# hamaadshah/gan_deeplearning4j

Hardware: NVIDIA H100
Metric: images/sec (full G+D step) (higher is better)
Workload: dtype bf16

## Files before the change

gan_deeplearning4j_b200/__init__.py:

```python
from ._lib import B200GanError, LIB_PATH, PROTOTYPES, load
from .engine import BF16, FP32, EPI_ACTBWD, EPI_BNBWD, EPI_PLAIN, EPI_STATS, Context, Gan, Net, comm_unique_id, test_bn, test_conv, test_conv_ex, test_dropout, test_ew, test_pool
from . import data, models, parallel, serializer
```

gan_deeplearning4j_b200/_lib.py:

```python
from __future__ import annotations

import ctypes as C
import os

_HERE = os.path.dirname(os.path.abspath(__file__))
LIB_PATH = os.path.join(_HERE, "lib", "libb200gan.so")
NAME_LEN = 64


class B200GanError(RuntimeError):
    def __init__(self, code, msg):
        super().__init__(f"libb200gan error {code}: {msg}")
        self.code = code


class LayerDesc(C.Structure):
    _fields_ = [("type", C.c_int32), ("name", C.c_char * NAME_LEN), ("n_in", C.c_int32), ("n_out", C.c_int32),
                ("k_h", C.c_int32), ("k_w", C.c_int32), ("s_h", C.c_int32), ("s_w", C.c_int32), ("p_h", C.c_int32), ("p_w", C.c_int32),
                ("has_bias", C.c_int32), ("act", C.c_int32), ("act_alpha", C.c_float), ("updater", C.c_int32),
                ("lr", C.c_float), ("beta1", C.c_float), ("beta2", C.c_float), ("eps", C.c_float), ("l2", C.c_float),
                ("bn_decay", C.c_float), ("bn_eps", C.c_float), ("pre_h", C.c_int32), ("pre_w", C.c_int32), ("pre_c", C.c_int32),
                ("loss", C.c_int32), ("frozen", C.c_int32)]


class NetConfig(C.Structure):
    _fields_ = [("in_h", C.c_int32), ("in_w", C.c_int32), ("in_c", C.c_int32), ("max_batch", C.c_int32), ("precision", C.c_int32),
                ("grad_clip", C.c_float), ("xent_clip_eps", C.c_float), ("bn_groups", C.c_int32), ("seed", C.c_uint64)]


class GanConfig(C.Structure):
    _fields_ = [("fake_bn_train", C.c_int32), ("use_cuda_graph", C.c_int32)]


class LrSchedule(C.Structure):
    _fields_ = [("kind", C.c_int32), ("type", C.c_int32), ("initial", C.c_double), ("gamma", C.c_double), ("power", C.c_double),
                ("step", C.c_double), ("decay_rate", C.c_double), ("n_map", C.c_int32), ("map_keys", C.POINTER(C.c_int32)),
                ("map_values", C.POINTER(C.c_double))]


class Constraint(C.Structure):
    _fields_ = [("kind", C.c_int32), ("dims_mask", C.c_int32), ("max_norm", C.c_double), ("min_norm", C.c_double), ("rate", C.c_double)]


class ConvGeom(C.Structure):
    _fields_ = [(k, C.c_int32) for k in ("n", "h", "w", "c", "oh", "ow", "o", "kh", "kw", "sh", "sw", "ph", "pw")]


class TestConvOpts(C.Structure):
    _fields_ = [("epi", C.c_int32), ("act", C.c_int32), ("alpha", C.c_float), ("bias", C.POINTER(C.c_float)), ("scale", C.POINTER(C.c_float)),
                ("groups", C.c_int32), ("aux", C.POINTER(C.c_float)), ("aux2", C.POINTER(C.c_float)), ("stats", C.POINTER(C.c_double)), ("kernel", C.c_char * 64),
                ("bn", C.c_int32), ("max_ctas", C.c_int32), ("poison", C.c_int32), ("w_mn", C.c_int32), ("per_tap", C.c_int32), ("slab", C.c_int32),
                ("defer", C.c_int32), ("db", C.POINTER(C.c_float)), ("param_offset", C.c_int32), ("splits", C.c_int32)]


class EwReduceJob(C.Structure):
    _fields_ = [("n", C.c_int64), ("stride", C.c_int64), ("src_off", C.c_int64), ("dst_off", C.c_int64), ("splits", C.c_int32), ("wide", C.c_int32)]


class TestEwOpts(C.Structure):
    _fields_ = [("op", C.c_int32), ("n", C.c_int64), ("rows", C.c_int32), ("cols", C.c_int32), ("groups", C.c_int32), ("splits", C.c_int32),
                ("stride", C.c_int64)] + [(k, C.c_int32) for k in ("N", "H", "W", "C", "KH", "KW", "SH", "SW", "act")] + [
                ("alpha", C.c_float), ("clip_eps", C.c_float), ("offset", C.c_int32), ("in_place", C.c_int32), ("accumulate", C.c_int32),
                ("poison", C.c_int32), ("n_jobs", C.c_int32), ("jobs", C.POINTER(EwReduceJob)), ("n_seg", C.c_int32),
                ("seg_off", C.POINTER(C.c_int64)), ("seg_len", C.POINTER(C.c_int64)), ("seg_coef", C.POINTER(C.c_float)), ("sumsq", C.c_double),
                ("kernel", C.c_char * 64), ("loss", C.c_int32)]


class TestPoolOpts(C.Structure):
    _fields_ = [("op", C.c_int32), ("pool", C.c_int32), ("pnorm", C.c_float)] + [
                (k, C.c_int32) for k in ("N", "H", "W", "C", "KH", "KW", "SH", "SW", "PH", "PW", "offset", "poison")] + [
                ("kernel", C.c_char * 64), ("splits", C.c_int32)]


_vp, _i32, _i64, _fp = C.c_void_p, C.c_int32, C.c_int64, C.POINTER(C.c_float)
_pvp = C.POINTER(C.c_void_p)

PROTOTYPES = {
    "b2g_version": (_i32, []),
    "b2g_ctx_create": (_i32, [_i32, _pvp]),
    "b2g_ctx_destroy": (_i32, [_vp]),
    "b2g_last_error": (C.c_char_p, []),
    "b2g_sync": (_i32, [_vp]),
    "b2g_launch_count": (_i32, [_vp, C.POINTER(C.c_uint64)]),
    "b2g_timer_start": (_i32, [_vp]),
    "b2g_timer_stop_ms": (_i32, [_vp, _fp]),
    "b2g_flush_l2": (_i32, [_vp]),
    "b2g_device_info": (_i32, [_vp, C.POINTER(_i32), C.POINTER(_i32), C.POINTER(_i32), C.POINTER(C.c_uint64)]),
    "b2g_net_create": (_i32, [_vp, C.POINTER(NetConfig), C.POINTER(LayerDesc), _i32, _pvp]),
    "b2g_net_destroy": (_i32, [_vp]),
    "b2g_net_num_params": (_i32, [_vp, C.POINTER(_i64)]),
    "b2g_net_output_size": (_i32, [_vp, C.POINTER(_i64)]),
    "b2g_net_layer_output_size": (_i32, [_vp, _i32, C.POINTER(_i64)]),
    "b2g_net_set_param": (_i32, [_vp, C.c_char_p, C.c_char_p, _fp, _i64]),
    "b2g_net_get_param": (_i32, [_vp, C.c_char_p, C.c_char_p, _fp, _i64]),
    "b2g_net_get_params": (_i32, [_vp, _fp, _i64]),
    "b2g_net_set_params": (_i32, [_vp, _fp, _i64]),
    "b2g_net_get_gradients": (_i32, [_vp, _fp, _i64]),
    "b2g_net_updater_state_size": (_i32, [_vp, C.POINTER(_i64)]),
    "b2g_net_get_updater_state": (_i32, [_vp, _fp, _i64]),
    "b2g_net_set_updater_state": (_i32, [_vp, _fp, _i64]),
    "b2g_net_output": (_i32, [_vp, _fp, _i32, _i32, _fp]),
    "b2g_net_get_activation": (_i32, [_vp, _i32, _i32, _fp]),
    "b2g_net_compute_gradient_and_score": (_i32, [_vp, _fp, _fp, _i32, _fp]),
    "b2g_net_get_input_gradient": (_i32, [_vp, _i32, _fp]),
    "b2g_net_fit": (_i32, [_vp, _fp, _fp, _i32, _fp]),
    "b2g_net_get_iteration": (_i32, [_vp, C.POINTER(_i64)]),
    "b2g_net_set_iteration": (_i32, [_vp, _i64]),
    "b2g_net_get_dropout_pass": (_i32, [_vp, C.POINTER(_i64)]),
    "b2g_net_set_dropout_pass": (_i32, [_vp, _i64]),
    "b2g_net_set_gradient_normalization": (_i32, [_vp, _i32, C.c_float]),
    "b2g_net_set_lr_schedule": (_i32, [_vp, C.c_char_p, C.POINTER(LrSchedule)]),
    "b2g_net_set_constraints": (_i32, [_vp, C.c_char_p, C.c_char_p, C.POINTER(Constraint), _i32]),
    "b2g_net_apply_constraints": (_i32, [_vp]),
    "b2g_net_get_learning_rate": (_i32, [_vp, C.c_char_p, _fp]),
    "b2g_net_get_epoch": (_i32, [_vp, C.POINTER(_i64)]),
    "b2g_net_set_epoch": (_i32, [_vp, _i64]),
    "b2g_net_simt_gemm_calls": (_i32, [_vp, C.POINTER(C.c_uint64)]),
    "b2g_gan_create": (_i32, [_vp, _vp, C.POINTER(GanConfig), _pvp]),
    "b2g_gan_destroy": (_i32, [_vp]),
    "b2g_gan_step": (_i32, [_vp, _fp, _fp, _fp, _fp, _fp, _fp, _i32, _fp]),
    "b2g_gan_upload": (_i32, [_vp, _fp, _fp, _fp, _fp, _fp, _fp, _i32]),
    "b2g_gan_step_resident": (_i32, [_vp, _i32]),
    "b2g_gan_read_losses": (_i32, [_vp, _fp]),
    "b2g_gan_last_step_ms": (_i32, [_vp, _fp]),
    "b2g_comm_unique_id": (_i32, [_vp]),
    "b2g_ctx_comm_init": (_i32, [_vp, _i32, _i32, _vp]),
    "b2g_ctx_comm_destroy": (_i32, [_vp]),
    "b2g_net_set_grad_allreduce": (_i32, [_vp, _i32]),
    "b2g_net_average_parameters": (_i32, [_vp]),
    "b2g_net_set_sync_bn": (_i32, [_vp, _i32]),
    "b2g_net_set_grad_payload_bf16": (_i32, [_vp, _i32]),
    "b2g_net_enable_p2p_allreduce": (_i32, [_vp, C.POINTER(C.c_int32)]),
    "b2g_ctx_allreduce_test": (_i32, [_vp, _fp, _i64]),
    "b2g_test_conv": (_i32, [_vp, _i32, _i32, _i32, C.POINTER(ConvGeom), _fp, _fp, _fp, _i32, _fp]),
    "b2g_test_hbm_kernels": (_i32, [_vp, _i32, _i32, _i32, _fp]),
    "b2g_test_conv_ex": (_i32, [_vp, _i32, _i32, _i32, C.POINTER(ConvGeom), _fp, _fp, _fp, _i32, _fp, C.POINTER(TestConvOpts)]),
    "b2g_test_bn": (_i32, [_vp, _i32, _i32, _i32, _i32, _i32, _fp, _fp, _fp, _fp, _fp, _fp, _i32, C.c_float, C.c_float, C.c_float,
                           _i32, _fp, _fp, _fp, _fp, _fp, _fp, _fp, _fp]),
    "b2g_test_net_shadow": (_i32, [_vp, _i32, _i32, _fp, _i64]),
    "b2g_test_dropout": (_i32, [_vp, _i32, C.c_uint64, _i32, _i32, _i64, _i32, _i32, _i32, _i32, C.c_float, _fp, _fp, _fp, _fp]),
    "b2g_test_ew": (_i32, [_vp, _i32, C.POINTER(TestEwOpts), _fp, _fp, _fp, _fp, _fp]),
    "b2g_test_pool": (_i32, [_vp, _i32, C.POINTER(TestPoolOpts), _fp, _fp, _fp, _fp, _fp]),
}

_lib = None


def load():
    global _lib
    if _lib is not None:
        return _lib
    if not os.path.exists(LIB_PATH):
        raise B200GanError(-7, f"{LIB_PATH} is missing: build it with `make` (nvcc, sm_90a). There is no CPU fallback.")
    lib = C.CDLL(LIB_PATH, mode=C.RTLD_GLOBAL)
    for name, (res, args) in PROTOTYPES.items():
        fn = getattr(lib, name)
        fn.restype, fn.argtypes = res, args
    _lib = lib
    return lib


def check(code):
    if code != 0:
        raise B200GanError(code, load().b2g_last_error().decode(errors="replace"))
```

gan_deeplearning4j_b200/csrc/engine.cu:

```cuda
#include <cuda_runtime.h>
#include <dlfcn.h>
#include <math.h>
#include <stdarg.h>
#include <stdio.h>
#include <stdlib.h>
#include <string.h>

#include <algorithm>
#include <string>
#include <vector>

#include "../../include/b200gan.h"
#include "kernels.h"

using namespace b2g;

static thread_local char g_err[1024] = "";
static int32_t fail(int32_t code, const char* fmt, ...) {
  va_list ap; va_start(ap, fmt); vsnprintf(g_err, sizeof(g_err), fmt, ap); va_end(ap); return code;
}
#define CU(call) do { cudaError_t e_ = (call); if (e_ != cudaSuccess) return fail(B2G_ERR_CUDA, "%s:%d %s -> %s", __FILE__, __LINE__, #call, cudaGetErrorString(e_)); } while (0)
#define B2(call) do { int32_t r_ = (call); if (r_ != 0) return r_; } while (0)
#define CHECK_KERNELS() CU(cudaGetLastError())

// ... 336 lines not shown
      const size_t part = k_global_pool_partial_elems(n->prec, R, l.ih * l.iw, l.ic);
      if (part) {
        B2(dalloc(n, &l.pool_part, sizeof(float) * part));
        if (l.pool == B2G_POOL_MAX) B2(dalloc(n, &l.pool_part_idx, sizeof(int32_t) * part));
      }
      B2(dalloc(n, &l.pool_ticket, sizeof(unsigned))); CU(cudaMemsetAsync(l.pool_ticket, 0, sizeof(unsigned), n->ctx->stream));
    }
    if (l.d.type == B2G_LAYER_BATCHNORM) { B2(dalloc(n, &l.bn_fold, sizeof(float) * 2 * l.oc)); B2(dalloc(n, &l.bn_mean, sizeof(float) * G * l.oc)); B2(dalloc(n, &l.bn_invstd, sizeof(float) * G * l.oc)); scratch = std::max(scratch, k_bn_scratch_floats(l.oc, G));
      if (k_bn_vec_ok(n->prec, l.oc)) { B2(dalloc(n, &l.bn_coef, sizeof(float) * 4 * G * l.oc)); bn_acc_words += 2 * k_bn_acc_elems(l.oc, G); } }
    if (l.has_gemm()) {
      ConvGeom g = l.geom; g.N = R;
      scratch = std::max(scratch, std::max(k_simt_wgrad_scratch_floats(g), k_tc_wgrad_scratch_floats(g)));
      scratch = std::max(scratch, std::max(k_edge_wgrad_scratch_floats(g), k_dense_small_o_wgrad_scratch_floats(g)));
      scratch = std::max(scratch, k_tc_edge_wgrad_scratch_floats(g));
      scratch = std::max(scratch, k_colsum_scratch_floats(std::max(l.oc, l.ic)));
      max_w = std::max(max_w, (size_t)l.n_W);
      if (n->prec == PREC_BF16 && n->ctx->tc_ok && !l.d.frozen) {
        l.wg_part_floats = std::max(std::max(k_tc_wgrad_scratch_floats(g), k_tc_edge_wgrad_scratch_floats(g)), k_head_wgrad_scratch_floats(g));
        if (l.wg_part_floats) B2(dalloc(n, &l.wg_part, sizeof(float) * l.wg_part_floats));
      }
    }
  }
  if (bn_acc_words) {
    n->bn_acc_bytes = sizeof(unsigned long long) * bn_acc_words; B2(dalloc(n, &n->bn_acc, n->bn_acc_bytes));
    unsigned long long* q = n->bn_acc;
    for (auto& l : n->L) if (l.bn_coef) { const size_t w = k_bn_acc_elems(l.oc, G); l.acc_fwd = q; l.acc_bwd = q + w; q += 2 * w; }
  }
  n->eps_elems = (size_t)R * max_act;
  B2(dalloc(n, (char**)&n->epsA, ts * n->eps_elems)); B2(dalloc(n, (char**)&n->epsB, ts * n->eps_elems)); B2(dalloc(n, (char**)&n->epsC, ts * n->eps_elems));
  n->scratch_floats = scratch; B2(dalloc(n, &n->scratch, sizeof(float) * scratch)); B2(dalloc(n, &n->scratch2, sizeof(float) * scratch));
  {
    double tot_p = (double)std::max<int64_t>(1, n->n_params), tot_w = 0; std::vector<double> work(n->L.size(), 0.0);
    for (size_t i = 0; i < n->L.size(); ++i) { const auto& l = n->L[i]; if (l.has_gemm()) work[i] = (double)l.geom.OH * l.geom.OW * l.geom.O * l.geom.KH * l.geom.KW * l.geom.C; tot_w += work[i]; }
    double best = 0.0, ahead = 0.0;
    for (size_t i = 1; i < n->L.size(); ++i) {
      ahead += work[i - 1];
      const auto& l = n->L[i]; int64_t off = -1;
      if (l.has_gemm()) off = l.off_b >= 0 ? std::min(l.off_b, l.off_W) : l.off_W; else if (l.d.type == B2G_LAYER_BATCHNORM) off = l.off_gamma;
      if (off < 0 || tot_w <= 0) continue;
      const double score = std::min((tot_p - (double)off) / tot_p, ahead / tot_w);
      if (score > best) { best = score; n->ar_split_layer = (int)i; n->ar_split_off = off; }
    }
    if (best < 0.1) n->ar_split_layer = -1;
  }
  n->ev_fork.resize(n->L.size()); n->ev_done.resize(n->L.size());
  for (size_t i = 0; i < n->L.size(); ++i) { CU(cudaEventCreateWithFlags(&n->ev_fork[i], cudaEventDisableTiming)); CU(cudaEventCreateWithFlags(&n->ev_done[i], cudaEventDisableTiming)); }
  CU(cudaEventCreateWithFlags(&n->ev_join, cudaEventDisableTiming));
  n->stage_floats = std::max((size_t)R * max_act, std::max((size_t)n->n_params, max_w)); B2(dalloc(n, &n->stage_f32, sizeof(float) * n->stage_floats));
  return 0;
}

static int updater_kind(int u) { return u; }

static int32_t net_init_params_and_updater(b2g_net* n) {
  cudaStream_t s = n->ctx->stream;
  std::vector<float> hp(n->n_params, 0.f), h0(n->n_params, 0.f);
  uint64_t seed = n->cfg.seed ? n->cfg.seed : 666;
  std::vector<int64_t> l2o, l2l; std::vector<float> l2c;
  std::vector<int> seg_layer;
  for (auto& l : n->L) {
    const b2g_layer_desc& d = l.d;
    auto add_seg = [&](int64_t off, int64_t len, bool weight, bool noop) {
      if (d.frozen) return;
      UpdSeg sg{}; sg.off = off; sg.len = len; sg.kind = noop ? 3 : updater_kind(d.updater);
      sg.lr = d.lr; sg.b1 = d.beta1; sg.b2 = d.beta2; sg.eps = d.eps; sg.l2 = weight ? d.l2 : 0.f; sg.clip = n->cfg.grad_clip; sg.div_mb = noop ? 0 : 1;
      sg.off_bf = (weight && l.off_W_bf >= 0) ? l.off_W_bf : -1; sg.off_ps = (weight && l.off_Wps_bf >= 0) ? l.off_Wps_bf : -1; sg.ps_O = l.geom.O; sg.ps_C = l.geom.C; n->segs.push_back(sg); seg_layer.push_back((int)(&l - n->L.data()));
      if (!noop && (sg.kind == 1 || sg.kind == 5)) for (int64_t i = 0; i < len; ++i) h0[off + i] = d.eps;
      if (weight && d.l2 != 0.f) { l2o.push_back(off); l2l.push_back(len); l2c.push_back(0.5f * d.l2); }
    };
    if (l.has_gemm()) {
      double fi = (double)d.n_in * l.wTaps, fo = (double)d.n_out * l.wTaps / ((d.type == B2G_LAYER_CONV2D || d.type == B2G_LAYER_DECONV2D) ? (double)(d.s_h * d.s_w) : 1.0);
      float sd = (float)sqrt(2.0 / (fi + fo));
      for (int64_t i = 0; i < l.n_W; ++i) hp[l.off_W + i] = sd * nrand(seed);
      if (l.off_b >= 0 && l.off_b < l.off_W) add_seg(l.off_b, d.n_out, false, false);
      add_seg(l.off_W, l.n_W, true, false);
      if (l.off_b >= 0 && l.off_b > l.off_W) add_seg(l.off_b, d.n_out, false, false);
    } else if (d.type == B2G_LAYER_BATCHNORM) {
      for (int c = 0; c < l.oc; ++c) { hp[l.off_gamma + c] = 1.f; hp[l.off_var + c] = 1.f; }
      add_seg(l.off_gamma, l.oc, false, false); add_seg(l.off_beta, l.oc, false, false);
      add_seg(l.off_mean, l.oc, false, true); add_seg(l.off_var, l.oc, false, true);
    }
  }
  CU(cudaMemcpyAsync(n->params, hp.data(), sizeof(float) * n->n_params, cudaMemcpyHostToDevice, s));
  CU(cudaMemcpyAsync(n->st0, h0.data(), sizeof(float) * n->n_params, cudaMemcpyHostToDevice, s));
  CU(cudaMemsetAsync(n->st1, 0, sizeof(float) * n->n_params, s)); CU(cudaMemsetAsync(n->grads, 0, sizeof(float) * n->n_params, s));
  bool amsgrad = false;
  for (const UpdSeg& sg : n->segs) { n->upd_ext = n->upd_ext || sg.kind >= 4; amsgrad = amsgrad || sg.kind == 8; }
  if (amsgrad) { B2(dalloc(n, &n->st2, sizeof(float) * n->n_params)); CU(cudaMemsetAsync(n->st2, 0, sizeof(float) * n->n_params, s)); }
  CU(cudaMemsetAsync(n->step_dev, 0, sizeof(int), s));
  std::vector<int32_t> cs; std::vector<int64_t> co;
  for (size_t i = 0; i < n->segs.size(); ++i) for (int64_t o = n->segs[i].off; o < n->segs[i].off + n->segs[i].len; o += UPD_CHUNK) { cs.push_back((int32_t)i); co.push_back(o); }
  n->nchunks = (int)cs.size();
  B2(dalloc(n, &n->segs_dev, sizeof(UpdSeg) * std::max<size_t>(1, n->segs.size()))); B2(dalloc(n, &n->chunk_seg_dev, sizeof(int32_t) * std::max(1, n->nchunks))); B2(dalloc(n, &n->chunk_off_dev, sizeof(int64_t) * std::max(1, n->nchunks)));
  CU(cudaMemcpyAsync(n->segs_dev, n->segs.data(), sizeof(UpdSeg) * n->segs.size(), cudaMemcpyHostToDevice, s));
  CU(cudaMemcpyAsync(n->chunk_seg_dev, cs.data(), sizeof(int32_t) * cs.size(), cudaMemcpyHostToDevice, s));
  CU(cudaMemcpyAsync(n->chunk_off_dev, co.data(), sizeof(int64_t) * co.size(), cudaMemcpyHostToDevice, s));
  {
    const int ns = (int)n->segs.size();
    std::vector<int32_t> seg_c0(ns + 1, n->nchunks);
    for (int c = n->nchunks - 1; c >= 0; --c) seg_c0[cs[c]] = c;
    std::vector<GnGroup> per_layer, per_param;
    for (int i = 0; i < ns; ++i) {
      per_param.push_back(GnGroup{seg_c0[i], seg_c0[i + 1], i, i + 1});
      if (i > 0 && seg_layer[i] == seg_layer[i - 1]) { per_layer.back().chunk_end = seg_c0[i + 1]; per_layer.back().seg_end = i + 1; }
      else per_layer.push_back(GnGroup{seg_c0[i], seg_c0[i + 1], i, i + 1});
    }
    n->gn_n_layer_groups = (int)per_layer.size(); n->gn_n_param_groups = (int)per_param.size();
    B2(dalloc(n, &n->gn_layer_groups, sizeof(GnGroup) * std::max<size_t>(1, per_layer.size()))); B2(dalloc(n, &n->gn_param_groups, sizeof(GnGroup) * std::max<size_t>(1, per_param.size())));
    B2(dalloc(n, &n->gn_partial, sizeof(double) * std::max(1, n->nchunks))); B2(dalloc(n, &n->gn_mult, sizeof(float) * std::max(1, ns)));
    B2(dalloc(n, &n->gn_ticket, sizeof(unsigned))); CU(cudaMemsetAsync(n->gn_ticket, 0, sizeof(unsigned), s));
    CU(cudaMemcpyAsync(n->gn_layer_groups, per_layer.data(), sizeof(GnGroup) * per_layer.size(), cudaMemcpyHostToDevice, s));
    CU(cudaMemcpyAsync(n->gn_param_groups, per_param.data(), sizeof(GnGroup) * per_param.size(), cudaMemcpyHostToDevice, s));
  }
  {
    n->seg_layer = seg_layer; n->layer_sched.assign(n->L.size(), b2g_net::LayerSched{});
    B2(dalloc(n, &n->sched_dev, sizeof(UpdSched) * std::max<size_t>(1, n->segs.size()))); CU(cudaMemsetAsync(n->sched_dev, 0, sizeof(UpdSched) * std::max<size_t>(1, n->segs.size()), s));
    B2(dalloc(n, &n->epoch_dev, sizeof(int64_t))); CU(cudaMemsetAsync(n->epoch_dev, 0, sizeof(int64_t), s));
    B2(dalloc(n, &n->lr_out, sizeof(float)));
  }
  n->n_l2 = (int)l2o.size();
  if (n->n_l2) {
    B2(dalloc(n, &n->l2_off_dev, sizeof(int64_t) * n->n_l2)); B2(dalloc(n, &n->l2_len_dev, sizeof(int64_t) * n->n_l2)); B2(dalloc(n, &n->l2_coef_dev, sizeof(float) * n->n_l2));
    CU(cudaMemcpyAsync(n->l2_off_dev, l2o.data(), sizeof(int64_t) * n->n_l2, cudaMemcpyHostToDevice, s));
    CU(cudaMemcpyAsync(n->l2_len_dev, l2l.data(), sizeof(int64_t) * n->n_l2, cudaMemcpyHostToDevice, s));
    CU(cudaMemcpyAsync(n->l2_coef_dev, l2c.data(), sizeof(float) * n->n_l2, cudaMemcpyHostToDevice, s));
  }
  CU(cudaStreamSynchronize(s));
  return 0;
}

static void net_refresh_shadow(b2g_net* n, int only_layer = -1) {
  if (n->prec != PREC_BF16) return;
  cudaStream_t st = n->ctx->stream;
  for (size_t i = 0; i < n->L.size(); ++i) { auto& l = n->L[i];
    if (!l.has_gemm() || (only_layer >= 0 && (int)i != only_layer)) continue;
    if (l.off_Wps_bf >= 0) k_pack_deconv_ps(n->params + l.off_W, n->shadow + l.off_Wps_bf, l.geom.O, l.geom.C, st);
    k_cast_f32_to_bf16(n->params + l.off_W, n->shadow + l.off_W_bf, (size_t)l.n_W, st);
  }
}

struct FwdOpts { int rows; int groups; bool train; bool update_running; void* out_override; };

static const void* w_ptr(const b2g_net* n, const LayerRT& l, int* wprec) {
  if (n->prec == PREC_BF16) { *wprec = PREC_BF16; return n->shadow + l.off_W_bf; }
  *wprec = PREC_F32; return n->params + l.off_W;
}

static inline bool tc_on(const b2g_net* n) { return n->prec == PREC_BF16 && n->ctx->tc_ok; }
static inline cudaStream_t fstream(const b2g_net* n) { return n->fwd_stream ? n->fwd_stream : n->ctx->stream; }
static inline void note_simt(b2g_net* n) { if (n->prec == PREC_BF16) ++n->simt_gemm_calls; }

static inline int sync_bn_world(const b2g_net* n) { return (n->sync_bn && n->ctx->comm && n->ctx->world > 1) ? n->ctx->world : 1; }
static int32_t gemm_fprop(b2g_net* n, const LayerRT& l, const ConvGeom& g, const void* x, const float* bias, void* out, int act, float alpha,
                          const float* scale = nullptr, const TcEpi* fuse = nullptr, bool* fused = nullptr) {
  cudaStream_t s = fstream(n); int wp; const void* w = w_ptr(n, l, &wp);
  if (fused) *fused = false;
  if (scale) {
    if (tc_on(n) && tc_fprop_supported(g)) { TcEpi e{}; e.mode = EPI_PLAIN; e.scale = scale; return k_tc_fprop(g, (const __nv_bfloat16*)x, (const __nv_bfloat16*)w, bias, (__nv_bfloat16*)out, act, alpha, s, &e) == 0 ? 0 : fail(B2G_ERR_CUDA, "tensor-core fprop launch failed"); }
    note_simt(n); k_simt_fprop(n->prec, wp, g, x, w, bias, out, act, alpha, s, scale); return 0;
  }
  if (tc_on(n) && tc_edge_conv_supported(g) && k_tc_edge_conv(g, (const __nv_bfloat16*)x, (const __nv_bfloat16*)w, bias, (__nv_bfloat16*)out, act, alpha, s) == 0) return 0;
  if (edge_conv_small_cin_supported(g)) { note_simt(n); k_edge_conv_small_cin(n->prec, wp, g, x, w, bias, out, act, alpha, s); return 0; }
  if (dense_small_o_supported(g)) { note_simt(n); k_dense_small_o_fwd(n->prec, wp, g, x, w, bias, out, act, alpha, s); return 0; }
  if (tc_on(n) && tc_fprop_supported(g)) {
    if (fuse && k_tc_fprop(g, (const __nv_bfloat16*)x, (const __nv_bfloat16*)w, bias, (__nv_bfloat16*)out, act, alpha, s, fuse) == 0) { if (fused) *fused = true; return 0; }
    if (k_tc_fprop(g, (const __nv_bfloat16*)x, (const __nv_bfloat16*)w, bias, (__nv_bfloat16*)out, act, alpha, s) == 0) return 0;
    return fail(B2G_ERR_CUDA, "tensor-core fprop launch failed");
  }
  if (n->prec == PREC_BF16 && head_conv_supported(g)) { k_head_fwd(g, (const __nv_bfloat16*)x, (const __nv_bfloat16*)w, bias, (__nv_bfloat16*)out, act, alpha, s); return 0; }
  note_simt(n); k_simt_fprop(n->prec, wp, g, x, w, bias, out, act, alpha, s); return 0;
}
static int32_t gemm_dgrad(b2g_net* n, const LayerRT& l, const ConvGeom& g, const void* dy, const float* bias, void* dx, int act, float alpha,
                          const float* scale = nullptr, const TcEpi* fuse = nullptr, bool* fused = nullptr) {
  cudaStream_t s = fstream(n); int wp; const void* w = w_ptr(n, l, &wp);
  if (fused) *fused = false;
  if (scale) {
    if (tc_on(n) && tc_dgrad_supported(g) && !edge_deconv_small_c_supported(g)) { TcEpi e{}; e.mode = EPI_PLAIN; e.scale = scale; return k_tc_dgrad(g, (const __nv_bfloat16*)dy, (const __nv_bfloat16*)w, bias, (__nv_bfloat16*)dx, act, alpha, s, &e) == 0 ? 0 : fail(B2G_ERR_CUDA, "tensor-core dgrad launch failed"); }
    note_simt(n); k_simt_dgrad(n->prec, wp, g, dy, w, bias, dx, act, alpha, s, scale); return 0;
  }
  if (tc_on(n) && l.off_Wps_bf >= 0 && tc_deconv_ps_supported(g)) {
    const TcEpi* f = (fuse && fuse->mode == EPI_ACTBWD) ? fuse : nullptr;
    if (k_tc_deconv_ps(g, (const __nv_bfloat16*)dy, n->shadow + l.off_Wps_bf, bias, (__nv_bfloat16*)dx, act, alpha, s, f) == 0) { if (fused) *fused = f != nullptr; return 0; }
    return fail(B2G_ERR_CUDA, "tensor-core pixel-shuffle deconv launch failed");
  }
  if (edge_deconv_small_c_supported(g)) { note_simt(n); k_edge_deconv_small_c(n->prec, wp, g, dy, w, bias, dx, act, alpha, s); return 0; }
  if (dense_small_o_supported(g) && !bias && act == ACT_IDENTITY) { note_simt(n); k_dense_small_o_dgrad(n->prec, wp, g, dy, w, dx, s); return 0; }
  if (dense_small_k_supported(g) && !(tc_on(n) && g.O % 64 == 0)) { note_simt(n); k_dense_small_k_dgrad(n->prec, wp, g, dy, w, bias, dx, act, alpha, s); return 0; }
  if (tc_on(n) && g.KH == 1 && g.KW == 1 && g.H == 1 && g.W == 1) {
    ConvGeom t = g; t.C = g.O; t.O = g.C;
    if (tc_fprop_supported(t)) {
      if (fuse && k_tc_fprop(t, (const __nv_bfloat16*)dy, (const __nv_bfloat16*)w, bias, (__nv_bfloat16*)dx, act, alpha, s, fuse, 1) == 0) { if (fused) *fused = true; return 0; }
      if (k_tc_fprop(t, (const __nv_bfloat16*)dy, (const __nv_bfloat16*)w, bias, (__nv_bfloat16*)dx, act, alpha, s, nullptr, 1) == 0) return 0;
      return fail(B2G_ERR_CUDA, "tensor-core dense dgrad launch failed");
    }
  }
  if (tc_on(n) && tc_dgrad_supported(g)) {
    if (fuse && k_tc_dgrad(g, (const __nv_bfloat16*)dy, (const __nv_bfloat16*)w, bias, (__nv_bfloat16*)dx, act, alpha, s, fuse) == 0) { if (fused) *fused = true; return 0; }
    if (k_tc_dgrad(g, (const __nv_bfloat16*)dy, (const __nv_bfloat16*)w, bias, (__nv_bfloat16*)dx, act, alpha, s) == 0) return 0;
    return fail(B2G_ERR_CUDA, "tensor-core dgrad launch failed");
  }
  if (n->prec == PREC_BF16 && head_conv_supported(g)) { k_head_dgrad(g, (const __nv_bfloat16*)dy, (const __nv_bfloat16*)w, bias, (__nv_bfloat16*)dx, act, alpha, s); return 0; }
  note_simt(n); k_simt_dgrad(n->prec, wp, g, dy, w, bias, dx, act, alpha, s); return 0;
}
static int32_t gemm_wgrad(b2g_net* n, LayerRT& l, const ConvGeom& g, const void* x, const void* dy, float* dw, cudaStream_t s, float* scratch, float* db = nullptr, bool* bias_done = nullptr) {
  if (tc_on(n) && tc_edge_wgrad_supported(g) && l.wg_part) { const int r = k_tc_edge_wgrad(g, (const __nv_bfloat16*)x, (const __nv_bfloat16*)dy, dw, db, l.wg_part, l.wg_part_floats, 0, s, &n->pending); if (r >= 0) { if (bias_done) *bias_done = r == 1; return 0; } }
  if (edge_wgrad_small_cin_supported(g)) { note_simt(n); k_edge_wgrad_small_cin(n->prec, g, x, dy, dw, scratch, 0, s); return 0; }
  if (dense_small_o_supported(g)) { note_simt(n); k_dense_small_o_wgrad(n->prec, g, x, dy, dw, scratch, 0, s); return 0; }
  if (dense_small_k_supported(g) && !(tc_on(n) && tc_wgrad_supported(g))) { note_simt(n); k_dense_small_k_wgrad(n->prec, g, x, dy, dw, s); return 0; }
  if (tc_on(n) && tc_wgrad_supported(g) && l.wg_part) {
    if (k_tc_wgrad(g, (const __nv_bfloat16*)x, (const __nv_bfloat16*)dy, dw, l.wg_part, l.wg_part_floats, 0, s, &n->pending) == 0) return 0;
    return fail(B2G_ERR_CUDA, "tensor-core wgrad launch failed");
  }
  if (n->prec == PREC_BF16 && head_conv_supported(g) && l.wg_part) {
    if (k_head_wgrad(g, (const __nv_bfloat16*)x, (const __nv_bfloat16*)dy, dw, l.wg_part, l.wg_part_floats, 0, s, &n->pending) == 0) return 0;
    return fail(B2G_ERR_CUDA, "few-output conv weight gradient: partials larger than the layer's region");
  }
  note_simt(n); k_simt_wgrad(n->prec, g, x, dy, dw, scratch, n->scratch_floats, 0, s); return 0;
}

static DropoutArgs make_dropout_args(uint64_t seed, int layer, int rank, float p) {
  DropoutArgs a{}; a.seed = seed ? seed : 666; a.tag = (uint32_t)layer | ((uint32_t)rank << 16);
  a.keep_all = p >= 1.f ? 1 : 0; a.threshold = a.keep_all ? 0u : (uint32_t)floor((double)p * 4294967296.0); a.scale = 1.0f / p;
  return a;
}
static DropoutArgs dropout_args(const b2g_net* n, int layer) { return make_dropout_args(n->cfg.seed, layer, n->ctx->rank, n->L[layer].d.act_alpha); }

static int32_t net_forward(b2g_net* n, const void* in, const FwdOpts& o, const void** result) {
  cudaStream_t s = fstream(n);
  if (o.rows > n->max_rows || o.rows < 1) return fail(B2G_ERR_SHAPE, "batch %d outside [1, max_batch=%d]", o.rows, n->max_rows);
  if (o.groups < 1 || o.rows % o.groups) return fail(B2G_ERR_SHAPE, "batch %d not divisible into %d groups", o.rows, o.groups);
  const int R = o.rows; const void* cur = in;
  n->last_rows = R;
  if (o.train && n->bn_acc) CU(cudaMemsetAsync(n->bn_acc, 0, n->bn_acc_bytes, s));
  int last_drop = -1;
  if (o.train) for (size_t i = 0; i < n->L.size(); ++i) if (n->L[i].drop_active()) last_drop = (int)i;
  for (size_t i = 0; i < n->L.size(); ++i) {
    LayerRT& l = n->L[i]; const b2g_layer_desc& d = l.d;
    void* out = l.out;
    if (i + 1 == n->L.size() && o.out_override && !l.out_alias) out = o.out_override;
    const float* bias = l.off_b >= 0 ? n->params + l.off_b : nullptr;
    const bool gemm_then_bn = (d.type == B2G_LAYER_CONV2D || d.type == B2G_LAYER_DECONV2D || d.type == B2G_LAYER_DENSE) && i + 1 < n->L.size() && n->L[i + 1].d.type == B2G_LAYER_BATCHNORM;
    const bool remapped = d.type == B2G_LAYER_DECONV2D && l.geom.KH == 1 && l.geom.C != l.oc;
    if (gemm_then_bn && d.act == B2G_ACT_IDENTITY && !l.ext_act && (!o.train || n->L[i + 1].d.frozen) && !(i + 2 == n->L.size() && o.out_override) && !remapped &&
        !l.n_skip) {
      LayerRT& bn = n->L[i + 1];
      ConvGeom g = l.geom; g.N = R;
      k_bn_fold(n->params + bn.off_mean, n->params + bn.off_var, n->params + bn.off_gamma, n->params + bn.off_beta, bias, bn.oc, bn.d.bn_eps, bn.bn_fold, bn.bn_fold + bn.oc, s);
      if (d.type == B2G_LAYER_DECONV2D) B2(gemm_dgrad(n, l, g, cur, bn.bn_fold + bn.oc, bn.out, bn.fused_act, bn.fused_alpha, bn.bn_fold));
      else B2(gemm_fprop(n, l, g, cur, bn.bn_fold + bn.oc, bn.out, bn.fused_act, bn.fused_alpha, bn.bn_fold));
      cur = bn.out; ++i; continue;
    }
    TcEpi st{}; const TcEpi* fuse = nullptr; bool fused = false;
    if (gemm_then_bn && o.train && !n->L[i + 1].d.frozen && n->L[i + 1].bn_coef && !remapped && tc_on(n) && !l.ext_act) {
      st.mode = EPI_STATS; st.acc = n->L[i + 1].acc_fwd; st.imgs_per_group = R / o.groups; fuse = &st;
    }
    void* gout = l.ext_z ? l.ext_z : out;
    switch (d.type) {
      case B2G_LAYER_CONV2D: case B2G_LAYER_DENSE: case B2G_LAYER_OUTPUT: { ConvGeom g = l.geom; g.N = R; B2(gemm_fprop(n, l, g, cur, bias, gout, d.act, d.act_alpha, nullptr, fuse, &fused)); } break;
      case B2G_LAYER_DECONV2D: { ConvGeom g = l.geom; g.N = R; B2(gemm_dgrad(n, l, g, cur, bias, gout, d.act, d.act_alpha, nullptr, fuse, &fused)); } break;
      case B2G_LAYER_BATCHNORM: {
        int rows_pg = (R / o.groups) * l.oh * l.ow;
        const bool bn_train = o.train && !d.frozen;
        l.fwd_fused = false;
        if (bn_train && l.bn_coef) {
          if (!l.stats_by_producer) k_bn_stats_acc(cur, rows_pg, l.oc, o.groups, l.acc_fwd, s);
          const int reps = sync_bn_world(n);
          if (reps > 1) NC(g_nccl.ar(l.acc_fwd, l.acc_fwd, k_bn_acc_elems(l.oc, o.groups),  5,  0, n->ctx->comm, s));
          k_bn_apply_acc(cur, out, rows_pg, l.oc, o.groups, l.acc_fwd, n->params + l.off_gamma, n->params + l.off_beta, l.fused_act, l.fused_alpha, d.bn_eps, l.bn_coef,
                         n->params + l.off_mean, n->params + l.off_var, o.update_running ? n->grads + l.off_mean : nullptr, o.update_running ? n->grads + l.off_var : nullptr, d.bn_decay, s, reps);
          l.fwd_fused = true; l.stats_by_producer = false; l.fwd_groups = o.groups;
          break;
        }
        if (bn_train) k_bn_stats(n->prec, cur, rows_pg, l.oc, o.groups, n->scratch, l.bn_mean, l.bn_invstd, d.bn_eps, n->params + l.off_mean, n->params + l.off_var,
                                o.update_running ? n->grads + l.off_mean : nullptr, o.update_running ? n->grads + l.off_var : nullptr, d.bn_decay, s);
        else k_bn_prep_infer(n->params + l.off_mean, n->params + l.off_var, l.oc, o.groups, d.bn_eps, l.bn_mean, l.bn_invstd, s);
        k_bn_apply(n->prec, cur, out, rows_pg, l.oc, o.groups, l.bn_mean, l.bn_invstd, n->params + l.off_gamma, n->params + l.off_beta, l.fused_act, l.fused_alpha, s);
      } break;
      case B2G_LAYER_ACTIVATION:
        if (l.act_fused_into_prev) out = (void*)cur;
        else if (l.ext_act) k_act_ext_fwd(n->prec, l.ext_act, l.ext_alpha, cur, out, (size_t)R * l.out_elems, s);
        else k_act_fwd(n->prec, cur, out, (size_t)R * l.out_elems, d.act, d.act_alpha, s);
        break;
      case B2G_LAYER_MAXPOOL: k_maxpool_fwd(n->prec, cur, out, l.argmax, R, l.ih, l.iw, l.ic, l.oh, l.ow, d.k_h, d.k_w, d.s_h, d.s_w, s); break;
      case B2G_LAYER_SUBSAMPLING: k_pool2d_fwd(n->prec, l.pool, l.pnorm, cur, out, R, l.ih, l.iw, l.ic, l.oh, l.ow, d.k_h, d.k_w, d.s_h, d.s_w, d.p_h, d.p_w, s); break;
      case B2G_LAYER_GLOBAL_POOLING: k_global_pool_fwd(n->prec, l.pool, l.pnorm, cur, out, l.pool_idx, R, l.ih * l.iw, l.ic, l.pool_part, l.pool_part_idx, l.pool_ticket, s); break;
      case B2G_LAYER_UPSAMPLE2D: k_upsample_fwd(n->prec, cur, out, R, l.ih, l.iw, l.ic, d.k_h, s); break;
      case B2G_LAYER_LOSS: case B2G_LAYER_CNN_LOSS: out = (void*)cur; break;
      case B2G_LAYER_FF_TO_CNN: if (l.out_alias) out = (void*)cur; else k_permute(n->prec, cur, out, R, l.oc, l.oh * l.ow, 1, s); break;
      case B2G_LAYER_CNN_TO_FF: if (l.out_alias) out = (void*)cur; else k_permute(n->prec, cur, out, R, l.ic, l.ih * l.iw, 0, s); break;
      case B2G_LAYER_DROPOUT:
        l.drop_live = o.train && l.drop_active();
        if (l.drop_live) {
          k_dropout_fwd(n->prec, cur, l.drop_buf, l.drop_mask, (size_t)R * l.out_elems, dropout_args(n, (int)i), n->drop_pass, n->drop_ticket, (int)i == last_drop, s);
          out = l.drop_buf;
        } else out = (void*)cur;
        l.out = out;
        break;
      case B2G_LAYER_ELEMENTWISE: {
        const void* sk = n->L[l.vsrc].out;
        k_vertex_ew_fwd(n->prec, d.act, l.vorder ? sk : cur, l.vorder ? cur : sk, out, (size_t)R * l.out_elems, s);
      } break;
      case B2G_LAYER_MERGE: {
        const LayerRT& src = n->L[l.vsrc]; const size_t px = (size_t)R * l.oh * l.ow;
        if (l.vorder) k_merge_fwd(n->prec, src.out, cur, out, px, src.oc, l.ic, s);
        else k_merge_fwd(n->prec, cur, src.out, out, px, l.ic, src.oc, s);
      } break;
    }
    if (l.ext_z) k_act_ext_fwd(n->prec, l.ext_act, l.ext_alpha, l.ext_z, out, (size_t)R * l.out_elems, s);
    if (fuse) n->L[i + 1].stats_by_producer = fused;
    if (l.out_alias) l.out = out;
    cur = out;
  }
  CHECK_KERNELS();
  if (result) *result = cur;
  return 0;
}

static bool ar_overlap_on(const b2g_net* n) {
  static int on = -1; if (on < 0) { const char* e = getenv("B2G_AR_OVERLAP"); on = (e && e[0] == '1') ? 1 : 0; }
  return on && n->ctx->comm && n->ctx->world > 1 && n->grad_allreduce && n->ar_split_layer > 0 && !n->sync_bn;
}
static void flush_pending_reduce(b2g_net* n, cudaStream_t s2) { if (n->pending.count) { k_reduce_multi(n->pending, s2); n->pending.count = 0; } }

static int32_t net_backward(b2g_net* n, const void* net_in, void* eps, int rows, int groups, bool want_wgrad, bool need_input_grad, bool allreduce_follows = false,
                            const TcEpi* input_act = nullptr, bool* input_act_done = nullptr, bool top_act_done = false) {
  cudaStream_t s = n->ctx->stream, s2 = n->ctx->side; const int R = rows;
  void* cur = eps;
  if (input_act_done) *input_act_done = false;
  n->pending.count = 0;
  void* bufs[3] = {n->epsA, n->epsB, n->epsC}; cudaEvent_t reader[3] = {nullptr, nullptr, nullptr}; bool forked = false;
  auto other = [&](void* p) -> void* {
    int pick = -1;
    for (int k = 0; k < 3; ++k) if (bufs[k] != p && !reader[k]) { pick = k; break; }
    if (pick < 0) for (int k = 0; k < 3; ++k) if (bufs[k] != p) { pick = k; break; }
    if (reader[pick]) { cudaStreamWaitEvent(s, reader[pick], 0); reader[pick] = nullptr; }
    return bufs[pick];
  };
  auto fork_wgrad = [&](int li, const void* delta) {
    cudaEventRecord(n->ev_fork[li], s); cudaStreamWaitEvent(s2, n->ev_fork[li], 0); forked = true; (void)delta;
  };
  auto mark_reader = [&](int li, const void* delta) {
    cudaEventRecord(n->ev_done[li], s2);
    for (int k = 0; k < 3; ++k) if (bufs[k] == delta) reader[k] = n->ev_done[li];
  };
  std::vector<char> act_done(n->L.size(), 0);
  if (top_act_done) act_done.back() = 1;
  auto pick_fuse = [&](int i, TcEpi* e, int* target) -> bool {
    *target = -1;
    if (!tc_on(n)) return false;
    int k = i - 1; while (k >= 0 && n->L[k].act_fused_into_prev) --k;
    if (k < 0) { if (input_act) { *e = *input_act; *target = -2; return true; } return false; }
    for (int m = k; m < i; ++m) if (n->L[m].n_skip) return false;
    LayerRT& b = n->L[k];
    if (b.d.type == B2G_LAYER_BATCHNORM && b.fwd_fused && !b.d.frozen && b.fwd_groups == groups) {
      e->mode = EPI_BNBWD; e->acc = b.acc_bwd; e->imgs_per_group = R / groups; e->aux = (const __nv_bfloat16*)b.out; e->aux2 = (const __nv_bfloat16*)(k == 0 ? net_in : n->L[k - 1].out);
      e->act = b.fused_act; e->alpha = b.fused_alpha; *target = k; return true;
    }
    if (k == i - 1 && b.has_gemm() && b.d.act != B2G_ACT_IDENTITY && b.d.type != B2G_LAYER_OUTPUT) {
      e->mode = EPI_ACTBWD; e->aux = (const __nv_bfloat16*)b.out; e->act = b.d.act; e->alpha = b.d.act_alpha; *target = k; return true;
    }
    return false;
  };
  auto note_fused = [&](int target, const TcEpi& e, bool fused) {
    if (!fused || target == -1) return;
    if (target == -2) { if (input_act_done) *input_act_done = true; return; }
    if (e.mode == EPI_BNBWD) n->L[target].bwd_premul = true; else act_done[target] = 1;
  };
  for (int i = (int)n->L.size() - 1; i >= 0; --i) {
    LayerRT& l = n->L[i]; const b2g_layer_desc& d = l.d;
    const void* lin = i == 0 ? net_in : n->L[i - 1].out;
    bool need_in = need_input_grad;
    if (!need_in) for (int j = 0; j < i; ++j) if (!n->L[j].d.frozen && (n->L[j].has_gemm() || n->L[j].d.type == B2G_LAYER_BATCHNORM)) need_in = true;
    const bool want_wgrad_l = want_wgrad && !d.frozen;
    if (l.skip_acc) k_skip_add(n->prec, cur, l.skip_acc, (size_t)R * l.out_elems, s);
    switch (d.type) {
      case B2G_LAYER_LOSS: case B2G_LAYER_CNN_LOSS: break;
      case B2G_LAYER_ELEMENTWISE:
        if (need_in) k_vertex_ew_bwd(n->prec, d.act, l.vorder, cur, lin, n->L[l.vsrc].out, n->L[l.vsrc].skip_acc, l.vfirst ? 0 : 1, (size_t)R * l.out_elems, s);
        break;
      case B2G_LAYER_MERGE:
        if (need_in) {
          const LayerRT& src = n->L[l.vsrc]; void* nx = other(cur);
          k_merge_bwd(n->prec, cur, nx, src.skip_acc, (size_t)R * l.oh * l.ow, l.vorder ? src.oc : l.ic, l.vorder ? l.ic : src.oc, l.vorder == 0, l.vfirst ? 0 : 1, s);
          cur = nx;
        }
        break;
      case B2G_LAYER_CONV2D: case B2G_LAYER_DENSE: case B2G_LAYER_OUTPUT: {
        ConvGeom g = l.geom; g.N = R;
        if (d.act != B2G_ACT_IDENTITY && !act_done[i]) k_act_bwd_from_output(n->prec, l.out, cur, cur, (size_t)R * l.out_elems, d.act, d.act_alpha, s);
        if (l.ext_z) k_act_ext_bwd(n->prec, l.ext_act, l.ext_alpha, l.ext_z, cur, (size_t)R * l.out_elems, s);
        if (want_wgrad_l) {
          fork_wgrad(i, cur);
          bool bias_done = false;
          B2(gemm_wgrad(n, l, g, lin, cur, n->grads + l.off_W, s2, n->scratch2, l.off_b >= 0 ? n->grads + l.off_b : nullptr, &bias_done));
          if (l.off_b >= 0 && !bias_done) k_colsum(n->prec, cur, R * l.oh * l.ow, l.oc, n->scratch2, n->grads + l.off_b, 0, s2);
          mark_reader(i, cur);
        }
        if (need_in) { void* nx = other(cur); TcEpi e{}; int tgt; bool fused = false; const bool can = pick_fuse(i, &e, &tgt);
          B2(gemm_dgrad(n, l, g, cur, nullptr, nx, ACT_IDENTITY, 0.f, nullptr, can ? &e : nullptr, &fused)); note_fused(tgt, e, fused); cur = nx; }
      } break;
      case B2G_LAYER_DECONV2D: {
        ConvGeom g = l.geom; g.N = R;
        if (d.act != B2G_ACT_IDENTITY && !act_done[i]) k_act_bwd_from_output(n->prec, l.out, cur, cur, (size_t)R * l.out_elems, d.act, d.act_alpha, s);
        if (l.ext_z) k_act_ext_bwd(n->prec, l.ext_act, l.ext_alpha, l.ext_z, cur, (size_t)R * l.out_elems, s);
        if (want_wgrad_l) {
          fork_wgrad(i, cur);
          B2(gemm_wgrad(n, l, g,  cur,  lin, n->grads + l.off_W, s2, n->scratch2));
          if (l.off_b >= 0) k_colsum(n->prec, cur, R * l.oh * l.ow, l.oc, n->scratch2, n->grads + l.off_b, 0, s2);
          mark_reader(i, cur);
        }
        if (need_in) { void* nx = other(cur); TcEpi e{}; int tgt; bool fused = false; const bool can = pick_fuse(i, &e, &tgt);
          B2(gemm_fprop(n, l, g, cur, nullptr, nx, ACT_IDENTITY, 0.f, nullptr, can ? &e : nullptr, &fused)); note_fused(tgt, e, fused); cur = nx; }
      } break;
      case B2G_LAYER_BATCHNORM: {
        if (d.frozen) { if (need_in) return fail(B2G_ERR_UNSUPPORTED, "layer %d: a gradient through a frozen BatchNorm (trainable layer or input gradient below it) is not implemented", i); break; }
        if (l.fwd_fused && l.fwd_groups != groups) return fail(B2G_ERR_ARG, "layer %d: BatchNorm backward in %d groups after a forward in %d", i, groups, l.fwd_groups);
        int rows_pg = (R / groups) * l.oh * l.ow; void* nx = need_in ? other(cur) : nullptr;
        if (l.fwd_fused) {
          if (!l.bwd_premul) k_bn_bwd_stats_acc(lin, cur, rows_pg, l.oc, groups, l.bn_coef, l.fused_act, l.fused_alpha, l.acc_bwd, s);
          const int reps = sync_bn_world(n);
          if (reps > 1) NC(g_nccl.ar(l.acc_bwd, l.acc_bwd, k_bn_acc_elems(l.oc, groups),  5,  0, n->ctx->comm, s));
          k_bn_bwd_apply_acc(lin, cur, nx, rows_pg, l.oc, groups, l.bn_coef, l.fused_act, l.fused_alpha, l.bwd_premul ? 1 : 0, l.acc_bwd, n->grads + l.off_gamma, n->grads + l.off_beta, want_wgrad_l ? 1 : 0, s, reps);
          l.bwd_premul = false;
        } else
        k_bn_bwd(n->prec, lin, cur, nx, rows_pg, l.oc, groups, l.bn_mean, l.bn_invstd, n->params + l.off_gamma, n->params + l.off_beta, l.fused_act, l.fused_alpha,
                 n->scratch, n->grads + l.off_gamma, n->grads + l.off_beta, want_wgrad_l ? 1 : 0, s);
        if (need_in) cur = nx;
      } break;
      case B2G_LAYER_ACTIVATION:
        if (l.ext_act) k_act_ext_bwd(n->prec, l.ext_act, l.ext_alpha, lin, cur, (size_t)R * l.out_elems, s);
        else if (!l.act_fused_into_prev) k_act_bwd_from_output(n->prec, l.out, cur, cur, (size_t)R * l.out_elems, d.act, d.act_alpha, s);
        break;
      case B2G_LAYER_MAXPOOL: if (need_in) { void* nx = other(cur); k_maxpool_bwd(n->prec, cur, l.argmax, nx, R, l.ih, l.iw, l.ic, l.oh, l.ow, d.k_h, d.k_w, d.s_h, d.s_w, s); cur = nx; } break;
      case B2G_LAYER_SUBSAMPLING:
        if (need_in) { void* nx = other(cur); k_pool2d_bwd(n->prec, l.pool, l.pnorm, cur, lin, l.out, nx, R, l.ih, l.iw, l.ic, l.oh, l.ow, d.k_h, d.k_w, d.s_h, d.s_w, d.p_h, d.p_w, s); cur = nx; }
        break;
      case B2G_LAYER_GLOBAL_POOLING:
        if (need_in) { void* nx = other(cur); k_global_pool_bwd(n->prec, l.pool, l.pnorm, cur, lin, l.out, l.pool_idx, nx, R, l.ih * l.iw, l.ic, s); cur = nx; }
        break;
      case B2G_LAYER_UPSAMPLE2D: if (need_in) { void* nx = other(cur); k_upsample_bwd(n->prec, cur, nx, R, l.ih, l.iw, l.ic, d.k_h, s); cur = nx; } break;
      case B2G_LAYER_FF_TO_CNN: if (!l.out_alias && need_in) { void* nx = other(cur); k_permute(n->prec, cur, nx, R, l.oc, l.oh * l.ow, 0, s); cur = nx; } break;
      case B2G_LAYER_CNN_TO_FF: if (!l.out_alias && need_in) { void* nx = other(cur); k_permute(n->prec, cur, nx, R, l.ic, l.ih * l.iw, 1, s); cur = nx; } break;
      case B2G_LAYER_DROPOUT: if (need_in && l.drop_live) k_dropout_bwd(n->prec, cur, cur, l.drop_mask, (size_t)R * l.out_elems, 1.0f / d.act_alpha, s); break;
    }
    if (i == n->ar_split_layer && want_wgrad && allreduce_follows && ar_overlap_on(n)) {
      b2g_ctx* c = n->ctx;
      cudaEventRecord(c->ev_c0, s); cudaStreamWaitEvent(c->comm_stream, c->ev_c0, 0);
      if (forked) { flush_pending_reduce(n, s2); cudaEventRecord(c->ev_c1, s2); cudaStreamWaitEvent(c->comm_stream, c->ev_c1, 0); }
      NC(g_nccl.ar(n->grads + n->ar_split_off, n->grads + n->ar_split_off, (size_t)(n->n_params - n->ar_split_off),  7,  0, c->comm, c->comm_stream));
      n->ar_tail_sent = true;
    }
    if (!need_in) { cur = nullptr; break; }
  }
  n->input_grad = cur;
  if (forked) { flush_pending_reduce(n, s2); cudaEventRecord(n->ev_join, s2); cudaStreamWaitEvent(s, n->ev_join, 0); }
  CHECK_KERNELS();
  return 0;
}

static int32_t net_allreduce_grads(b2g_net* n) {
  b2g_ctx* c = n->ctx; if (!c->comm || c->world == 1 || !n->grad_allreduce) return 0;
  if (n->ar_tail_sent) {
    n->ar_tail_sent = false;
    cudaEventRecord(c->ev_c0, c->stream); cudaStreamWaitEvent(c->comm_stream, c->ev_c0, 0);
    NC(g_nccl.ar(n->grads, n->grads, (size_t)n->ar_split_off,  7,  0, c->comm, c->comm_stream));
    cudaEventRecord(c->ev_c2, c->comm_stream); cudaStreamWaitEvent(c->stream, c->ev_c2, 0);
    return 0;
  }
  if (n->ar_bf16 && n->ar_buf) {
    k_cast_f32_to_bf16(n->grads, n->ar_buf, (size_t)n->n_params, c->stream);
    NC(g_nccl.ar(n->ar_buf, n->ar_buf, (size_t)n->n_params,  9,  0, c->comm, c->stream));
    k_nhwc_to_nchw_f32(PREC_BF16, n->ar_buf, n->grads, 1, 1, (int)n->n_params, c->stream);
    return 0;
  }
  if (n->p2p) {
    P2pArgs a{}; for (int r = 0; r < c->world; ++r) { a.grads[r] = n->p2p_peer_grads[r]; a.flags[r] = c->p2p_peer_flags[r]; }
    a.rank = c->rank; a.world = c->world; a.n = (size_t)n->n_params; a.state = c->p2p_state;
    k_p2p_allreduce(a, c->stream); CHECK_KERNELS(); return 0;
  }
  NC(g_nccl.ar(n->grads, n->grads, (size_t)n->n_params,  7,  0, c->comm, c->stream));
  return 0;
}
static void net_launch_constraints(b2g_net* n, cudaStream_t s) {
  for (const auto& r : n->con_rounds) {
    k_constraint_onepass(n->params, n->shadow, n->con_jobs, r.j0, r.j1, r.onepass_blocks, s);
    k_constraint_twopass(n->params, n->shadow, n->con_jobs, r.t0, r.t1, r.norm_blocks, r.scale_blocks, n->con_partial, n->con_ticket, n->con_mult, s);
  }
}
static int32_t net_update(b2g_net* n, int mb_local) {
  cudaStream_t s = n->ctx->stream; int W = n->ctx->comm ? n->ctx->world : 1;
  if (!n->grad_allreduce) W = 1;
  const float inv_mb = 1.0f / ((float)mb_local * W), inv_world = 1.0f / (float)W;
  const bool gn = n->gn_mode != B2G_GN_NONE;
  if (gn) {
    const bool per_layer = n->gn_mode == B2G_GN_RENORM_L2_LAYER || n->gn_mode == B2G_GN_CLIP_L2_LAYER;
    const bool clip = n->gn_mode == B2G_GN_CLIP_L2_LAYER || n->gn_mode == B2G_GN_CLIP_L2_PARAM;
    k_gradnorm(n->grads, n->segs_dev, n->chunk_seg_dev, n->chunk_off_dev, n->nchunks, per_layer ? n->gn_layer_groups : n->gn_param_groups,
               per_layer ? n->gn_n_layer_groups : n->gn_n_param_groups, clip ? 1 : 0, n->gn_threshold, inv_mb, inv_world, n->gn_partial, n->gn_ticket, n->gn_mult, s);
  }
  k_updater(n->params, n->grads, n->st0, n->st1, n->st2, n->segs_dev, n->chunk_seg_dev, n->chunk_off_dev, n->nchunks, inv_mb, inv_world, n->step_dev, n->upd_ticket,
            n->shadow, gn ? n->gn_mult : nullptr, n->sched_on ? n->sched_dev : nullptr, n->epoch_dev, n->upd_ext, s);
  net_launch_constraints(n, s);
  CHECK_KERNELS();
  return 0;
}

extern "C" int32_t b2g_version(void) { return B2G_VERSION; }
extern "C" const char* b2g_last_error(void) { return g_err; }

extern "C" int32_t b2g_ctx_create(int32_t device, b2g_ctx** out) {
  if (!out) return fail(B2G_ERR_ARG, "null out");
  int count = 0; cudaError_t e = cudaGetDeviceCount(&count);
  if (e != cudaSuccess || count == 0) return fail(B2G_ERR_NO_DEVICE, "no CUDA device (%s); libb200gan has no CPU fallback", e == cudaSuccess ? "count=0" : cudaGetErrorString(e));
  if (device < 0 || device >= count) return fail(B2G_ERR_ARG, "device %d of %d", device, count);
  CU(cudaSetDevice(device));
  b2g_ctx* c = new b2g_ctx(); c->device = device;
  CU(cudaGetDeviceProperties(&c->prop, device));
  if (c->prop.major != 9) { int mj = c->prop.major, mn = c->prop.minor; delete c; return fail(B2G_ERR_NO_DEVICE, "device is sm_%d%d; this library is built for sm_90a (H100) only", mj, mn); }
  CU(cudaStreamCreateWithFlags(&c->stream, cudaStreamNonBlocking));
  CU(cudaStreamCreateWithFlags(&c->side, cudaStreamNonBlocking)); CU(cudaStreamCreateWithFlags(&c->side2, cudaStreamNonBlocking));
  CU(cudaEventCreateWithFlags(&c->ev_a, cudaEventDisableTiming)); CU(cudaEventCreateWithFlags(&c->ev_b, cudaEventDisableTiming));
  CU(cudaStreamCreateWithFlags(&c->comm_stream, cudaStreamNonBlocking));
  CU(cudaEventCreateWithFlags(&c->ev_c0, cudaEventDisableTiming)); CU(cudaEventCreateWithFlags(&c->ev_c1, cudaEventDisableTiming)); CU(cudaEventCreateWithFlags(&c->ev_c2, cudaEventDisableTiming));
  c->tc_ok = tc_init() == 0;
  *out = c; return 0;
}
extern "C" int32_t b2g_ctx_destroy(b2g_ctx* c) {
  if (!c) return 0; cudaSetDevice(c->device);
  if (c->p2p_flags_mapped) for (int r = 0; r < c->world; ++r) if (r != c->rank && c->p2p_peer_flags[r]) cudaIpcCloseMemHandle(c->p2p_peer_flags[r]);
  if (c->p2p_flags) cudaFree(c->p2p_flags); if (c->p2p_state) cudaFree(c->p2p_state);
  if (c->comm && g_nccl.destroy) g_nccl.destroy(c->comm);
  if (c->t0) { cudaEventDestroy(c->t0); cudaEventDestroy(c->t1); } if (c->flush_buf) cudaFree(c->flush_buf);
  if (c->side) cudaStreamDestroy(c->side); if (c->side2) cudaStreamDestroy(c->side2); if (c->ev_a) cudaEventDestroy(c->ev_a); if (c->ev_b) cudaEventDestroy(c->ev_b);
  if (c->comm_stream) cudaStreamDestroy(c->comm_stream); if (c->ev_c0) cudaEventDestroy(c->ev_c0); if (c->ev_c1) cudaEventDestroy(c->ev_c1); if (c->ev_c2) cudaEventDestroy(c->ev_c2);
  if (c->stream) cudaStreamDestroy(c->stream); delete c; return 0;
}
extern "C" int32_t b2g_timer_start(b2g_ctx* c) {
  if (!c) return fail(B2G_ERR_ARG, "null ctx"); CU(cudaSetDevice(c->device));
  if (!c->t0) { CU(cudaEventCreate(&c->t0)); CU(cudaEventCreate(&c->t1)); }
  CU(cudaEventRecord(c->t0, c->stream)); return 0;
}
extern "C" int32_t b2g_timer_stop_ms(b2g_ctx* c, float* ms) {
  if (!c || !ms || !c->t0) return fail(B2G_ERR_ARG, "timer not started"); CU(cudaSetDevice(c->device));
  CU(cudaEventRecord(c->t1, c->stream)); CU(cudaEventSynchronize(c->t1)); CU(cudaEventElapsedTime(ms, c->t0, c->t1)); return 0;
}
extern "C" int32_t b2g_flush_l2(b2g_ctx* c) {
  if (!c) return fail(B2G_ERR_ARG, "null ctx"); CU(cudaSetDevice(c->device));
  if (!c->flush_buf) { c->flush_bytes = (size_t)256 << 20; CU(cudaMalloc(&c->flush_buf, c->flush_bytes)); }
  CU(cudaMemsetAsync(c->flush_buf, 0, c->flush_bytes, c->stream)); return 0;
}
extern "C" int32_t b2g_sync(b2g_ctx* c) { if (!c) return fail(B2G_ERR_ARG, "null ctx"); CU(cudaSetDevice(c->device)); CU(cudaStreamSynchronize(c->stream)); return 0; }
extern "C" int32_t b2g_launch_count(b2g_ctx* c, uint64_t* out) { if (!c || !out) return fail(B2G_ERR_ARG, "null"); *out = g_launch_count; return 0; }
extern "C" int32_t b2g_device_info(b2g_ctx* c, int32_t* sm, int32_t* mj, int32_t* mn, uint64_t* mem) {
  if (!c) return fail(B2G_ERR_ARG, "null ctx");
  if (sm) *sm = c->prop.multiProcessorCount; if (mj) *mj = c->prop.major; if (mn) *mn = c->prop.minor; if (mem) *mem = c->prop.totalGlobalMem; return 0;
}

extern "C" int32_t b2g_net_create(b2g_ctx* ctx, const b2g_net_config* cfg, const b2g_layer_desc* layers, int32_t nl, b2g_net** out) {
  if (!ctx || !cfg || !layers || nl < 1 || !out) return fail(B2G_ERR_ARG, "b2g_net_create: null/empty argument");
  if (cfg->max_batch < 1 || cfg->in_h < 1 || cfg->in_w < 1 || cfg->in_c < 1) return fail(B2G_ERR_ARG, "b2g_net_create: bad input type / max_batch");
  if (cfg->precision != B2G_PREC_FP32 && cfg->precision != B2G_PREC_BF16) return fail(B2G_ERR_ARG, "b2g_net_create: precision %d", cfg->precision);
  for (int32_t i = 0; i < nl; ++i)
    if (layers[i].updater < B2G_UPD_SGD || layers[i].updater > B2G_UPD_ADADELTA) return fail(B2G_ERR_ARG, "b2g_net_create: layer %d: unknown updater %d", i, layers[i].updater);
  CU(cudaSetDevice(ctx->device));
  b2g_net* n = new b2g_net(); n->ctx = ctx; n->cfg = *cfg; n->prec = cfg->precision == B2G_PREC_BF16 ? PREC_BF16 : PREC_F32;
  if (n->cfg.bn_groups < 1) n->cfg.bn_groups = 1;
  int32_t r = net_build(n, layers, nl); if (!r) r = net_alloc(n); if (!r) r = net_init_params_and_updater(n);
  if (!r) { net_refresh_shadow(n); cudaError_t e = cudaStreamSynchronize(ctx->stream); if (e != cudaSuccess) r = fail(B2G_ERR_CUDA, "init: %s", cudaGetErrorString(e)); }
  if (r) { for (void* p : n->allocs) cudaFree(p); delete n; return r; }
  *out = n; return 0;
}
extern "C" int32_t b2g_net_destroy(b2g_net* n) {
  if (!n) return 0; cudaSetDevice(n->ctx->device); cudaStreamSynchronize(n->ctx->stream); cudaStreamSynchronize(n->ctx->side);
  for (auto e : n->ev_fork) if (e) cudaEventDestroy(e); for (auto e : n->ev_done) if (e) cudaEventDestroy(e); if (n->ev_join) cudaEventDestroy(n->ev_join);
  if (n->p2p) for (int r = 0; r < n->ctx->world; ++r) if (r != n->ctx->rank && n->p2p_peer_grads[r]) cudaIpcCloseMemHandle(n->p2p_peer_grads[r]);
  if (n->sched_map) cudaFree(n->sched_map);
  cudaFree(n->con_jobs); cudaFree(n->con_partial); cudaFree(n->con_mult);
  for (void* p : n->allocs) cudaFree(p); delete n; return 0;
}
extern "C" int32_t b2g_net_num_params(b2g_net* n, int64_t* out) { if (!n || !out) return fail(B2G_ERR_ARG, "null"); *out = n->n_params; return 0; }
extern "C" int32_t b2g_net_output_size(b2g_net* n, int64_t* out) { if (!n || !out) return fail(B2G_ERR_ARG, "null"); *out = (int64_t)n->L.back().out_elems; return 0; }
extern "C" int32_t b2g_net_layer_output_size(b2g_net* n, int32_t layer, int64_t* out) {
  if (!n || !out || layer < 0 || layer >= (int)n->L.size()) return fail(B2G_ERR_ARG, "bad layer index"); *out = (int64_t)n->L[layer].out_elems; return 0;
}

struct ParamRef { int64_t off, len; bool conv_w; int A, B, taps; int layer; };
static int32_t find_param(b2g_net* n, const char* layer, const char* param, ParamRef* r) {
  for (size_t i = 0; i < n->L.size(); ++i) { LayerRT& l = n->L[i];
    if (strncmp(l.d.name, layer, B2G_NAME_LEN)) continue;
    r->conv_w = false; r->layer = (int)i;
    if (!strcmp(param, "W") && l.off_W >= 0) { r->off = l.off_W; r->len = l.n_W; r->conv_w = l.wTaps > 1; r->A = l.wA; r->B = l.wB; r->taps = l.wTaps; return 0; }
    if (!strcmp(param, "b") && l.off_b >= 0) { r->off = l.off_b; r->len = l.d.n_out; return 0; }
    if (l.d.type == B2G_LAYER_BATCHNORM) {
      if (!strcmp(param, "gamma")) { r->off = l.off_gamma; r->len = l.oc; return 0; }
      if (!strcmp(param, "beta")) { r->off = l.off_beta; r->len = l.oc; return 0; }
      if (!strcmp(param, "mean")) { r->off = l.off_mean; r->len = l.oc; return 0; }
      if (!strcmp(param, "var")) { r->off = l.off_var; r->len = l.oc; return 0; }
    }
    return fail(B2G_ERR_ARG, "layer %s has no parameter %s", layer, param);
  }
  return fail(B2G_ERR_ARG, "no layer named %s", layer);
}
extern "C" int32_t b2g_net_set_param(b2g_net* n, const char* layer, const char* param, const float* host, int64_t cnt) {
  if (!n || !layer || !param || !host) return fail(B2G_ERR_ARG, "null"); CU(cudaSetDevice(n->ctx->device));
  ParamRef r; B2(find_param(n, layer, param, &r));
  if (cnt != r.len) return fail(B2G_ERR_SHAPE, "%s.%s has %lld elements, got %lld", layer, param, (long long)r.len, (long long)cnt);
  std::vector<float> tmp; const float* src = host;
  if (r.conv_w) { tmp.resize(r.len); w_dl4j_to_internal(host, tmp.data(), r.A, r.B, r.taps); src = tmp.data(); }
// ... 1018 lines not shown
      }
      break;
    }
    case B2G_EW_ACT_FWD: case B2G_EW_ACT_BWD: {
      const size_t n = (size_t)o->n; const bool bwd = o->op == B2G_EW_ACT_BWD;
      if (!in0 || (bwd && !in1) || o->n < 1 || o->n > lim || o->act < B2G_ACT_IDENTITY || o->act > B2G_ACT_LRELU) return fail(B2G_ERR_ARG, "bad activation arguments");
      void *a = nullptr, *e = nullptr, *r = nullptr; B2(m.upT(in0, n, &a, off));
      if (bwd) B2(m.upT(in1, n, &e, off));
      if (bwd && o->in_place) r = e;
      else { B2(m.dev(n, ts, &r, off)); B2(poison(r, ts * n)); }
      if (bwd) k_act_bwd_from_output(prec, a, e, r, n, o->act, o->alpha, s);
      else k_act_fwd(prec, a, r, n, o->act, o->alpha, s);
      ran();
      B2(m.downT(out0, r, n));
      break;
    }
    case B2G_EW_ACT_EXT_FWD: case B2G_EW_ACT_EXT_BWD: {
      const size_t n = (size_t)o->n; const bool bwd = o->op == B2G_EW_ACT_EXT_BWD;
      if (!in0 || (bwd && !in1) || o->n < 1 || o->n > lim || !act_ext_kind(o->act) || !std::isfinite(o->alpha)) return fail(B2G_ERR_ARG, "bad activation arguments");
      void *z = nullptr, *r = nullptr; B2(m.upT(in0, n, &z, off));
      if (bwd) B2(m.upT(in1, n, &r, off));
      else { B2(m.dev(n, ts, &r, off)); B2(poison(r, ts * n)); }
      if (bwd) k_act_ext_bwd(prec, o->act, o->alpha, z, r, n, s);
      else k_act_ext_fwd(prec, o->act, o->alpha, z, r, n, s);
      ran();
      B2(m.downT(out0, r, n));
      break;
    }
    case B2G_EW_MAXPOOL: {
      if (!in0 || !in1 || o->N < 1 || o->C < 1 || o->KH < 1 || o->KW < 1 || o->SH < 1 || o->SW < 1 || o->H < o->KH || o->W < o->KW || o->KH * o->KW > 255)
        return fail(B2G_ERR_ARG, "bad MAXPOOL arguments");
      const int OH = (o->H - o->KH) / o->SH + 1, OW = (o->W - o->KW) / o->SW + 1;
      const size_t ni = (size_t)o->N * o->H * o->W * o->C, no = (size_t)o->N * OH * OW * o->C;
      if (ni > (size_t)lim) return fail(B2G_ERR_ARG, "MAXPOOL input too large");
      void *x = nullptr, *eo = nullptr, *y = nullptr, *ei = nullptr; uint8_t* arg = nullptr;
      B2(m.upT(in0, ni, &x, off)); B2(m.upT(in1, no, &eo, off)); B2(m.dev(no, ts, &y, off)); B2(m.dev(ni, ts, &ei, off)); B2(m.dev(no, 1, (void**)&arg, off));
      B2(poison(y, ts * no)); B2(poison(ei, ts * ni)); B2(poison(arg, no));
      k_maxpool_fwd(prec, x, y, arg, o->N, o->H, o->W, o->C, OH, OW, o->KH, o->KW, o->SH, o->SW, s); ran();
      k_maxpool_bwd(prec, eo, arg, ei, o->N, o->H, o->W, o->C, OH, OW, o->KH, o->KW, o->SH, o->SW, s); ran();
      B2(m.downT(out0, y, no)); B2(m.downT(out1, ei, ni));
      if (out2) {
        std::vector<uint8_t> h(no); CU(cudaMemcpyAsync(h.data(), arg, no, cudaMemcpyDeviceToHost, s)); CU(cudaStreamSynchronize(s));
        for (size_t i = 0; i < no; ++i) out2[i] = (float)h[i];
      }
      break;
    }
    case EW_POOL2D: {
      if (!po) return fail(B2G_ERR_ARG, "unknown op %d", o->op);
      if (!in0 || !in1 || o->N < 1 || o->H < 1 || o->W < 1 || o->C < 1 || o->KH < 1 || o->KW < 1 || o->SH < 1 || o->SW < 1 || po->PH < 0 || po->PW < 0 ||
          po->PH >= o->KH || po->PW >= o->KW || o->H + 2 * po->PH < o->KH || o->W + 2 * po->PW < o->KW || po->pool < B2G_POOL_AVG || po->pool > B2G_POOL_PNORM ||
          (po->pool == B2G_POOL_PNORM && !(po->pnorm >= 1.f && po->pnorm <= 1024.f && po->pnorm == floorf(po->pnorm))))
        return fail(B2G_ERR_ARG, "bad POOL2D arguments");
      const int OH = (o->H + 2 * po->PH - o->KH) / o->SH + 1, OW = (o->W + 2 * po->PW - o->KW) / o->SW + 1;
      const size_t ni = (size_t)o->N * o->H * o->W * o->C, no = (size_t)o->N * OH * OW * o->C;
      if (ni > (size_t)lim || no > (size_t)lim) return fail(B2G_ERR_ARG, "POOL2D tensors too large");
      void *x = nullptr, *eo = nullptr, *y = nullptr, *ei = nullptr;
      B2(m.upT(in0, ni, &x, off)); B2(m.upT(in1, no, &eo, off)); B2(m.dev(no, ts, &y, off)); B2(m.dev(ni, ts, &ei, off)); B2(poison(y, ts * no)); B2(poison(ei, ts * ni));
      const int pn = po->pool == B2G_POOL_PNORM ? (int)po->pnorm : 0;
      k_pool2d_fwd(prec, po->pool, pn, x, y, o->N, o->H, o->W, o->C, OH, OW, o->KH, o->KW, o->SH, o->SW, po->PH, po->PW, s); ran();
      k_pool2d_bwd(prec, po->pool, pn, eo, x, y, ei, o->N, o->H, o->W, o->C, OH, OW, o->KH, o->KW, o->SH, o->SW, po->PH, po->PW, s); ran();
      B2(m.downT(out0, y, no)); B2(m.downT(out1, ei, ni));
      break;
    }
    case EW_GLOBAL_POOL: {
      if (!po) return fail(B2G_ERR_ARG, "unknown op %d", o->op);
      if (!in0 || !in1 || o->N < 1 || o->H < 1 || o->W < 1 || o->C < 1 || po->pool < B2G_POOL_MAX || po->pool > B2G_POOL_PNORM ||
          (po->pool == B2G_POOL_PNORM && !(po->pnorm >= 1.f && po->pnorm <= 1024.f && po->pnorm == floorf(po->pnorm))))
        return fail(B2G_ERR_ARG, "bad GLOBAL_POOL arguments");
      const int HW = o->H * o->W;
      const size_t ni = (size_t)o->N * HW * o->C, no = (size_t)o->N * o->C;
      if (ni > (size_t)lim) return fail(B2G_ERR_ARG, "GLOBAL_POOL input too large");
      void *x = nullptr, *eo = nullptr, *y = nullptr, *ei = nullptr; int32_t *idx = nullptr, *part_idx = nullptr; float* part = nullptr; unsigned* ticket = nullptr;
      B2(m.upT(in0, ni, &x, off)); B2(m.upT(in1, no, &eo, off)); B2(m.dev(no, ts, &y, off)); B2(m.dev(ni, ts, &ei, off)); B2(m.dev(no, 4, (void**)&idx, off));
      const size_t np = std::max<size_t>(1, k_global_pool_partial_elems(prec, o->N, HW, o->C));
      B2(m.dev(np, 4, (void**)&part, off)); B2(m.dev(np, 4, (void**)&part_idx, off)); B2(m.dev(1, 4, (void**)&ticket, off)); CU(cudaMemsetAsync(ticket, 0, 4, s));
      B2(poison(y, ts * no)); B2(poison(ei, ts * ni)); B2(poison(idx, 4 * no));
      const int pn = po->pool == B2G_POOL_PNORM ? (int)po->pnorm : 0;
      k_global_pool_fwd(prec, po->pool, pn, x, y, po->pool == B2G_POOL_MAX ? idx : nullptr, o->N, HW, o->C, part, part_idx, ticket, s); ran();
      po->splits = g_pool_last_splits;
      k_global_pool_bwd(prec, po->pool, pn, eo, x, y, idx, ei, o->N, HW, o->C, s); ran();
      B2(m.downT(out0, y, no)); B2(m.downT(out1, ei, ni));
      if (out2) {
        std::vector<int32_t> h(no); CU(cudaMemcpyAsync(h.data(), idx, 4 * no, cudaMemcpyDeviceToHost, s)); CU(cudaStreamSynchronize(s));
        for (size_t i = 0; i < no; ++i) out2[i] = (float)h[i];
      }
      unsigned t = 1; CU(cudaMemcpyAsync(&t, ticket, 4, cudaMemcpyDeviceToHost, s)); CU(cudaStreamSynchronize(s));
      if (t != 0) return fail(B2G_ERR_CUDA, "GLOBAL_POOL: the forward left its ticket word at %u", t);
      break;
    }
    case B2G_EW_UPSAMPLE: {
      const int f = o->KH;
      if (!in0 || !in1 || o->N < 1 || o->H < 1 || o->W < 1 || o->C < 1 || f < 1) return fail(B2G_ERR_ARG, "bad UPSAMPLE arguments");
      const size_t ni = (size_t)o->N * o->H * o->W * o->C, no = ni * f * f;
      if (no > (size_t)lim) return fail(B2G_ERR_ARG, "UPSAMPLE output too large");
      void *x = nullptr, *eo = nullptr, *y = nullptr, *ei = nullptr;
      B2(m.upT(in0, ni, &x, off)); B2(m.upT(in1, no, &eo, off)); B2(m.dev(no, ts, &y, off)); B2(m.dev(ni, ts, &ei, off)); B2(poison(y, ts * no)); B2(poison(ei, ts * ni));
      k_upsample_fwd(prec, x, y, o->N, o->H, o->W, o->C, f, s); ran();
      k_upsample_bwd(prec, eo, ei, o->N, o->H, o->W, o->C, f, s); ran();
      B2(m.downT(out0, y, no)); B2(m.downT(out1, ei, ni));
      break;
    }
    case B2G_EW_SUMSQ: {
      if (!in0 || o->n < 1 || o->n_seg < 1 || !o->seg_off || !o->seg_len || !o->seg_coef) return fail(B2G_ERR_ARG, "bad SUMSQ arguments");
      for (int i = 0; i < o->n_seg; ++i)
        if (o->seg_off[i] < 0 || o->seg_len[i] < 0 || o->seg_off[i] + o->seg_len[i] > o->n) return fail(B2G_ERR_ARG, "segment %d outside the tensor", i);
      float *p = nullptr, *coef = nullptr; int64_t *so = nullptr, *sl = nullptr; double* res = nullptr;
      B2(m.upF(in0, (size_t)o->n, &p, off)); B2(m.upF(o->seg_coef, (size_t)o->n_seg, &coef, off)); B2(m.dev((size_t)o->n_seg, 8, (void**)&so, off)); B2(m.dev((size_t)o->n_seg, 8, (void**)&sl, off)); B2(m.dev(1, 8, (void**)&res, off));
      CU(cudaMemcpyAsync(so, o->seg_off, 8 * (size_t)o->n_seg, cudaMemcpyHostToDevice, s)); CU(cudaMemcpyAsync(sl, o->seg_len, 8 * (size_t)o->n_seg, cudaMemcpyHostToDevice, s));
      B2(poison(res, 8));
      k_sumsq_segments(p, so, sl, coef, o->n_seg, res, s); ran();
      CU(cudaMemcpyAsync(&o->sumsq, res, 8, cudaMemcpyDeviceToHost, s));
      break;
    }
    default: return fail(B2G_ERR_ARG, "unknown op %d", o->op);
  }
  CU(cudaStreamSynchronize(s)); CHECK_KERNELS();
  strncpy(o->kernel, names.c_str(), sizeof(o->kernel) - 1); o->kernel[sizeof(o->kernel) - 1] = 0;
  return 0;
}
extern "C" int32_t b2g_test_ew(b2g_ctx* c, int32_t precision, b2g_test_ew_opts* o, const float* in0, const float* in1, float* out0, float* out1, float* out2) {
  return test_ew_impl(c, precision, o, nullptr, in0, in1, out0, out1, out2);
}
extern "C" int32_t b2g_test_pool(b2g_ctx* c, int32_t precision, b2g_test_pool_opts* po, const float* in0, const float* in1, float* out0, float* out1, float* out2) {
  if (!c || !po) return fail(B2G_ERR_ARG, "null");
  if (po->op != B2G_TEST_POOL2D && po->op != B2G_TEST_GLOBAL_POOL) return fail(B2G_ERR_ARG, "unknown pooling op %d", po->op);
  b2g_test_ew_opts o{};
  o.op = po->op == B2G_TEST_POOL2D ? EW_POOL2D : EW_GLOBAL_POOL;
  o.N = po->N; o.H = po->H; o.W = po->W; o.C = po->C; o.KH = po->KH; o.KW = po->KW; o.SH = po->SH; o.SW = po->SW;
  o.offset = po->offset; o.poison = po->poison;
  po->splits = 1;
  B2(test_ew_impl(c, precision, &o, po, in0, in1, out0, out1, out2));
  memcpy(po->kernel, o.kernel, sizeof(po->kernel));
  return 0;
}

extern "C" int32_t b2g_test_net_shadow(b2g_net* n, int32_t layer, int32_t which, float* out, int64_t count) {
  if (!n || !out) return fail(B2G_ERR_ARG, "null");
  if (layer < 0 || layer >= (int)n->L.size()) return fail(B2G_ERR_ARG, "layer %d out of range", layer);
  if (n->prec != PREC_BF16) return fail(B2G_ERR_UNSUPPORTED, "FP32 nets keep no bf16 weight copies");
  const LayerRT& l = n->L[layer];
  int64_t off = -1, len = 0;
  if (which == 0) { off = l.off_W_bf; len = l.n_W; }
  else if (which == 1) { off = l.off_Wps_bf; len = (int64_t)k_tc_deconv_ps_weight_elems(l.geom); }
  else return fail(B2G_ERR_ARG, "which = %d (0 straight copy, 1 pixel-shuffle operand)", which);
  if (off < 0) return fail(B2G_ERR_UNSUPPORTED, "layer %d has no %s", layer, which ? "pixel-shuffle operand" : "bf16 weight copy");
  if (count != len) return fail(B2G_ERR_SHAPE, "layer %d operand has %lld elements, %lld requested", layer, (long long)len, (long long)count);
  CU(cudaSetDevice(n->ctx->device)); cudaStream_t s = n->ctx->stream;
  if ((size_t)len > n->stage_floats) return fail(B2G_ERR_SHAPE, "operand larger than the staging buffer");
  k_nhwc_to_nchw_f32(PREC_BF16, n->shadow + off, n->stage_f32, 1, 1, (int)len, s);
  CU(cudaMemcpyAsync(out, n->stage_f32, sizeof(float) * len, cudaMemcpyDeviceToHost, s)); CU(cudaStreamSynchronize(s)); CHECK_KERNELS();
  return 0;
}

extern "C" int32_t b2g_test_hbm_kernels(b2g_net* n, int32_t rows, int32_t channels, int32_t iters, float* ms3) {
  if (!n || !ms3 || rows < 8 || iters < 1) return fail(B2G_ERR_ARG, "bad arguments"); b2g_ctx* c = n->ctx; CU(cudaSetDevice(c->device)); cudaStream_t s = c->stream;
  if (!k_bn_vec_ok(PREC_BF16, channels)) return fail(B2G_ERR_UNSUPPORTED, "channels %d not supported by the vector BatchNorm kernels", channels);
  const size_t ne = (size_t)rows * channels; __nv_bfloat16 *x = nullptr, *e = nullptr, *y = nullptr; float *coef = nullptr, *gb = nullptr; unsigned long long* acc = nullptr;
  HookMem m(s, PREC_BF16);
  B2(m.dev(ne, 2, (void**)&x)); B2(m.dev(ne, 2, (void**)&e)); B2(m.dev(ne, 2, (void**)&y)); B2(m.upF(nullptr, 4 * (size_t)channels, &coef)); B2(m.upF(nullptr, 4 * (size_t)channels, &gb));
  B2(m.dev(k_bn_acc_elems(channels, 1), 8, (void**)&acc));
  CU(cudaMemsetAsync(x, 0x3c, 2 * ne, s)); CU(cudaMemsetAsync(e, 0x3c, 2 * ne, s)); CU(cudaMemsetAsync(acc, 0, 8 * k_bn_acc_elems(channels, 1), s)); k_fill_f32(coef, 1.0f, 4 * channels, s); k_fill_f32(gb, 1.0f, 4 * channels, s);
  cudaEvent_t e0, e1; B2(m.event(&e0)); B2(m.event(&e1));
  ms3[0] = ms3[1] = ms3[2] = 0.f;
  for (int which = 0; which < 3; ++which) for (int it = -1; it < iters; ++it) {
    B2(b2g_flush_l2(c));
    CU(cudaEventRecord(e0, s));
    if (which == 0) k_updater(n->params, n->grads, n->st0, n->st1, n->st2, n->segs_dev, n->chunk_seg_dev, n->chunk_off_dev, n->nchunks, 1.0f, 1.0f, n->step_dev, n->upd_ticket,
                              n->shadow, nullptr, nullptr, nullptr, n->upd_ext, s);
    else if (which == 1) k_bn_apply_acc(x, y, rows, channels, 1, acc, gb, gb + channels, ACT_LRELU, 0.2f, 1e-5f, coef, gb + 2 * channels, gb + 3 * channels, nullptr, nullptr, 0.9f, s);
    else k_bn_bwd_apply_acc(x, e, y, rows, channels, 1, coef, ACT_LRELU, 0.2f, 1, acc, gb, gb + channels, 0, s);
    CU(cudaEventRecord(e1, s)); CU(cudaEventSynchronize(e1));
    float ms = 0.f; CU(cudaEventElapsedTime(&ms, e0, e1)); if (it >= 0) ms3[which] += ms / iters;
  }
  CHECK_KERNELS();
  return 0;
}
```

gan_deeplearning4j_b200/csrc/kernels.h:

```cpp
#pragma once
#include <cuda_runtime.h>
#include <cuda_bf16.h>
#include <stdint.h>

namespace b2g {

enum Prec { PREC_F32 = 0, PREC_BF16 = 1 };
enum Act { ACT_IDENTITY = 0, ACT_TANH = 1, ACT_SIGMOID = 2, ACT_RELU = 3, ACT_LRELU = 4,
           ACT_ELU = 5, ACT_SELU = 6, ACT_SOFTPLUS = 7, ACT_SOFTSIGN = 8, ACT_HARDTANH = 9, ACT_HARDSIGMOID = 10, ACT_RELU6 = 11, ACT_SWISH = 12,
           ACT_CUBE = 13, ACT_RATIONALTANH = 14, ACT_RECTIFIEDTANH = 15, ACT_THRESHOLDEDRELU = 16, ACT_EXT_FIRST = ACT_ELU, ACT_EXT_LAST = ACT_THRESHOLDEDRELU };
enum Loss { LOSS_MSE = 2, LOSS_L1 = 3, LOSS_L2 = 4, LOSS_MAE = 5, LOSS_HINGE = 6, LOSS_SQUARED_HINGE = 7, LOSS_WASSERSTEIN = 8 };

inline size_t prec_size(int prec) { return prec == PREC_F32 ? 4 : 2; }

struct ConvGeom {
  int N, H, W, C;
  int OH, OW, O;
  int KH, KW, SH, SW, PH, PW;
};

extern uint64_t g_launch_count;
extern const char* g_ew_last_kernel;
int device_sm_count();

// ... 19 lines not shown
void k_bn_stats_acc(const void* x, int rows_per_group, int C, int groups, unsigned long long* acc, cudaStream_t s);
void k_bn_apply_acc(const void* x, void* y, int rows_per_group, int C, int groups, const unsigned long long* acc, const float* gamma, const float* beta,
                    int act, float alpha, float eps, float* coef, const float* run_mean, const float* run_var, float* g_mean, float* g_var, float decay, cudaStream_t s, int replicas = 1);
void k_bn_bwd_stats_acc(const void* x, const void* eps_out, int rows_per_group, int C, int groups, const float* coef, int act, float alpha, unsigned long long* acc, cudaStream_t s);
void k_bn_bwd_apply_acc(const void* x, const void* eps_out, void* eps_in, int rows_per_group, int C, int groups, const float* coef, int act, float alpha, int premul,
                        const unsigned long long* acc, float* g_gamma, float* g_beta, int want_param_grads, cudaStream_t s, int replicas = 1);

void k_act_fwd(int prec, const void* x, void* y, size_t n, int act, float alpha, cudaStream_t s);
void k_act_bwd_from_output(int prec, const void* a, const void* eps_out, void* eps_in, size_t n, int act, float alpha, cudaStream_t s);
bool act_ext_kind(int act);
void k_act_ext_fwd(int prec, int act, float alpha, const void* z, void* a, size_t n, cudaStream_t s);
void k_act_ext_bwd(int prec, int act, float alpha, const void* z, void* eps, size_t n, cudaStream_t s);
void k_maxpool_fwd(int prec, const void* x, void* y, uint8_t* argmax, int N, int H, int W, int C, int OH, int OW, int KH, int KW, int SH, int SW, cudaStream_t s);
void k_maxpool_bwd(int prec, const void* eps_out, const uint8_t* argmax, void* eps_in, int N, int H, int W, int C, int OH, int OW, int KH, int KW, int SH, int SW, cudaStream_t s);
void k_upsample_fwd(int prec, const void* x, void* y, int N, int H, int W, int C, int f, cudaStream_t s);
void k_upsample_bwd(int prec, const void* eps_out, void* eps_in, int N, int H, int W, int C, int f, cudaStream_t s);

enum Pool { POOL_MAX = 0, POOL_AVG = 1, POOL_SUM = 2, POOL_PNORM = 3 };
void k_pool2d_fwd(int prec, int kind, int pn, const void* x, void* y, int N, int H, int W, int C, int OH, int OW, int KH, int KW, int SH, int SW, int PH, int PW,
                  cudaStream_t s);
void k_pool2d_bwd(int prec, int kind, int pn, const void* eps_out, const void* x, const void* y, void* eps_in, int N, int H, int W, int C, int OH, int OW, int KH,
                  int KW, int SH, int SW, int PH, int PW, cudaStream_t s);
int k_global_pool_splits(int prec, int N, int HW, int C, int vec);
size_t k_global_pool_partial_elems(int prec, int max_rows, int HW, int C);
void k_global_pool_fwd(int prec, int kind, int pn, const void* x, void* y, int32_t* idx, int N, int HW, int C, float* part, int32_t* part_idx, unsigned* ticket,
                       cudaStream_t s);
void k_global_pool_bwd(int prec, int kind, int pn, const void* eps_out, const void* x, const void* y, const int32_t* idx, void* eps_in, int N, int HW, int C,
                       cudaStream_t s);
extern int g_pool_last_splits;

struct DropoutArgs { uint64_t seed; uint32_t tag; uint32_t threshold; float scale; int keep_all; };
void k_dropout_fwd(int prec, const void* x, void* y, uint32_t* mask, size_t n, const DropoutArgs& a, unsigned long long* pass, unsigned* ticket, int bump_pass, cudaStream_t s);
void k_dropout_bwd(int prec, const void* eps_out, void* eps_in, const uint32_t* mask, size_t n, float scale, cudaStream_t s);

void k_xent(int prec, const void* z, const float* y, void* dz, float* loss_sums, int rows_per_group, int groups, float clip_eps, cudaStream_t s);
void k_sigmoid_out(int prec, const void* z, void* p, size_t n, cudaStream_t s);
void k_softmax_xent(int prec, const void* z, const float* y, void* dz, void* p_out, float* loss_sums, int rows, int K, cudaStream_t s);
int k_loss_blocks(size_t n_per_group, int groups);
void k_loss(int prec, int loss, int act, float alpha, const void* z, const float* y, void* dz, float* loss_sums, int rows_per_group, int n_out, int groups,
            double* partial, unsigned* ticket, cudaStream_t s);
void k_cnn_xent(int prec, const void* z, const float* y, void* dz, float* loss_sums, size_t n_per_group, int groups, float clip_eps, double* partial,
                unsigned* ticket, cudaStream_t s);
int k_cnn_softmax_blocks(int rows_per_group, int groups);
void k_cnn_softmax_xent(int prec, const void* z, const float* y, void* dz, void* p_out, float* loss_sums, int rows_per_group, int C, int groups,
                        double* partial, unsigned* ticket, cudaStream_t s);

enum VertexOp { VERTEX_ADD = 0, VERTEX_SUBTRACT = 1, VERTEX_PRODUCT = 2, VERTEX_AVERAGE = 3, VERTEX_MAX = 4 };
void k_vertex_ew_fwd(int prec, int op, const void* a, const void* b, void* y, size_t n, cudaStream_t s);
void k_vertex_ew_bwd(int prec, int op, int order, void* eps, const void* spine, const void* skip, float* acc, int accumulate, size_t n, cudaStream_t s);
void k_merge_fwd(int prec, const void* a, const void* b, void* y, size_t P, int Ca, int Cb, cudaStream_t s);
void k_merge_bwd(int prec, const void* eps, void* dst, float* acc, size_t P, int Ca, int Cb, int spine_first, int accumulate, cudaStream_t s);
void k_skip_add(int prec, void* eps, const float* acc, size_t n, cudaStream_t s);

void k_colsum(int prec, const void* x, int rows, int C, float* scratch, float* out, int accumulate, cudaStream_t s);
size_t k_colsum_scratch_floats(int C);
void k_sumsq_segments(const float* p, const int64_t* seg_off, const int64_t* seg_len, const float* seg_coef, int nseg, double* out, cudaStream_t s);
void k_reduce_splits(const float* src, float* dst, size_t n, int splits, size_t stride, int accumulate, cudaStream_t s);
struct ReduceJob { const float* src; float* dst; int64_t n, stride; int splits, blocks; };
struct ReduceList { static const int MAX_JOBS = 24; ReduceJob jobs[MAX_JOBS]; int count; };
void reduce_list_push(ReduceList* rl, const float* src, float* dst, int64_t n, int splits, int64_t stride);
void k_reduce_multi(const ReduceList& rl, cudaStream_t s);

struct UpdSeg {
  int64_t off, len;
  int kind;
  float lr, b1, b2, eps;
  float l2;
  float clip;
  int div_mb;
  int64_t off_bf, off_ps;
  int ps_O, ps_C;
};
__device__ __forceinline__ void upd_shadow(const UpdSeg& sg, __nv_bfloat16* __restrict__ shadow, int64_t i, __nv_bfloat16 pb) {
  shadow[sg.off_bf + (i - sg.off)] = pb;
  if (sg.off_ps >= 0) {
    const int e = (int)(i - sg.off), c = e % sg.ps_C, tap = (e / sg.ps_C) % 16, o = e / (sg.ps_C * 16), r = tap >> 2, sx = tap & 3;
    const int py = (r == 0 || r == 2) ? 1 : 0, dyr = r == 3 ? -1 : r == 0 ? 1 : 0, px = (sx == 0 || sx == 2) ? 1 : 0, dxc = sx == 3 ? -1 : sx == 0 ? 1 : 0;
    shadow[sg.off_ps + ((int64_t)((py * 8 + px * 4 + c) * 9 + (dyr + 1) * 3 + (dxc + 1))) * sg.ps_O + o] = pb;
  }
}
struct UpdSched {
  int kind, type;
  int n_map;
  double initial, gamma, power, step, decay;
  const int32_t* keys; const double* vals;
};
void k_updater(float* params, const float* grads, float* st0, float* st1, float* st2, const UpdSeg* segs_dev, const int32_t* chunk_seg_dev,
               const int64_t* chunk_off_dev, int nchunks, float inv_mb, float inv_world, int* step_dev , unsigned* ticket,
               __nv_bfloat16* shadow, const float* gn_mult, const UpdSched* sched, const int64_t* epoch_dev, bool ext, cudaStream_t s);
void k_sched_lr(const UpdSeg* segs_dev, const UpdSched* sched, int seg, const int* step_dev, const int64_t* epoch_dev, float* out, cudaStream_t s);
static const int UPD_CHUNK = 4096;

struct GnGroup { int32_t chunk_begin, chunk_end, seg_begin, seg_end; };
void k_gradnorm(const float* grads, const UpdSeg* segs_dev, const int32_t* chunk_seg_dev, const int64_t* chunk_off_dev, int nchunks,
                const GnGroup* groups_dev, int ngroups, int clip, float threshold, float inv_mb, float inv_world, double* partial, unsigned* ticket,
                float* mult, cudaStream_t s);
enum { CON_ONEPASS = 0, CON_TWOPASS = 1, CON_ELEMWISE = 2 };
static const int CON_CHUNK = 4096, CON_SCHUNK = 256;
struct ConJob {
  UpdSeg sg;
  int kind, path;
  double max_norm, min_norm, rate;
  int K0, R0, K1, R1, K2, groups, R;
  int blk_begin, blocks, blk2_begin, blocks2, chunks;
  int64_t part_begin, mult_begin;
};
void k_constraint_onepass(float* params, __nv_bfloat16* shadow, const ConJob* jobs, int j0, int j1, int blocks, cudaStream_t s);
void k_constraint_twopass(float* params, __nv_bfloat16* shadow, const ConJob* jobs, int j0, int j1, int norm_blocks, int scale_blocks, double* partial,
                          unsigned* ticket, float* mult, cudaStream_t s);
void k_fill_f32(float* p, float v, size_t n, cudaStream_t s);
void k_scale_f32(float* p, float v, size_t n, cudaStream_t s);
struct P2pArgs { float* grads[8]; unsigned* flags[8]; int rank, world; size_t n; unsigned* state; };
void k_p2p_allreduce(const P2pArgs& a, cudaStream_t s);

void k_simt_fprop(int prec, int wprec, const ConvGeom& g, const void* x, const void* w, const float* bias, void* out, int act, float alpha, cudaStream_t s, const float* scale = nullptr);
void k_simt_dgrad(int prec, int wprec, const ConvGeom& g, const void* dy, const void* w, const float* bias, void* dx, int act, float alpha, cudaStream_t s, const float* scale = nullptr);
void k_simt_wgrad(int prec, const ConvGeom& g, const void* x, const void* dy, float* dw, float* scratch, size_t scratch_floats, int accumulate, cudaStream_t s);
size_t k_simt_wgrad_scratch_floats(const ConvGeom& g);
extern const char* g_gemm_last_kernel;
extern int g_gemm_last_splits;

bool edge_deconv_small_c_supported(const ConvGeom& g);
bool edge_conv_small_cin_supported(const ConvGeom& g);
bool edge_wgrad_small_cin_supported(const ConvGeom& g);
bool dense_small_o_supported(const ConvGeom& g);
void k_edge_deconv_small_c(int prec, int wprec, const ConvGeom& g, const void* dy, const void* w, const float* bias, void* dx, int act, float alpha, cudaStream_t s);
void k_edge_conv_small_cin(int prec, int wprec, const ConvGeom& g, const void* x, const void* w, const float* bias, void* out, int act, float alpha, cudaStream_t s);
void k_edge_wgrad_small_cin(int prec, const ConvGeom& g, const void* x, const void* dy, float* dw, float* scratch, int accumulate, cudaStream_t s);
size_t k_edge_wgrad_scratch_floats(const ConvGeom& g);
void k_dense_small_o_fwd(int prec, int wprec, const ConvGeom& g, const void* x, const void* w, const float* bias, void* out, int act, float alpha, cudaStream_t s);
void k_dense_small_o_dgrad(int prec, int wprec, const ConvGeom& g, const void* dy, const void* w, void* dx, cudaStream_t s);
void k_dense_small_o_wgrad(int prec, const ConvGeom& g, const void* x, const void* dy, float* dw, float* scratch, int accumulate, cudaStream_t s);
size_t k_dense_small_o_wgrad_scratch_floats(const ConvGeom& g);
bool dense_small_k_supported(const ConvGeom& g);
void k_dense_small_k_dgrad(int prec, int wprec, const ConvGeom& g, const void* dy, const void* w, const float* bias, void* dx, int act, float alpha, cudaStream_t s);
void k_dense_small_k_wgrad(int prec, const ConvGeom& g, const void* x, const void* dy, float* dw, cudaStream_t s);

bool head_conv_supported(const ConvGeom& g);
size_t k_head_wgrad_scratch_floats(const ConvGeom& g);
void k_head_fwd(const ConvGeom& g, const __nv_bfloat16* x, const __nv_bfloat16* w, const float* bias, __nv_bfloat16* out, int act, float alpha, cudaStream_t s);
void k_head_dgrad(const ConvGeom& g, const __nv_bfloat16* dy, const __nv_bfloat16* w, const float* bias, __nv_bfloat16* dx, int act, float alpha, cudaStream_t s);
int k_head_wgrad(const ConvGeom& g, const __nv_bfloat16* x, const __nv_bfloat16* dy, float* dw, float* part, size_t part_floats, int force_splits, cudaStream_t s,
                 ReduceList* defer);

bool tc_fprop_supported(const ConvGeom& g);
bool tc_dgrad_supported(const ConvGeom& g);
bool tc_wgrad_supported(const ConvGeom& g);
int  tc_init();
extern const char* g_tc_last_kernel;
extern int g_tc_test_bn, g_tc_test_max_ctas;
extern int g_tc_test_per_tap;
extern bool g_tc_last_slab;
extern int g_tc_test_splits, g_tc_last_splits;
enum { EPI_PLAIN = 0, EPI_STATS = 1, EPI_BNBWD = 2, EPI_ACTBWD = 3 };
struct TcEpi {
  int mode;
  const float* scale;
  unsigned long long* acc;
  int imgs_per_group;
  const __nv_bfloat16* aux;
  const __nv_bfloat16* aux2;
  int act; float alpha;
};
int k_tc_fprop(const ConvGeom& g, const __nv_bfloat16* x, const __nv_bfloat16* w, const float* bias, __nv_bfloat16* out, int act, float alpha, cudaStream_t s, const TcEpi* epi = nullptr, int w_mn = 0);
int k_tc_dgrad(const ConvGeom& g, const __nv_bfloat16* dy, const __nv_bfloat16* w, const float* bias, __nv_bfloat16* dx, int act, float alpha, cudaStream_t s, const TcEpi* epi = nullptr);
int k_tc_wgrad(const ConvGeom& g, const __nv_bfloat16* x, const __nv_bfloat16* dy, float* dw, float* scratch, size_t scratch_floats, int accumulate, cudaStream_t s, ReduceList* defer = nullptr);
size_t k_tc_wgrad_scratch_floats(const ConvGeom& g);
bool tc_deconv_ps_shape(const ConvGeom& g);
bool tc_deconv_ps_supported(const ConvGeom& g);
size_t k_tc_deconv_ps_weight_elems(const ConvGeom& g);
void k_pack_deconv_ps(const float* w, __nv_bfloat16* wps, int O, int C, cudaStream_t s);
bool tc_edge_conv_supported(const ConvGeom& g);
bool tc_edge_wgrad_supported(const ConvGeom& g);
size_t k_tc_edge_wgrad_scratch_floats(const ConvGeom& g);
int k_tc_edge_conv(const ConvGeom& g, const __nv_bfloat16* x, const __nv_bfloat16* w, const float* bias, __nv_bfloat16* out, int act, float alpha, cudaStream_t s);
int k_tc_edge_wgrad(const ConvGeom& g, const __nv_bfloat16* x, const __nv_bfloat16* dy, float* dw, float* db, float* scratch, size_t scratch_floats, int accumulate, cudaStream_t s, ReduceList* defer = nullptr);
int k_tc_deconv_ps(const ConvGeom& g, const __nv_bfloat16* dy, const __nv_bfloat16* wps, const float* bias, __nv_bfloat16* dx, int act, float alpha, cudaStream_t s, const TcEpi* epi = nullptr);

}
```

gan_deeplearning4j_b200/csrc/kernels_tc.cu:

```cuda
#include <cuda.h>
#include <stdio.h>
#include <stdlib.h>
#include <algorithm>

#include "common.cuh"
#include "kernels.h"

namespace b2g {

typedef CUresult (*PFN_encodeTiled)(CUtensorMap*, CUtensorMapDataType, cuuint32_t, void*, const cuuint64_t*, const cuuint64_t*, const cuuint32_t*,
                                    const cuuint32_t*, CUtensorMapInterleave, CUtensorMapSwizzle, CUtensorMapL2promotion, CUtensorMapFloatOOBfill);
static PFN_encodeTiled g_encode = nullptr;

int tc_init() {
  if (g_encode) return 0;
  void* fn = nullptr; cudaDriverEntryPointQueryResult q;
  if (cudaGetDriverEntryPoint("cuTensorMapEncodeTiled", &fn, cudaEnableDefault, &q) != cudaSuccess || !fn || q != cudaDriverEntryPointSuccess) return -1;
  g_encode = (PFN_encodeTiled)fn; return 0;
}

static int make_map_bf16(CUtensorMap* m, const void* base, int rank, const cuuint64_t* dims, const cuuint64_t* strides_bytes, const cuuint32_t* box, const cuuint32_t* estr) {
  if (!g_encode) return -1;
  CUresult r = g_encode(m, CU_TENSOR_MAP_DATA_TYPE_BFLOAT16, (cuuint32_t)rank, const_cast<void*>(base), dims, strides_bytes, box, estr, CU_TENSOR_MAP_INTERLEAVE_NONE,
                        CU_TENSOR_MAP_SWIZZLE_128B, CU_TENSOR_MAP_L2_PROMOTION_L2_256B, CU_TENSOR_MAP_FLOAT_OOB_FILL_NONE);
// ... 317 lines not shown
  const uint32_t bar_empty = bar_full + 8 * STAGES;
  const uint32_t park_full = bar_empty + 8 * STAGES;
  const uint32_t park_empty = park_full + 8 * S::PARKS;
  float* sst = reinterpret_cast<float*>(smem_gen + S::STAT_OFF);
  const int warp = threadIdx.x >> 5, lane = threadIdx.x & 31;
  const int num_kb = p.taps_h * p.taps_w * p.chunks;
  const int tiles = p.tiles_m * p.tiles_n * p.phases;
  auto tile_coords = [&](int t, int& nb0, int& phase, int& n0, int& y0) {
    const int mt = t % p.tiles_m, r = t / p.tiles_m;
    nb0 = (r % p.tiles_n) * BN; phase = r / p.tiles_n;
    if (p.Nt > 1) { n0 = mt * p.Nt; y0 = 0; } else { n0 = mt / p.tiles_y; y0 = (mt % p.tiles_y) * p.Ht; }
  };

  if (threadIdx.x == 0) {
    prefetch_map(&tmA); prefetch_map(&tmB);
    for (int s = 0; s < STAGES; ++s) { mbar_init(bar_full + 8 * s, 1); mbar_init(bar_empty + 8 * s, 8); }
    for (int k = 0; k < S::PARKS; ++k) { mbar_init(park_full + 8 * k, 256); mbar_init(park_empty + 8 * k, 256); }
    fence_mbar_init();
  }
  __syncthreads();
  pdl_wait();

  if (warp >= 16) {
    setmaxnreg_dec<R::PRODUCER>();
    if (warp == 16) {
      int s = 0; uint32_t ph = 0;
      for (int t = blockIdx.x; t < tiles; t += gridDim.x) {
        int nb0, phase, n0, y0; tile_coords(t, nb0, phase, n0, y0);
        const int py = phase >> 1, px = phase & 1;
        const int ybase = p.mode == 0 ? y0 * p.SH : y0;
        int ch = 0, ta = 0, tb = 0;
        int ax, dy_, wtap, wtap2 = 0;
        auto coords = [&]() { if constexpr (SLAB) slab_coords(p, ta, tb, py, px, ax, dy_, wtap, wtap2); else tap_coords(p, ta, tb, py, px, ax, dy_, wtap); };
        coords();
        for (int kb = 0; kb < num_kb; ++kb) {
          mbar_wait(bar_empty + 8 * s, ph ^ 1);
          if (elect_one_sync()) {
            const uint32_t st = smem_base + s * S::STAGE_BYTES;
            mbar_expect_tx(bar_full + 8 * s, SLAB ? p.slab_bytes + S::B_BYTES : S::STAGE_BYTES);
            tma_load_4d(st, &tmA, bar_full + 8 * s, ch * 64, ax, ybase + dy_, n0);
            load_b_tile<BN>(p, &tmB, st + S::A_BYTES, bar_full + 8 * s, ch, wtap, nb0);
            if constexpr (SLAB) load_b_tile<BN>(p, &tmB, st + S::A_BYTES + BN * 128, bar_full + 8 * s, ch, wtap2, nb0);
          }
          __syncwarp();
          if (++s == STAGES) { s = 0; ph ^= 1; }
          if (++ch == p.chunks) { ch = 0; if (++tb == p.taps_w) { tb = 0; ++ta; } coords(); }
        }
      }
    }
  } else if (warp < 8) {
    if constexpr (R::MMA < R::LAUNCH) setmaxnreg_dec<R::MMA>();
    const int wg = warp >> 2;
    const int r0 = wg * 64 + (warp & 3) * 16 + (lane >> 2);
    int s = 0, k = 0; uint32_t ph = 0, kph = 0;
    for (int t = blockIdx.x; t < tiles; t += gridDim.x) {
      float acc[NB][NACC];
#pragma unroll
      for (int nb = 0; nb < NB; ++nb)
#pragma unroll
        for (int j = 0; j < NACC; ++j) acc[nb][j] = 0.f;
      int prev = -1;
      for (int kb = 0; kb < num_kb; ++kb) {
        mbar_wait(bar_full + 8 * s, ph);
        wg_fence();
        const uint32_t st = smem_base + s * S::STAGE_BYTES;
        if constexpr (SLAB) {
          const uint32_t a = st + wg * p.a_wg_bytes;
          mma_kblock<BN, NB, NACC>(acc, a, st + S::A_BYTES, p.b_mn);
          mma_kblock<BN, NB, NACC>(acc, a + p.a_tap_bytes, st + S::A_BYTES + BN * 128, p.b_mn);
        } else {
          mma_kblock<BN, NB, NACC>(acc, st + wg * 8192, st + S::A_BYTES, PS ? 0 : p.b_mn);
        }
        wg_commit();
        wg_wait<1>();
        if (prev >= 0 && lane == 0) mbar_arrive(bar_empty + 8 * prev);
        prev = s;
        if (++s == STAGES) { s = 0; ph ^= 1; }
      }
      wg_wait<0>();
      if (lane == 0) mbar_arrive(bar_empty + 8 * prev);
      mbar_wait(park_empty + 8 * k, kph ^ 1);
      float* park = reinterpret_cast<float*>(smem_gen + S::PARK_OFF + k * S::PARK_BYTES);
#pragma unroll
      for (int nb = 0; nb < NB; ++nb)
#pragma unroll
        for (int j = 0; j < NACC / 4; ++j) {
          const int col = nb * 64 + j * 8 + 2 * (lane & 3);
          *reinterpret_cast<float2*>(park + r0 * S::ACC_PITCH + col) = make_float2(acc[nb][4 * j], acc[nb][4 * j + 1]);
          *reinterpret_cast<float2*>(park + (r0 + 8) * S::ACC_PITCH + col) = make_float2(acc[nb][4 * j + 2], acc[nb][4 * j + 3]);
        }
      mbar_arrive(park_full + 8 * k);
      if (++k == S::PARKS) { k = 0; kph ^= 1; }
    }
  } else {
    setmaxnreg_inc<R::EPI>();
    const int ew = warp - 8, q = ew & 3, half = ew >> 2;
    const int row = q * 32 + lane;
    const int img = row / (p.Ht * p.Wt), rem = row % (p.Ht * p.Wt), yy = rem / p.Wt, xx = rem % p.Wt;
    int k = 0; uint32_t kph = 0;
    for (int t = blockIdx.x; t < tiles; t += gridDim.x) {
      int nb0, phase, n0, y0; tile_coords(t, nb0, phase, n0, y0);
      const int py = phase >> 1, px = phase & 1;
      const int n = n0 + img, gy = y0 + yy, gx = xx;
      mbar_wait(park_full + 8 * k, kph);
      const float* srow = reinterpret_cast<const float*>(smem_gen + S::PARK_OFF + k * S::PARK_BYTES) + row * S::ACC_PITCH;
      if constexpr (PS) {
        if (half == 0) {
          const int C = p.OC;
#pragma unroll
          for (int ppy = 0; ppy < 2; ++ppy) {
            const size_t doff = (((size_t)n * p.outH + 2 * gy + ppy) * p.outW + 2 * gx) * C;
            __nv_bfloat16* dst = p.out + doff;
            float o[8];
#pragma unroll
            for (int ppx = 0; ppx < 2; ++ppx)
#pragma unroll
              for (int c = 0; c < 4; ++c) {
                float a = srow[(ppy * 2 + ppx) * 4 + c];
                if constexpr (EPI == EPI_ACTBWD) { if (c < C) a *= act_grad_from_out(p.act, __bfloat162float(p.aux[doff + ppx * C + c]), p.alpha); }
                else { if (p.bias && c < C) a += p.bias[c]; a = act_fwd(p.act, a, p.alpha); }
                o[ppx * 4 + c] = a;
              }
            if (C == 3) {
              __nv_bfloat162 h0 = __floats2bfloat162_rn(o[0], o[1]), h1 = __floats2bfloat162_rn(o[2], o[4]), h2 = __floats2bfloat162_rn(o[5], o[6]);
              uint32_t* d32 = reinterpret_cast<uint32_t*>(dst);
              d32[0] = *reinterpret_cast<uint32_t*>(&h0); d32[1] = *reinterpret_cast<uint32_t*>(&h1); d32[2] = *reinterpret_cast<uint32_t*>(&h2);
            } else {
#pragma unroll
              for (int ppx = 0; ppx < 2; ++ppx)
#pragma unroll
                for (int c = 0; c < 4; ++c) if (c < C) dst[ppx * C + c] = __float2bfloat16(o[ppx * 4 + c]);
            }
          }
        }
      } else {
        size_t pix;
        if (p.mode == 0) pix = ((size_t)n * p.outH + gy) * p.outW + gx;
        else pix = ((size_t)n * p.outH + 2 * gy + py) * p.outW + 2 * gx + px;
        const int group = p.imgs_per_group > 0 ? n0 / p.imgs_per_group : 0;
        epi_tile<BN, EPI, AFFINE>(p, srow, pix * p.OC + nb0, nb0, group, sst, reinterpret_cast<uint4*>(smem_gen + S::STG_OFF) + ew * 128, q, lane,
                                  (int)threadIdx.x - 256, half * (BN / 2), (half + 1) * (BN / 2));
        if constexpr (EPI == EPI_STATS || EPI == EPI_BNBWD) epi_bar_sync();
      }
      mbar_arrive(park_empty + 8 * k);
      if (++k == S::PARKS) { k = 0; kph ^= 1; }
    }
  }
}

const char* g_tc_last_kernel = "";
bool g_tc_last_slab = false;
int g_tc_test_bn = 0, g_tc_test_max_ctas = 0, g_tc_test_per_tap = 0, g_tc_test_splits = 0;
int g_tc_last_splits = 0;
static int tc_device() { int dev = 0; cudaGetDevice(&dev); return dev < 0 || dev >= 64 ? 0 : dev; }
#define TC_SET_SMEM_ONCE(kernel, bytes)                                                                                            \
  do { static bool set_[64] = {}; const int d_ = tc_device();                                                                       \
       if (!set_[d_]) { if (cudaFuncSetAttribute(kernel, cudaFuncAttributeMaxDynamicSharedMemorySize, (int)(bytes)) != cudaSuccess) return -2; set_[d_] = true; } } while (0)

static bool pick_row_tile(int N, int GH, int GW, int rows, int* Nt, int* Ht, int* Wt) {
  const int P = GH * GW;
  if (GW > rows || rows % GW) return false;
  if (P >= rows) { if (P % rows) return false; *Nt = 1; *Ht = rows / GW; *Wt = GW; return GH % *Ht == 0; }
  if (rows % P || N % (rows / P)) return false;
  *Nt = rows / P; *Ht = GH; *Wt = GW; return true;
}
static int pick_bn(int OC) { return OC % 128 == 0 ? 128 : OC % 64 == 0 ? 64 : 0; }
static int pick_bn_fill(int OC, long m_tiles_x_phases) {
  if (g_tc_test_bn) return g_tc_test_bn;
  const int target = device_sm_count();
  int bn = pick_bn(OC);
  while (bn > 64 && m_tiles_x_phases * (OC / bn) < target) bn /= 2;
  return bn;
}

bool tc_fprop_supported(const ConvGeom& g) {
  int a, b, c;
  return g.C % 64 == 0 && pick_bn(g.O) != 0 && g.SH >= 1 && g.SH <= 2 && g.SW == g.SH && g.KH * g.KW * (g.C / 64) >= 1 &&
         pick_row_tile(g.N, g.OH, g.OW, 128, &a, &b, &c) && c * g.SW <= 256 && b * g.SH <= 256 && g.N >= 1;
}
bool tc_dgrad_supported(const ConvGeom& g) {
  int a, b, c;
  return g.KH == 4 && g.KW == 4 && g.SH == 2 && g.SW == 2 && g.PH == 1 && g.PW == 1 && g.O % 64 == 0 && pick_bn(g.C) != 0 && g.H == 2 * g.OH && g.W == 2 * g.OW &&
         pick_row_tile(g.N, g.OH, g.OW, 128, &a, &b, &c);
}
static bool tc_epi_ok(const TcEpi* e, int Nt) { return !e || e->mode == EPI_PLAIN || e->mode == EPI_ACTBWD || (e->imgs_per_group > 0 && e->imgs_per_group % Nt == 0 && e->acc); }

template <int BN, int STAGES, int EPI, bool AFFINE, bool PS = false, bool SLAB = false>
static int launch_conv_e(const CUtensorMap& tmA, const CUtensorMap& tmB, const TcConvParams& p, cudaStream_t s) {
  using S = TcSmem<BN, STAGES, EPI, SLAB>;
  TC_SET_SMEM_ONCE((tc_conv_kernel<BN, STAGES, EPI, AFFINE, PS, SLAB>), S::TOTAL);
  const long tiles = (long)p.tiles_m * p.tiles_n * p.phases;
  const unsigned grid = (unsigned)std::min<long>(tiles, g_tc_test_max_ctas > 0 ? g_tc_test_max_ctas : device_sm_count());
  launch_pdl(tc_conv_kernel<BN, STAGES, EPI, AFFINE, PS, SLAB>, dim3(grid), dim3(TC_CONV_THREADS), (size_t)(S::TOTAL), s, tmA, tmB, p);
  LAUNCHED();
  return cudaPeekAtLastError() == cudaSuccess ? 0 : -3;
}
template <int BN, int STAGES, bool SLAB>
static int launch_conv(const CUtensorMap& tmA, const CUtensorMap& tmB, const TcConvParams& p, cudaStream_t s, const char* name) {
  g_tc_last_kernel = name; g_tc_last_slab = SLAB;
  switch (p.epi) {
    case EPI_STATS: return launch_conv_e<BN, STAGES, EPI_STATS, false, false, SLAB>(tmA, tmB, p, s);
    case EPI_BNBWD: return launch_conv_e<BN, STAGES, EPI_BNBWD, false, false, SLAB>(tmA, tmB, p, s);
    case EPI_ACTBWD: return launch_conv_e<BN, STAGES, EPI_ACTBWD, false, false, SLAB>(tmA, tmB, p, s);
  }
  return (p.scale && p.bias) ? launch_conv_e<BN, STAGES, EPI_PLAIN, true, false, SLAB>(tmA, tmB, p, s) : launch_conv_e<BN, STAGES, EPI_PLAIN, false, false, SLAB>(tmA, tmB, p, s);
}
static int dispatch_conv(int BN, bool slab, const CUtensorMap& tmA, const CUtensorMap& tmB, const TcConvParams& p, cudaStream_t s) {
  switch (BN * 2 + slab) {
    case 128: return launch_conv<64, 4, false>(tmA, tmB, p, s, "tc_conv_kernel<64,4>");
    case 256: return launch_conv<128, 4, false>(tmA, tmB, p, s, "tc_conv_kernel<128,4>");
    case 129: return launch_conv<64, 4, true>(tmA, tmB, p, s, "tc_conv_kernel<64,4>");
  }
  return -4;
}
static bool slab_tile(const TcConvParams& p, int BN) {
  if (g_tc_test_per_tap || BN != 64 || p.Wt % 8) return false;
  if (!((p.Nt == 1 && p.Ht >= 2) || (p.Nt == 2 && p.Ht * p.Wt == 64))) return false;
  return p.Nt * (p.Ht + 1) * p.Wt <= SLAB_ROWS;
}
static bool is_k4s2p1_geom(const ConvGeom& g) { return g.KH == 4 && g.KW == 4 && g.SH == 2 && g.SW == 2 && g.PH == 1 && g.PW == 1 && g.H == 2 * g.OH && g.W == 2 * g.OW; }
static void set_slab(TcConvParams& p) {
  p.taps_h = p.mode == 0 ? 2 : 1;
  p.slab_bytes = p.Nt * (p.Ht + 1) * p.Wt * 128;
  p.a_wg_bytes = p.Nt == 1 ? 64 * 128 : (p.Ht + 1) * p.Wt * 128;
  p.a_tap_bytes = p.Wt * 128;
}

static int weight_map(CUtensorMap* m, const __nv_bfloat16* w, int rows, int taps, int inner, int box_rows) {
  cuuint64_t dims[3] = {(cuuint64_t)inner, (cuuint64_t)taps, (cuuint64_t)rows};
  cuuint64_t strides[2] = {(cuuint64_t)inner * 2, (cuuint64_t)taps * inner * 2};
  cuuint32_t box[3] = {64, 1, (cuuint32_t)box_rows}; cuuint32_t es[3] = {1, 1, 1};
  return make_map_bf16(m, w, 3, dims, strides, box, es);
}
static void fill_epi(TcConvParams& p, const float* bias, int act, float alpha, const TcEpi* e) {
  p.bias = bias; p.act = act; p.alpha = alpha; p.epi = EPI_PLAIN;
  if (!e) return;
  p.scale = e->scale; p.epi = e->mode; p.acc = e->acc; p.imgs_per_group = e->mode == EPI_STATS || e->mode == EPI_BNBWD ? e->imgs_per_group : 0;
  p.aux = e->aux; p.aux2 = e->aux2;
  if (e->mode == EPI_BNBWD || e->mode == EPI_ACTBWD) { p.act = e->act; p.alpha = e->alpha; p.bias = nullptr; p.scale = nullptr; }
}

int k_tc_fprop(const ConvGeom& g, const __nv_bfloat16* x, const __nv_bfloat16* w, const float* bias, __nv_bfloat16* out, int act, float alpha, cudaStream_t s, const TcEpi* epi, int w_mn) {
  TcConvParams p{}; p.mode = 0;
  if (!pick_row_tile(g.N, g.OH, g.OW, 128, &p.Nt, &p.Ht, &p.Wt) || !tc_epi_ok(epi, p.Nt)) return -1;
  if (w_mn && (g.KH != 1 || g.KW != 1)) return -1;
  const int BN = pick_bn_fill(g.O, (long)g.N * g.OH * g.OW / 128);
  p.GH = g.OH; p.GW = g.OW; p.tiles_y = g.OH / p.Ht; p.taps_h = g.KH; p.taps_w = g.KW; p.chunks = g.C / 64; p.KW = g.KW;
  p.SH = g.SH; p.SW = g.SW; p.PH = g.PH; p.PW = g.PW; p.OC = g.O; p.outH = g.OH; p.outW = g.OW; p.out = out; p.b_mn = w_mn;
  fill_epi(p, bias, act, alpha, epi);
  const bool slab = is_k4s2p1_geom(g) && !w_mn && slab_tile(p, BN);
  if (slab) set_slab(p);
  CUtensorMap tmA, tmB;
  cuuint64_t dims[4] = {(cuuint64_t)g.C, (cuuint64_t)g.W, (cuuint64_t)g.H, (cuuint64_t)g.N};
  cuuint64_t strides[3] = {(cuuint64_t)g.C * 2, (cuuint64_t)g.W * g.C * 2, (cuuint64_t)g.H * g.W * g.C * 2};
  cuuint32_t box[4] = {64, (cuuint32_t)(p.Wt * g.SW), (cuuint32_t)((p.Ht + slab) * g.SH), (cuuint32_t)p.Nt};
  cuuint32_t es[4] = {1, (cuuint32_t)g.SW, (cuuint32_t)g.SH, 1};
  if (make_map_bf16(&tmA, x, 4, dims, strides, box, es)) return -1;
  p.tiles_m = g.N * g.OH * g.OW / 128; p.tiles_n = g.O / BN; p.phases = 1;
  if (w_mn ? weight_map(&tmB, w, g.C, 1, g.O, 64) : weight_map(&tmB, w, g.O, g.KH * g.KW, g.C, BN)) return -1;
  return dispatch_conv(BN, slab, tmA, tmB, p, s);
}

int k_tc_dgrad(const ConvGeom& g, const __nv_bfloat16* dy, const __nv_bfloat16* w, const float* bias, __nv_bfloat16* dx, int act, float alpha, cudaStream_t s, const TcEpi* epi) {
  TcConvParams p{}; p.mode = 1;
  if (!pick_row_tile(g.N, g.OH, g.OW, 128, &p.Nt, &p.Ht, &p.Wt) || !tc_epi_ok(epi, p.Nt)) return -1;
  const int BN = pick_bn_fill(g.C, (long)g.N * g.OH * g.OW / 128 * 4);
  p.GH = g.OH; p.GW = g.OW; p.tiles_y = g.OH / p.Ht; p.taps_h = 2; p.taps_w = 2; p.chunks = g.O / 64; p.KW = 4;
  p.SH = 1; p.SW = 1; p.PH = 0; p.PW = 0; p.OC = g.C; p.outH = g.H; p.outW = g.W; p.out = dx; p.b_mn = 1;
  fill_epi(p, bias, act, alpha, epi);
  const bool slab = slab_tile(p, BN);
  if (slab) set_slab(p);
  CUtensorMap tmA, tmB;
  cuuint64_t dims[4] = {(cuuint64_t)g.O, (cuuint64_t)g.OW, (cuuint64_t)g.OH, (cuuint64_t)g.N};
  cuuint64_t strides[3] = {(cuuint64_t)g.O * 2, (cuuint64_t)g.OW * g.O * 2, (cuuint64_t)g.OH * g.OW * g.O * 2};
  cuuint32_t box[4] = {64, (cuuint32_t)p.Wt, (cuuint32_t)(p.Ht + slab), (cuuint32_t)p.Nt};
  cuuint32_t es[4] = {1, 1, 1, 1};
  if (weight_map(&tmB, w, g.O, 16, g.C, 64)) return -1;
  if (make_map_bf16(&tmA, dy, 4, dims, strides, box, es)) return -1;
  p.tiles_m = g.N * g.OH * g.OW / 128; p.tiles_n = g.C / BN; p.phases = 4;
  return dispatch_conv(BN, slab, tmA, tmB, p, s);
}

bool tc_deconv_ps_shape(const ConvGeom& g) { return is_k4s2p1_geom(g) && g.C >= 1 && g.C <= 4 && g.O % 64 == 0; }
bool tc_deconv_ps_supported(const ConvGeom& g) { int a, b, c; return tc_deconv_ps_shape(g) && pick_row_tile(g.N, g.OH, g.OW, 128, &a, &b, &c); }
size_t k_tc_deconv_ps_weight_elems(const ConvGeom& g) { return tc_deconv_ps_shape(g) ? (size_t)16 * 9 * g.O : 0; }
__global__ void pack_deconv_ps_kernel(const float* __restrict__ w, __nv_bfloat16* __restrict__ wps, int O, int C) { pdl_wait();
  const int idx = blockIdx.x * blockDim.x + threadIdx.x; if (idx >= 16 * 9 * O) return;
  const int o = idx % O, t = (idx / O) % 9, n = idx / (9 * O);
  const int py = n >> 3, px = (n >> 2) & 1, c = n & 3, dyr = t / 3 - 1, dxc = t % 3 - 1;
  const int r = dyr == -1 ? (py == 0 ? 3 : -1) : dyr == 0 ? (py == 0 ? 1 : 2) : (py == 1 ? 0 : -1);
  const int sx = dxc == -1 ? (px == 0 ? 3 : -1) : dxc == 0 ? (px == 0 ? 1 : 2) : (px == 1 ? 0 : -1);
  wps[idx] = __float2bfloat16((r >= 0 && sx >= 0 && c < C) ? w[((size_t)o * 16 + r * 4 + sx) * C + c] : 0.f);
}
void k_pack_deconv_ps(const float* w, __nv_bfloat16* wps, int O, int C, cudaStream_t s) {
  launch_pdl(pack_deconv_ps_kernel, dim3((16 * 9 * O + 255) / 256), dim3(256), (size_t)(0), s, w, wps, O, C); LAUNCHED();
}
int k_tc_deconv_ps(const ConvGeom& g, const __nv_bfloat16* dy, const __nv_bfloat16* wps, const float* bias, __nv_bfloat16* dx, int act, float alpha, cudaStream_t s, const TcEpi* epi) {
  TcConvParams p{}; p.mode = 0;
  if (!tc_deconv_ps_shape(g) || !pick_row_tile(g.N, g.OH, g.OW, 128, &p.Nt, &p.Ht, &p.Wt)) return -1;
  if (epi && epi->mode != EPI_PLAIN && epi->mode != EPI_ACTBWD) return -1;
  p.GH = g.OH; p.GW = g.OW; p.tiles_y = g.OH / p.Ht; p.taps_h = 3; p.taps_w = 3; p.chunks = g.O / 64; p.KW = 3;
  p.SH = 1; p.SW = 1; p.PH = 1; p.PW = 1; p.OC = g.C; p.outH = g.H; p.outW = g.W; p.out = dx;
  fill_epi(p, bias, act, alpha, epi);
  CUtensorMap tmA, tmB;
  cuuint64_t dims[4] = {(cuuint64_t)g.O, (cuuint64_t)g.OW, (cuuint64_t)g.OH, (cuuint64_t)g.N};
  cuuint64_t strides[3] = {(cuuint64_t)g.O * 2, (cuuint64_t)g.OW * g.O * 2, (cuuint64_t)g.OH * g.OW * g.O * 2};
  cuuint32_t box[4] = {64, (cuuint32_t)p.Wt, (cuuint32_t)p.Ht, (cuuint32_t)p.Nt}; cuuint32_t es[4] = {1, 1, 1, 1};
  if (make_map_bf16(&tmA, dy, 4, dims, strides, box, es)) return -1;
  if (weight_map(&tmB, wps, 16, 9, g.O, 16)) return -1;
  p.tiles_m = (int)((long)g.N * g.OH * g.OW / 128); p.tiles_n = 1; p.phases = 1;
  g_tc_last_kernel = "tc_conv_kernel<16,4,PS>";
  return p.epi == EPI_ACTBWD ? launch_conv_e<16, 4, EPI_ACTBWD, false, true>(tmA, tmB, p, s) : launch_conv_e<16, 4, EPI_PLAIN, false, true>(tmA, tmB, p, s);
}

struct TcEdgeParams {
  const __nv_bfloat16* x; const __nv_bfloat16* w; const __nv_bfloat16* dy; const float* bias; __nv_bfloat16* out; float* part; float* part_b;
  int N, H, W, C, OH, OW, O, Ht, tiles_y, tiles_total, tiles_per_cta, act; float alpha;
};
static constexpr int EDGE_SLAB_BYTES = 6144;
__device__ __forceinline__ uint32_t swz128(int row, int byte) { return (uint32_t)(row * 128 + ((((byte >> 4) ^ (row & 7)) << 4) | (byte & 15))); }

struct EdgeSlabRegs { uint4 v[3]; };
__device__ __forceinline__ void edge_fetch_slab(const TcEdgeParams& p, int n, int oy0, EdgeSlabRegs& r) {
  const int WC = p.W * p.C, cpr = WC >> 3, total = (2 * p.Ht + 2) * cpr;
#pragma unroll
  for (int q = 0; q < 3; ++q) {
    const int i = threadIdx.x + q * 128; r.v[q] = make_uint4(0u, 0u, 0u, 0u);
    if (i < total) { const int j = i / cpr, cc = i - j * cpr, iy = 2 * oy0 - 1 + j;
      if (iy >= 0 && iy < p.H) r.v[q] = __ldg(reinterpret_cast<const uint4*>(p.x + ((size_t)n * p.H + iy) * WC) + cc); }
  }
}
__device__ __forceinline__ void edge_store_slab(const TcEdgeParams& p, const EdgeSlabRegs& r, uint8_t* slab) {
  const int total = (2 * p.Ht + 2) * ((p.W * p.C) >> 3);
#pragma unroll
  for (int q = 0; q < 3; ++q) { const int i = threadIdx.x + q * 128; if (i < total) reinterpret_cast<uint4*>(slab)[i] = r.v[q]; }
}
template <int C>
__device__ __forceinline__ void edge_build_row_c(const TcEdgeParams& p, const uint8_t* slab, uint8_t* tile, int row, bool ones) {
  const int WC = p.W * C, oy_l = row / p.OW, ox = row - oy_l * p.OW;
  const int lo = ox == 0 ? C : 0, hi = ox == p.OW - 1 ? 3 * C : 4 * C;
  uint32_t out[32];
#pragma unroll
  for (int i = 0; i < 32; ++i) out[i] = 0u;
#pragma unroll
  for (int r = 0; r < 4; ++r) {
    const int b0 = ((2 * oy_l + r) * WC + (2 * ox - 1) * C) * 2;
    if (C & 1) {
      const uint32_t* wp = reinterpret_cast<const uint32_t*>(slab + b0 - 2);
      uint32_t w[2 * C + 1];
#pragma unroll
      for (int i = 0; i <= 2 * C; ++i) w[i] = wp[i];
#pragma unroll
      for (int i = 0; i < 2 * C; ++i) out[r * 2 * C + i] = __funnelshift_r(w[i], w[i + 1], 16);
    } else {
      const uint32_t* wp = reinterpret_cast<const uint32_t*>(slab + b0);
#pragma unroll
      for (int i = 0; i < 2 * C; ++i) out[r * 2 * C + i] = wp[i];
    }
#pragma unroll
    for (int i = 0; i < 2 * C; ++i) {
      const uint32_t m = ((2 * i >= lo && 2 * i < hi) ? 0xFFFFu : 0u) | ((2 * i + 1 >= lo && 2 * i + 1 < hi) ? 0xFFFF0000u : 0u);
      out[r * 2 * C + i] &= m;
    }
  }
  if (C < 4 && ones) out[8 * C] = 0x3F80u;
#pragma unroll
  for (int cc = 0; cc < 8; ++cc) *reinterpret_cast<uint4*>(tile + row * 128 + ((cc ^ (row & 7)) << 4)) = make_uint4(out[4 * cc], out[4 * cc + 1], out[4 * cc + 2], out[4 * cc + 3]);
}
__device__ __forceinline__ void edge_build_row(const TcEdgeParams& p, const uint8_t* slab, uint8_t* tile, int row, bool ones = false) {
  switch (p.C) { case 1: edge_build_row_c<1>(p, slab, tile, row, ones); break; case 2: edge_build_row_c<2>(p, slab, tile, row, ones); break;
                 case 3: edge_build_row_c<3>(p, slab, tile, row, ones); break; default: edge_build_row_c<4>(p, slab, tile, row, ones); break; }
}


__global__ void __launch_bounds__(128) tc_edge_conv_kernel(const TcEdgeParams p) { pdl_wait();
  extern __shared__ uint8_t smem_raw[];
  const uint32_t smem_base = (smem_u32(smem_raw) + 1023u) & ~1023u;
  uint8_t* sm = smem_raw + (smem_base - smem_u32(smem_raw));
  uint8_t* sA = sm; uint8_t* sB = sm + 16384; uint8_t* slab = sm + 24576;
  const int tid = threadIdx.x, warp = tid >> 5, lane = tid & 31;
  const int nb0 = blockIdx.y * 64, K = 16 * p.C;
  const int t_beg = blockIdx.x * p.tiles_per_cta, t_end = min(p.tiles_total, t_beg + p.tiles_per_cta);
  EdgeSlabRegs pre;
  if (t_beg < t_end) edge_fetch_slab(p, t_beg / p.tiles_y, (t_beg % p.tiles_y) * p.Ht, pre);
  {
    uint4 wv[4];
#pragma unroll
    for (int q = 0; q < 4; ++q) { const int i = tid + q * 128, o = i >> 3, cc = i & 7;
      wv[q] = cc < 2 * p.C ? __ldg(reinterpret_cast<const uint4*>(p.w + (size_t)(nb0 + o) * K) + cc) : make_uint4(0u, 0u, 0u, 0u); }
#pragma unroll
    for (int q = 0; q < 4; ++q) { const int i = tid + q * 128, o = i >> 3, cc = i & 7; *reinterpret_cast<uint4*>(sB + o * 128 + ((cc ^ (o & 7)) << 4)) = wv[q]; }
  }
  const bool has_bias = p.bias != nullptr;
  const int r0 = warp * 16 + (lane >> 2), cq = lane & 3;
  for (int t = t_beg; t < t_end; ++t) {
    const int n = t / p.tiles_y, oy0 = (t % p.tiles_y) * p.Ht;
    edge_store_slab(p, pre, slab);
    __syncthreads();
    if (t + 1 < t_end) edge_fetch_slab(p, (t + 1) / p.tiles_y, ((t + 1) % p.tiles_y) * p.Ht, pre);
    edge_build_row(p, slab, sA, tid);
    fence_proxy_async_smem();
    __syncthreads();
    float acc[2][32];
#pragma unroll
    for (int h = 0; h < 2; ++h)
#pragma unroll
      for (int j = 0; j < 32; ++j) acc[h][j] = 0.f;
    wg_fence();
    {
      const uint64_t bdesc = desc_kmajor_sw128(smem_base + 16384);
#pragma unroll
      for (int k = 0; k < 4; ++k)
#pragma unroll
        for (int h = 0; h < 2; ++h) wgmma_n64<0, 0>(acc[h], desc_kmajor_sw128(smem_base + h * 8192) + 2 * k, bdesc + 2 * k);
    }
    wg_commit();
    wg_wait<0>();
    __syncthreads();
#pragma unroll
    for (int h = 0; h < 2; ++h)
#pragma unroll
      for (int i = 0; i < 2; ++i) {
        const int row = h * 64 + r0 + 8 * i;
#pragma unroll
        for (int j = 0; j < 8; ++j) {
          const int col = j * 8 + 2 * cq;
          float a = acc[h][4 * j + 2 * i], b = acc[h][4 * j + 2 * i + 1];
          if (has_bias) { a += p.bias[nb0 + col]; b += p.bias[nb0 + col + 1]; }
          __nv_bfloat162 v = __floats2bfloat162_rn(act_fwd(p.act, a, p.alpha), act_fwd(p.act, b, p.alpha));
          *reinterpret_cast<__nv_bfloat162*>(sA + row * 128 + ((j ^ (row & 7)) << 4) + cq * 4) = v;
        }
      }
    __syncthreads();
    __nv_bfloat16* obase = p.out + ((size_t)n * p.OH + oy0) * p.OW * p.O + nb0;
#pragma unroll
    for (int i = 0; i < 8; ++i) {
      const int idx = tid + i * 128, r = idx >> 3, cc = idx & 7;
      *reinterpret_cast<uint4*>(obase + (size_t)r * p.O + cc * 8) = *reinterpret_cast<const uint4*>(sA + r * 128 + ((cc ^ (r & 7)) << 4));
    }
  }
}

__global__ void __launch_bounds__(128) tc_edge_wgrad_kernel(const TcEdgeParams p) { pdl_wait();
  extern __shared__ uint8_t smem_raw[];
  const uint32_t smem_base = (smem_u32(smem_raw) + 1023u) & ~1023u;
  uint8_t* sm = smem_raw + (smem_base - smem_u32(smem_raw));
  uint8_t* sDy = sm; uint8_t* sX = sm + 16384; uint8_t* slab = sm + 32768;
  const int tid = threadIdx.x, warp = tid >> 5, lane = tid & 31, K = 16 * p.C;
  const int t_beg = blockIdx.x * p.tiles_per_cta, t_end = min(p.tiles_total, t_beg + p.tiles_per_cta);
  float acc[32];
#pragma unroll
  for (int j = 0; j < 32; ++j) acc[j] = 0.f;
  EdgeSlabRegs pre; uint4 dyr[8];
  auto fetch = [&](int t) {
    const int n = t / p.tiles_y, oy0 = (t % p.tiles_y) * p.Ht;
    edge_fetch_slab(p, n, oy0, pre);
    const uint4* dyt = reinterpret_cast<const uint4*>(p.dy + (((size_t)n * p.OH + oy0) * p.OW) * 64);
#pragma unroll
    for (int i = 0; i < 8; ++i) dyr[i] = __ldg(dyt + tid + i * 128);
  };
  if (t_beg < t_end) fetch(t_beg);
  for (int t = t_beg; t < t_end; ++t) {
    edge_store_slab(p, pre, slab);
#pragma unroll
    for (int i = 0; i < 8; ++i) { const int idx = tid + i * 128, r = idx >> 3, cc = idx & 7; *reinterpret_cast<uint4*>(sDy + r * 128 + ((cc ^ (r & 7)) << 4)) = dyr[i]; }
    __syncthreads();
    if (t + 1 < t_end) fetch(t + 1);
    edge_build_row(p, slab, sX, tid, p.part_b != nullptr);
    fence_proxy_async_smem();
    __syncthreads();
    wg_fence();
#pragma unroll
    for (int k = 0; k < 8; ++k)
      wgmma_n64<1, 1>(acc, desc_mnmajor_sw128(smem_base + k * 2048, 8192), desc_mnmajor_sw128(smem_base + 16384 + k * 2048, 8192));
    wg_commit();
    wg_wait<0>();
    __syncthreads();
  }
#pragma unroll
  for (int i = 0; i < 2; ++i) {
    const int o = warp * 16 + (lane >> 2) + 8 * i;
    float* orow = p.part + ((size_t)blockIdx.x * 64 + o) * K;
#pragma unroll
    for (int j = 0; j < 8; ++j) {
      const int col = j * 8 + 2 * (lane & 3);
      if (col < K) *reinterpret_cast<float2*>(orow + col) = make_float2(acc[4 * j + 2 * i], acc[4 * j + 2 * i + 1]);
      else if (col == K && p.part_b) p.part_b[(size_t)blockIdx.x * 64 + o] = acc[4 * j + 2 * i];
    }
  }
}

static bool edge_tile(const ConvGeom& g, int* Ht) {
  if (!is_k4s2p1_geom(g) || g.C < 1 || g.C > 4 || g.OW > 128 || 128 % g.OW) return false;
  const int ht = 128 / g.OW;
  if (g.OH % ht || (g.W * g.C) % 8 || (2 * ht + 2) * g.W * g.C * 2 > EDGE_SLAB_BYTES) return false;
  *Ht = ht; return true;
}
bool tc_edge_conv_supported(const ConvGeom& g) { int ht; return edge_tile(g, &ht) && g.O % 64 == 0; }
bool tc_edge_wgrad_supported(const ConvGeom& g) { int ht; return edge_tile(g, &ht) && g.O == 64; }
static int tc_edge_wgrad_target() { return 2 * device_sm_count(); }
static int tc_edge_wgrad_ctas(const ConvGeom& g, int* tpc) {
  int ht = 1; edge_tile(g, &ht);
  const int tiles = g.N * (g.OH / ht), target = g_tc_test_splits > 0 ? g_tc_test_splits : tc_edge_wgrad_target();
  const int per = (tiles + target - 1) / target; *tpc = per < 1 ? 1 : per;
  return (tiles + *tpc - 1) / *tpc;
}
size_t k_tc_edge_wgrad_scratch_floats(const ConvGeom& g) { return tc_edge_wgrad_supported(g) ? (size_t)tc_edge_wgrad_target() * (64 * 16 * g.C + 64) : 0; }
int k_tc_edge_conv(const ConvGeom& g, const __nv_bfloat16* x, const __nv_bfloat16* w, const float* bias, __nv_bfloat16* out, int act, float alpha, cudaStream_t s) {
  TcEdgeParams p{}; if (!edge_tile(g, &p.Ht) || g.O % 64) return -1;
  if ((reinterpret_cast<uintptr_t>(x) & 15) || (reinterpret_cast<uintptr_t>(w) & 15) || (reinterpret_cast<uintptr_t>(out) & 15)) return -1;
  p.x = x; p.w = w; p.bias = bias; p.out = out; p.N = g.N; p.H = g.H; p.W = g.W; p.C = g.C; p.OH = g.OH; p.OW = g.OW; p.O = g.O; p.tiles_y = g.OH / p.Ht;
  p.tiles_total = g.N * p.tiles_y; p.act = act; p.alpha = alpha;
  const size_t smem = 1024 + 24576 + EDGE_SLAB_BYTES;
  TC_SET_SMEM_ONCE(tc_edge_conv_kernel, smem);
  const int target = g_tc_test_max_ctas > 0 ? g_tc_test_max_ctas : 8 * device_sm_count();
  p.tiles_per_cta = (p.tiles_total + target - 1) / target;
  launch_pdl(tc_edge_conv_kernel, dim3(dim3((unsigned)((p.tiles_total + p.tiles_per_cta - 1) / p.tiles_per_cta), (unsigned)(g.O / 64))), dim3(128), (size_t)(smem), s, p);
  LAUNCHED(); g_tc_last_kernel = "tc_edge_conv_kernel";
  return cudaPeekAtLastError() == cudaSuccess ? 0 : -3;
}
static void reduce_or_defer(ReduceList* defer, const float* src, float* dst, size_t n, int splits, size_t stride, int accumulate, cudaStream_t s);
int k_tc_edge_wgrad(const ConvGeom& g, const __nv_bfloat16* x, const __nv_bfloat16* dy, float* dw, float* db, float* scratch, size_t scratch_floats, int accumulate, cudaStream_t s, ReduceList* defer) {
  TcEdgeParams p{}; if (!edge_tile(g, &p.Ht) || g.O != 64) return -1;
  if ((reinterpret_cast<uintptr_t>(x) & 15) || (reinterpret_cast<uintptr_t>(dy) & 15)) return -1;
  p.x = x; p.dy = dy; p.part = scratch; p.N = g.N; p.H = g.H; p.W = g.W; p.C = g.C; p.OH = g.OH; p.OW = g.OW; p.O = g.O; p.tiles_y = g.OH / p.Ht;
  p.tiles_total = g.N * p.tiles_y;
  const int ctas = tc_edge_wgrad_ctas(g, &p.tiles_per_cta); const size_t n = (size_t)64 * 16 * g.C;
  if ((size_t)ctas * (n + 64) > scratch_floats) return -5;
  if (db && g.C < 4) p.part_b = scratch + (size_t)ctas * n;
  const size_t smem = 1024 + 32768 + EDGE_SLAB_BYTES;
  TC_SET_SMEM_ONCE(tc_edge_wgrad_kernel, smem);
  launch_pdl(tc_edge_wgrad_kernel, dim3(dim3((unsigned)ctas)), dim3(128), (size_t)(smem), s, p);
  LAUNCHED(); g_tc_last_kernel = "tc_edge_wgrad_kernel"; g_tc_last_splits = ctas;
  if (cudaPeekAtLastError() != cudaSuccess) return -3;
  reduce_or_defer(defer, scratch, dw, n, ctas, n, accumulate, s);
  if (p.part_b) reduce_or_defer(defer, p.part_b, db, 64, ctas, 64, accumulate, s);
  return p.part_b ? 1 : 0;
}

struct TcWgradParams {
  int Nt, Ht, Wt;
  int tiles_y;
  int KW, SH, SW, PH, PW;
  int taps, C;
  int kb_total, kb_per_split;
  float* out; size_t split_stride;
};

template <int BNW, int STAGES>
struct TcWgradSmem {
  static constexpr int A_BYTES = 2 * 64 * 128;
  static constexpr int B_BYTES = (BNW / 64) * 64 * 128;
  static constexpr int STAGE_BYTES = A_BYTES + B_BYTES;
  static constexpr int BAR_OFF = STAGES * STAGE_BYTES;
  static constexpr int TOTAL = BAR_OFF + 256 + 1024;
};

template <int BNW, int STAGES>
__global__ void __launch_bounds__(TC_THREADS, 1) tc_wgrad_kernel(const __grid_constant__ CUtensorMap tmDy, const __grid_constant__ CUtensorMap tmX, const TcWgradParams p) {
  using S = TcWgradSmem<BNW, STAGES>;
  constexpr int NB = BNW / 64;
  extern __shared__ uint8_t smem_raw[];
  const uint32_t smem_base = (smem_u32(smem_raw) + 1023u) & ~1023u;
  const uint32_t bar_full = smem_base + S::BAR_OFF, bar_empty = bar_full + 8 * STAGES;
  const int warp = threadIdx.x >> 5, lane = threadIdx.x & 31;
  const int split = blockIdx.x, col0 = blockIdx.y * BNW, o0 = blockIdx.z * 128;
  const int kb_beg = split * p.kb_per_split, kb_end = min(p.kb_total, kb_beg + p.kb_per_split);
  const int num_kb = max(0, kb_end - kb_beg);

  if (threadIdx.x == 0) {
    prefetch_map(&tmDy); prefetch_map(&tmX);
    for (int s = 0; s < STAGES; ++s) { mbar_init(bar_full + 8 * s, 1); mbar_init(bar_empty + 8 * s, 8); }
    fence_mbar_init();
  }
  __syncthreads();
  pdl_trigger();
  pdl_wait();

  if (warp == 0) {
    int xc[NB], xw[NB], xh[NB];
#pragma unroll
    for (int j = 0; j < NB; ++j) { const int col = col0 + j * 64, tap = col / p.C; xc[j] = col % p.C; xw[j] = -p.PW + tap % p.KW; xh[j] = -p.PH + tap / p.KW; }
    int n0, y0;
    if (p.Nt > 1) { n0 = kb_beg * p.Nt; y0 = 0; } else { n0 = kb_beg / p.tiles_y; y0 = (kb_beg % p.tiles_y) * p.Ht; }
    int s = 0; uint32_t ph = 0;
    for (int i = 0; i < num_kb; ++i) {
      const int kb = kb_beg + i;
      mbar_wait(bar_empty + 8 * s, ph ^ 1);
      if (elect_one_sync()) {
        mbar_expect_tx(bar_full + 8 * s, S::STAGE_BYTES);
        const uint32_t a = smem_base + s * S::STAGE_BYTES, b = a + S::A_BYTES;
        tma_load_2d(a, &tmDy, bar_full + 8 * s, o0, kb * 64);
        tma_load_2d(a + 8192, &tmDy, bar_full + 8 * s, o0 + 64, kb * 64);
#pragma unroll
        for (int j = 0; j < NB; ++j) tma_load_4d(b + j * 8192, &tmX, bar_full + 8 * s, xc[j], xw[j], y0 * p.SH + xh[j], n0);
      }
      __syncwarp();
      if (++s == STAGES) { s = 0; ph ^= 1; }
      if (p.Nt > 1) n0 += p.Nt; else { y0 += p.Ht; if (y0 >= p.tiles_y * p.Ht) { y0 = 0; ++n0; } }
    }
  } else if (warp >= 4) {
    const int wg = (warp >> 2) - 1;
    float acc[NB][32];
#pragma unroll
    for (int nb = 0; nb < NB; ++nb)
#pragma unroll
      for (int j = 0; j < 32; ++j) acc[nb][j] = 0.f;
    int s = 0, prev = -1; uint32_t ph = 0;
    for (int i = 0; i < num_kb; ++i) {
      mbar_wait(bar_full + 8 * s, ph);
      wg_fence();
      const uint32_t a = smem_base + s * S::STAGE_BYTES + wg * 8192, b = smem_base + s * S::STAGE_BYTES + S::A_BYTES;
#pragma unroll
      for (int k = 0; k < 4; ++k) {
        if constexpr (NB == 2) wgmma_n128<1, 1>(acc[0], acc[1], desc_mnmajor_sw128(a + k * 2048, 8192), desc_mnmajor_sw128(b + k * 2048, 8192));
        else wgmma_n64<1, 1>(acc[0], desc_mnmajor_sw128(a + k * 2048, 8192), desc_mnmajor_sw128(b + k * 2048, 8192));
      }
      wg_commit();
      wg_wait<1>();
      if (prev >= 0 && lane == 0) mbar_arrive(bar_empty + 8 * prev);
      prev = s;
      if (++s == STAGES) { s = 0; ph ^= 1; }
    }
    wg_wait<0>();
#pragma unroll
    for (int i = 0; i < 2; ++i) {
      const int o = o0 + wg * 64 + (warp & 3) * 16 + (lane >> 2) + 8 * i;
      float* orow = p.out + (size_t)split * p.split_stride + (size_t)o * p.taps * p.C + col0;
#pragma unroll
      for (int nb = 0; nb < NB; ++nb)
#pragma unroll
        for (int j = 0; j < 8; ++j)
          *reinterpret_cast<float2*>(orow + nb * 64 + j * 8 + 2 * (lane & 3)) = make_float2(acc[nb][4 * j + 2 * i], acc[nb][4 * j + 2 * i + 1]);
    }
  }
}

static int wgrad_bnw(const ConvGeom& g) { if (g.C % 64) return 0; const long cols = (long)g.KH * g.KW * g.C; return cols % 128 == 0 ? 128 : 64; }
static int wgrad_target() { return (2 * device_sm_count()) / 3; }
static int wgrad_splits_for(const ConvGeom& g, int o_tile) {
  const int bnw = wgrad_bnw(g); if (!bnw) return 1;
  long tiles = (long)(g.O / o_tile) * (g.KH * g.KW * g.C / bnw), kbt = (long)g.N * g.OH * g.OW / 64;
  long sp = wgrad_target() / tiles, cap = kbt / 8; if (cap < 1) cap = 1; if (sp > cap) sp = cap; if (sp < 1) sp = 1; return (int)sp;
}
static int tc_wgrad_splits(const ConvGeom& g) { return g_tc_test_splits > 0 ? g_tc_test_splits : wgrad_splits_for(g, 128); }
bool tc_wgrad_supported(const ConvGeom& g) {
  int a, b, c;
  return g.O % 128 == 0 && wgrad_bnw(g) != 0 && g.SH >= 1 && g.SH <= 2 && g.SW == g.SH && ((long)g.N * g.OH * g.OW) % 64 == 0 &&
         pick_row_tile(g.N, g.OH, g.OW, 64, &a, &b, &c) && c * g.SW <= 256 && b * g.SH <= 256;
}
size_t k_tc_wgrad_scratch_floats(const ConvGeom& g) {
  if (!tc_wgrad_supported(g)) return 0;
  return (size_t)wgrad_splits_for(g, 128) * g.O * g.KH * g.KW * g.C;
}

template <int BNW, int STAGES>
static int launch_wgrad(const CUtensorMap& tmDy, const CUtensorMap& tmX, const TcWgradParams& p, dim3 grid, cudaStream_t s, const char* name) {
  using S = TcWgradSmem<BNW, STAGES>;
  TC_SET_SMEM_ONCE((tc_wgrad_kernel<BNW, STAGES>), S::TOTAL);
  launch_pdl(tc_wgrad_kernel<BNW, STAGES>, dim3(grid), dim3(TC_THREADS), (size_t)(S::TOTAL), s, tmDy, tmX, p);
  LAUNCHED(); g_tc_last_kernel = name;
  return cudaPeekAtLastError() == cudaSuccess ? 0 : -3;
}

static void reduce_or_defer(ReduceList* defer, const float* src, float* dst, size_t n, int splits, size_t stride, int accumulate, cudaStream_t s) {
  if (defer && !accumulate && defer->count < ReduceList::MAX_JOBS) { reduce_list_push(defer, src, dst, (int64_t)n, splits, (int64_t)stride); return; }
  k_reduce_splits(src, dst, n, splits, stride, accumulate, s);
}

int k_tc_wgrad(const ConvGeom& g, const __nv_bfloat16* x, const __nv_bfloat16* dy, float* dw, float* scratch, size_t scratch_floats, int accumulate, cudaStream_t s, ReduceList* defer) {
  TcWgradParams p{};
  if (!pick_row_tile(g.N, g.OH, g.OW, 64, &p.Nt, &p.Ht, &p.Wt)) return -1;
  const int BNW = wgrad_bnw(g); const size_t n = (size_t)g.O * g.KH * g.KW * g.C;
  int splits = tc_wgrad_splits(g);
  if ((size_t)splits * n > scratch_floats) return -5;
  p.tiles_y = g.OH / p.Ht; p.KW = g.KW; p.SH = g.SH; p.SW = g.SW; p.PH = g.PH; p.PW = g.PW; p.taps = g.KH * g.KW; p.C = g.C;
  p.kb_total = (int)((long)g.N * g.OH * g.OW / 64); p.kb_per_split = (p.kb_total + splits - 1) / splits;
  p.out = scratch; p.split_stride = n;
  CUtensorMap tmDy, tmX;
  { cuuint64_t dims[2] = {(cuuint64_t)g.O, (cuuint64_t)g.N * g.OH * g.OW}; cuuint64_t strides[1] = {(cuuint64_t)g.O * 2};
    cuuint32_t box[2] = {64, 64}; cuuint32_t es[2] = {1, 1};
    if (make_map_bf16(&tmDy, dy, 2, dims, strides, box, es)) return -1; }
  { cuuint64_t dims[4] = {(cuuint64_t)g.C, (cuuint64_t)g.W, (cuuint64_t)g.H, (cuuint64_t)g.N};
    cuuint64_t strides[3] = {(cuuint64_t)g.C * 2, (cuuint64_t)g.W * g.C * 2, (cuuint64_t)g.H * g.W * g.C * 2};
    cuuint32_t box[4] = {64, (cuuint32_t)(p.Wt * g.SW), (cuuint32_t)(p.Ht * g.SH), (cuuint32_t)p.Nt}; cuuint32_t es[4] = {1, (cuuint32_t)g.SW, (cuuint32_t)g.SH, 1};
    if (make_map_bf16(&tmX, x, 4, dims, strides, box, es)) return -1; }
  dim3 grid((unsigned)splits, (unsigned)(p.taps * g.C / BNW), (unsigned)(g.O / 128));
  const int rc = BNW == 64 ? launch_wgrad<64, 4>(tmDy, tmX, p, grid, s, "tc_wgrad_kernel<64,4>") : launch_wgrad<128, 4>(tmDy, tmX, p, grid, s, "tc_wgrad_kernel<128,4>");
  if (rc) return rc;
  g_tc_last_splits = splits;
  reduce_or_defer(defer, scratch, dw, n, splits, n, accumulate, s);
  return 0;
}

}
```

gan_deeplearning4j_b200/engine.py:

```python
from __future__ import annotations

import copy
import ctypes as C
import math
from typing import Dict, List, Optional, Sequence

import numpy as np

from . import _lib
from ._lib import GanConfig, LayerDesc, LrSchedule, NetConfig, check

LAYER_TYPES = {"conv2d": 0, "deconv2d": 1, "batchnorm": 2, "dense": 3, "activation": 4, "maxpool": 5, "upsample2d": 6,
               "output": 7, "loss": 8, "ff_to_cnn": 9, "cnn_to_ff": 10, "dropout": 11, "subsampling": 12, "global_pooling": 13,
               "cnn_loss": 14, "elementwise": 15, "merge": 16}
ELEMENTWISE_OPS = {"add": 0, "subtract": 1, "product": 2, "average": 3, "max": 4}
VERTEX_TYPES = ("elementwise", "merge")
POOLINGS = {"max": 0, "avg": 1, "sum": 2, "pnorm": 3}
GLOBAL_PNORM_DEFAULT = 2
ACTS = {"identity": 0, "tanh": 1, "sigmoid": 2, "relu": 3, "lrelu": 4, "elu": 5, "selu": 6, "softplus": 7, "softsign": 8, "hardtanh": 9,
        "hardsigmoid": 10, "relu6": 11, "swish": 12, "cube": 13, "rationaltanh": 14, "rectifiedtanh": 15, "thresholdedrelu": 16}
ACT_ALPHA_DEFAULTS = {"elu": 1.0, "thresholdedrelu": 1.0}
LOSSES = {"xent": 0, "mcxent": 1, "mse": 2, "l1": 3, "l2": 4, "mae": 5, "hinge": 6, "squared_hinge": 7, "wasserstein": 8}
UPDATERS = {"sgd": 0, "rmsprop": 1, "adam": 2, "noop": 3, "nesterovs": 4, "adagrad": 5, "adamax": 6, "nadam": 7, "amsgrad": 8, "adadelta": 9}
NO_LR_UPDATERS = ("noop", "adadelta")
# ... 371 lines not shown

    def _push_constraints(self, spec: Dict, before: Dict[str, List[Dict]]):
        now = resolve_constraints(spec)
        for p in sorted(set(now) | set(before)):
            lst = now.get(p, [])
            arr = (_lib.Constraint * max(1, len(lst)))(*[constraint_struct(c) for c in lst])
            check(self.lib.b2g_net_set_constraints(self.h, spec["name"].encode(), p.encode(), arr, len(lst)))

    def set_constraints(self, constraints: Optional[Sequence[Dict]], layer: Optional[str] = None):
        for sp in self.specs:
            if (layer is not None and sp.get("name") != layer) or sp["type"] not in GEMM_TYPES + ("batchnorm",):
                continue
            before = resolve_constraints(sp)
            new = dict(sp, constraints=copy.deepcopy(list(constraints or [])))
            resolve_constraints(new)
            sp["constraints"] = new["constraints"]
            if not sp["constraints"]:
                del sp["constraints"]
            self._push_constraints(sp, before)
            if layer is not None:
                break

    def apply_constraints(self):
        check(self.lib.b2g_net_apply_constraints(self.h))

    def learning_rate(self, layer: str) -> float:
        v = C.c_float()
        check(self.lib.b2g_net_get_learning_rate(self.h, layer.encode(), C.byref(v)))
        return v.value

    def epoch(self) -> int:
        v = C.c_int64()
        check(self.lib.b2g_net_get_epoch(self.h, C.byref(v)))
        return v.value

    def set_epoch(self, epoch: int):
        check(self.lib.b2g_net_set_epoch(self.h, int(epoch)))

    def set_grad_allreduce(self, enabled: bool):
        check(self.lib.b2g_net_set_grad_allreduce(self.h, int(enabled)))

    def set_sync_bn(self, enabled: bool):
        check(self.lib.b2g_net_set_sync_bn(self.h, int(enabled)))

    def set_grad_payload_bf16(self, enabled: bool):
        check(self.lib.b2g_net_set_grad_payload_bf16(self.h, int(enabled)))

    def enable_p2p_allreduce(self) -> bool:
        out = C.c_int32(0)
        check(self.lib.b2g_net_enable_p2p_allreduce(self.h, C.byref(out)))
        return bool(out.value)

    def average_parameters(self):
        check(self.lib.b2g_net_average_parameters(self.h))

    def iteration(self) -> int:
        v = C.c_int64()
        check(self.lib.b2g_net_get_iteration(self.h, C.byref(v)))
        return v.value

    def set_iteration(self, it: int):
        check(self.lib.b2g_net_set_iteration(self.h, int(it)))

    def dropout_pass(self) -> int:
        v = C.c_int64()
        check(self.lib.b2g_net_get_dropout_pass(self.h, C.byref(v)))
        return v.value

    def set_dropout_pass(self, p: int):
        check(self.lib.b2g_net_set_dropout_pass(self.h, int(p)))

    def simt_gemm_calls(self) -> int:
        v = C.c_uint64()
        check(self.lib.b2g_net_simt_gemm_calls(self.h, C.byref(v)))
        return v.value

    def time_hbm_kernels(self, rows: int, channels: int, iters: int = 10):
        ms = np.zeros(3, np.float32)
        check(self.lib.b2g_test_hbm_kernels(self.h, rows, channels, iters, _fp(ms)))
        return [float(v) for v in ms]

    def weight_operand(self, layer: int, which: int, size: int) -> np.ndarray:
        out = np.empty(size, np.float32)
        check(self.lib.b2g_test_net_shadow(self.h, layer, which, _fp(out), out.size))
        return out

    def input_gradient(self, batch: int) -> np.ndarray:
        out = np.empty((batch, int(np.prod(self.input_shape))), np.float32)
        check(self.lib.b2g_net_get_input_gradient(self.h, batch, _fp(out)))
        return out

    def close(self):
        if self.h:
            self.lib.b2g_net_destroy(self.h)
            self.h = None


class Gan:

    def __init__(self, gen: Net, dis: Net, fake_bn_train: bool = False, use_cuda_graph: bool = True):
        self.gen, self.dis, self.lib = gen, dis, gen.lib
        cfg = GanConfig(int(fake_bn_train), int(use_cuda_graph))
        h = C.c_void_p()
        check(self.lib.b2g_gan_create(gen.h, dis.h, C.byref(cfg), C.byref(h)))
        self.h = h

    def _args(self, x_real, z_d, z_g, y_real, y_fake, y_gen):
        x = _f32(x_real)
        n, oe = x.shape[0], self.dis.out_elems
        ys = []
        for name, y in (("y_real", y_real), ("y_fake", y_fake), ("y_gen", y_gen)):
            y = _f32(y).reshape(n, -1)
            if y.shape[1] == 1 and oe > 1:
                y = np.ascontiguousarray(np.broadcast_to(y, (n, oe)))
            if y.shape[1] != oe:
                raise ValueError(f"{name}: {y.shape[1]} labels per example; the discriminator has {oe} outputs per example (or pass one per image)")
            ys.append(y)
        return [x, _f32(z_d), _f32(z_g)] + ys

    def step(self, x_real, z_d, z_g, y_real, y_fake, y_gen):
        a = self._args(x_real, z_d, z_g, y_real, y_fake, y_gen)
        losses = np.zeros(3, np.float32)
        check(self.lib.b2g_gan_step(self.h, *[_fp(v) for v in a], a[0].shape[0], _fp(losses)))
        return losses

    def step_ptr(self, ptrs, batch: int, losses: np.ndarray):
        args = [C.cast(C.c_void_p(p), C.POINTER(C.c_float)) for p in ptrs]
        check(self.lib.b2g_gan_step(self.h, *args, batch, _fp(losses)))

    def upload(self, x_real, z_d, z_g, y_real, y_fake, y_gen):
        a = self._args(x_real, z_d, z_g, y_real, y_fake, y_gen)
        check(self.lib.b2g_gan_upload(self.h, *[_fp(v) for v in a], a[0].shape[0]))
        self.gen.ctx.sync()

    def step_resident(self, batch: int):
        check(self.lib.b2g_gan_step_resident(self.h, batch))

    def losses(self) -> np.ndarray:
        out = np.zeros(3, np.float32)
        check(self.lib.b2g_gan_read_losses(self.h, _fp(out)))
        return out

    def last_step_ms(self) -> float:
        v = C.c_float()
        check(self.lib.b2g_gan_last_step_ms(self.h, C.byref(v)))
        return v.value

    def close(self):
        if self.h:
            self.lib.b2g_gan_destroy(self.h)
            self.h = None


def test_conv(ctx: Context, kind: int, impl: int, precision: int, geom: Dict[str, int], a, b, out_size: int, iters: int = 1):
    g = _lib.ConvGeom(**geom)
    a, b = _f32(a).ravel(), _f32(b).ravel()
    out = np.empty(out_size, np.float32)
    ms = C.c_float()
    check(ctx.lib.b2g_test_conv(ctx.h, kind, impl, precision, C.byref(g), _fp(a), _fp(b), _fp(out), iters, C.byref(ms)))
    return out, ms.value


EPI_PLAIN, EPI_STATS, EPI_BNBWD, EPI_ACTBWD = 0, 1, 2, 3


def test_conv_ex(ctx: Context, kind: int, geom: Dict[str, int], a, b, out_size: int, *, epi: int = 0, act: str = "identity", alpha: float = 0.0,
                 bias=None, scale=None, groups: int = 1, aux=None, aux2=None, iters: int = 1, impl: int = 1, bn: int = 0, max_ctas: int = 0,
                 poison: bool = False, w_mn: bool = False, per_tap: bool = False, info: Optional[dict] = None, defer: bool = False, db=None,
                 precision: int = BF16, param_offset: int = 0, splits: int = 0):
    g = _lib.ConvGeom(**geom)
    a, b = _f32(a).ravel(), _f32(b).ravel()
    out = np.empty(out_size, np.float32)
    oc = geom["o"] if kind == 0 else geom["c"]
    o = _lib.TestConvOpts()
    o.epi, o.act, o.alpha, o.groups = epi, ACTS[act], alpha, groups
    o.bn, o.max_ctas, o.poison, o.w_mn, o.per_tap, o.defer = bn, max_ctas, int(poison), int(w_mn), int(per_tap), int(defer)
    o.param_offset, o.splits = param_offset, splits
    if db is not None:
        assert db.dtype == np.float32 and db.flags.c_contiguous
        o.db = _fp(db)
    keep = []
    for name, v in (("bias", bias), ("scale", scale), ("aux", aux), ("aux2", aux2)):
        if v is not None:
            arr = _f32(v).ravel(); keep.append(arr); setattr(o, name, _fp(arr))
    stats = None
    if epi in (EPI_STATS, EPI_BNBWD):
        stats = np.zeros((groups, 2, oc), np.float64); o.stats = stats.ctypes.data_as(C.POINTER(C.c_double))
    ms = C.c_float()
    check(ctx.lib.b2g_test_conv_ex(ctx.h, kind, impl, precision, C.byref(g), _fp(a), _fp(b), _fp(out), iters, C.byref(ms), C.byref(o)))
    if info is not None:
        info["slab"], info["splits"] = bool(o.slab), o.splits
    return out, stats, o.kernel.decode(), ms.value


def test_bn(ctx: Context, precision: int, path: int, x, eps_out, gamma, beta, run_mean, run_var, *, act: str = "identity", alpha: float = 0.0,
            eps: float = 1e-5, decay: float = 0.9, g_gamma=None, g_beta=None, want_param_grads: bool = True):
    x, e = _f32(x), _f32(eps_out)
    groups, rows, ch = x.shape
    par = [_f32(v).ravel() for v in (gamma, beta, run_mean, run_var)]
    r = {k: np.empty(x.shape, np.float32) for k in ("y", "eps_in")}
    r["g_gamma"] = _f32(np.zeros(ch) if g_gamma is None else g_gamma).copy()
    r["g_beta"] = _f32(np.zeros(ch) if g_beta is None else g_beta).copy()
    r.update({k: np.empty(ch, np.float32) for k in ("g_mean", "g_var")})
    r.update({k: np.empty((groups, ch), np.float32) for k in ("mean", "invstd")})
    check(ctx.lib.b2g_test_bn(ctx.h, precision, path, groups, rows, ch, _fp(x), _fp(e), *[_fp(v) for v in par], ACTS[act], alpha, eps, decay,
                              int(want_param_grads), *[_fp(r[k]) for k in ("y", "eps_in", "g_gamma", "g_beta", "g_mean", "g_var", "mean", "invstd")]))
    return r


def test_dropout(ctx: Context, precision: int, x, dy, p: float, *, seed: int = 666, layer: int = 0, rank: int = 0, pass_: int = 0):
    x, e = _f32(x), _f32(dy)
    rows = x.shape[0]
    h, w, c = (x.shape[1:] if x.ndim == 4 else (1, 1, int(np.prod(x.shape[1:]))))
    y, dx = np.empty_like(x), np.empty_like(x)
    check(ctx.lib.b2g_test_dropout(ctx.h, precision, seed, layer, rank, pass_, rows, h, w, c, p, _fp(x), _fp(e), _fp(y), _fp(dx)))
    return y, dx


EW_OPS = {"reduce_splits": 0, "reduce_multi": 1, "colsum": 2, "xent": 3, "softmax_xent": 4, "act_fwd": 5, "act_bwd": 6, "maxpool": 7,
          "upsample": 8, "sumsq": 9, "loss": 10, "act_ext_fwd": 11, "act_ext_bwd": 12,
          "cnn_xent": 13, "cnn_softmax_xent": 14, "vertex_fwd": 15, "vertex_bwd": 16, "merge_fwd": 17, "merge_bwd": 18, "skip_add": 19}


def test_ew(ctx: Context, precision: int, op: str, in0, in1=None, out_sizes=(0, 0, 0), *, act: str = "identity", jobs=None, segments=None,
            loss: str = "xent", **opts):
    o = _lib.TestEwOpts()
    o.op, o.act, o.loss = EW_OPS[op], ELEMENTWISE_OPS[act] if op in ("vertex_fwd", "vertex_bwd") else ACTS[act], LOSSES[loss]
    for k, v in opts.items():
        setattr(o, k, int(v) if isinstance(v, bool) else v)
    keep = []
    if jobs is not None:
        arr = (_lib.EwReduceJob * len(jobs))(*[_lib.EwReduceJob(j["n"], j["stride"], j["src_off"], j["dst_off"], j["splits"], 0) for j in jobs])
        o.n_jobs, o.jobs = len(jobs), arr
        keep.append(arr)
    if segments is not None:
        so, sl, sc = (np.ascontiguousarray(segments[0], np.int64), np.ascontiguousarray(segments[1], np.int64), _f32(segments[2]))
        keep += [so, sl, sc]
        o.n_seg = len(so)
        o.seg_off, o.seg_len, o.seg_coef = so.ctypes.data_as(C.POINTER(C.c_int64)), sl.ctypes.data_as(C.POINTER(C.c_int64)), _fp(sc)
    ins = [None if v is None else _f32(v).ravel() for v in (in0, in1)]
    outs = [np.empty(k, np.float32) if k else None for k in out_sizes]
    ptr = lambda a: None if a is None else _fp(a)
    check(ctx.lib.b2g_test_ew(ctx.h, precision, C.byref(o), *[ptr(a) for a in ins], *[ptr(a) for a in outs]))
    info = {"kernel": o.kernel.decode(), "sumsq": o.sumsq, "wide": [o.jobs[i].wide for i in range(o.n_jobs)] if jobs is not None else []}
    return outs, info


POOL_TEST_OPS = {"pool2d": 0, "global_pool": 1}


def test_pool(ctx: Context, precision: int, op: str, in0, in1, out_sizes=(0, 0, 0), *, pooling: str = "max", pnorm: float = 2.0, **opts):
    o = _lib.TestPoolOpts()
    o.op, o.pool, o.pnorm = POOL_TEST_OPS[op], POOLINGS[pooling], float(pnorm)
    for k, v in opts.items():
        setattr(o, k, int(v))
    ins = [_f32(v).ravel() for v in (in0, in1)]
    outs = [np.empty(k, np.float32) if k else None for k in out_sizes]
    ptr = lambda a: None if a is None else _fp(a)
    check(ctx.lib.b2g_test_pool(ctx.h, precision, C.byref(o), *[ptr(a) for a in ins], *[ptr(a) for a in outs]))
    return outs, {"kernel": o.kernel.decode(), "splits": o.splits}
```

include/b200gan.h:

```cpp
#ifndef B200GAN_H
#define B200GAN_H

#include <stddef.h>
#include <stdint.h>

#ifdef __cplusplus
extern "C" {
#endif

#define B2G_VERSION 101
#define B2G_NAME_LEN 64

typedef struct b2g_ctx b2g_ctx;
typedef struct b2g_net b2g_net;
typedef struct b2g_gan b2g_gan;

typedef enum {
  B2G_OK = 0,
  B2G_ERR_ARG = -1,
  B2G_ERR_SHAPE = -2,
  B2G_ERR_CUDA = -3,
  B2G_ERR_NCCL = -4,
  B2G_ERR_OOM = -5,
  B2G_ERR_UNSUPPORTED = -6,
// ... 41 lines not shown
typedef enum { B2G_PREC_FP32 = 0, B2G_PREC_BF16 = 1 } b2g_precision;
typedef enum {
  B2G_LOSS_XENT = 0, B2G_LOSS_MCXENT = 1, B2G_LOSS_MSE = 2, B2G_LOSS_L1 = 3, B2G_LOSS_L2 = 4, B2G_LOSS_MAE = 5, B2G_LOSS_HINGE = 6,
  B2G_LOSS_SQUARED_HINGE = 7, B2G_LOSS_WASSERSTEIN = 8
} b2g_loss;

typedef struct {
  int32_t type;
  char name[B2G_NAME_LEN];
  int32_t n_in, n_out;
  int32_t k_h, k_w, s_h, s_w, p_h, p_w;
  int32_t has_bias;
  int32_t act;
  float act_alpha;
  int32_t updater;
  float lr, beta1, beta2, eps;
  float l2;
  float bn_decay, bn_eps;
  int32_t pre_h, pre_w, pre_c;
  int32_t loss;
  int32_t frozen;
} b2g_layer_desc;

typedef struct {
  int32_t in_h, in_w, in_c;
  int32_t max_batch;
  int32_t precision;
  float grad_clip;
  float xent_clip_eps;
  int32_t bn_groups;
  uint64_t seed;
} b2g_net_config;

int32_t b2g_version(void);
int32_t b2g_ctx_create(int32_t device, b2g_ctx** out);
int32_t b2g_ctx_destroy(b2g_ctx* ctx);
const char* b2g_last_error(void);
int32_t b2g_sync(b2g_ctx* ctx);
int32_t b2g_launch_count(b2g_ctx* ctx, uint64_t* out);
int32_t b2g_timer_start(b2g_ctx* ctx);
int32_t b2g_timer_stop_ms(b2g_ctx* ctx, float* ms);
int32_t b2g_flush_l2(b2g_ctx* ctx);
int32_t b2g_device_info(b2g_ctx* ctx, int32_t* sm_count, int32_t* cc_major, int32_t* cc_minor, uint64_t* mem_bytes);

int32_t b2g_net_create(b2g_ctx* ctx, const b2g_net_config* cfg, const b2g_layer_desc* layers, int32_t n_layers, b2g_net** out);
int32_t b2g_net_destroy(b2g_net* net);
int32_t b2g_net_num_params(b2g_net* net, int64_t* out);
int32_t b2g_net_output_size(b2g_net* net, int64_t* per_example);
int32_t b2g_net_layer_output_size(b2g_net* net, int32_t layer, int64_t* per_example);
int32_t b2g_net_set_param(b2g_net* net, const char* layer, const char* param, const float* host, int64_t n);
int32_t b2g_net_get_param(b2g_net* net, const char* layer, const char* param, float* host, int64_t n);
int32_t b2g_net_get_params(b2g_net* net, float* host, int64_t n);
int32_t b2g_net_set_params(b2g_net* net, const float* host, int64_t n);
int32_t b2g_net_get_gradients(b2g_net* net, float* host, int64_t n);
int32_t b2g_net_updater_state_size(b2g_net* net, int64_t* out);
int32_t b2g_net_get_updater_state(b2g_net* net, float* host, int64_t n);
int32_t b2g_net_set_updater_state(b2g_net* net, const float* host, int64_t n);
int32_t b2g_net_output(b2g_net* net, const float* x, int32_t batch, int32_t train, float* out);
int32_t b2g_net_get_activation(b2g_net* net, int32_t layer, int32_t batch, float* host);
int32_t b2g_net_compute_gradient_and_score(b2g_net* net, const float* x, const float* y, int32_t batch, float* score);
int32_t b2g_net_get_input_gradient(b2g_net* net, int32_t batch, float* host);
int32_t b2g_net_fit(b2g_net* net, const float* x, const float* y, int32_t batch, float* score);
int32_t b2g_net_get_iteration(b2g_net* net, int64_t* out);
int32_t b2g_net_set_iteration(b2g_net* net, int64_t iteration);
int32_t b2g_net_get_dropout_pass(b2g_net* net, int64_t* out);
int32_t b2g_net_set_dropout_pass(b2g_net* net, int64_t pass);
typedef enum {
  B2G_GN_NONE = 0, B2G_GN_RENORM_L2_LAYER = 1, B2G_GN_RENORM_L2_PARAM = 2, B2G_GN_CLIP_ELEMENTWISE = 3, B2G_GN_CLIP_L2_LAYER = 4, B2G_GN_CLIP_L2_PARAM = 5
} b2g_gradient_normalization;
int32_t b2g_net_set_gradient_normalization(b2g_net* net, int32_t mode, float threshold);
typedef enum {
  B2G_CONSTRAINT_MAX_NORM = 0, B2G_CONSTRAINT_MIN_MAX_NORM = 1, B2G_CONSTRAINT_UNIT_NORM = 2, B2G_CONSTRAINT_NON_NEGATIVE = 3
} b2g_constraint_kind;
typedef struct {
  int32_t kind;
  int32_t dims_mask;
  double max_norm, min_norm, rate;
} b2g_constraint;
int32_t b2g_net_set_constraints(b2g_net* net, const char* layer, const char* param, const b2g_constraint* list, int32_t n);
int32_t b2g_net_apply_constraints(b2g_net* net);
typedef enum {
  B2G_SCHED_NONE = 0, B2G_SCHED_EXPONENTIAL = 1, B2G_SCHED_INVERSE = 2, B2G_SCHED_SIGMOID = 3, B2G_SCHED_STEP = 4, B2G_SCHED_MAP = 5
} b2g_schedule_kind;
typedef enum { B2G_SCHED_ITERATION = 0, B2G_SCHED_EPOCH = 1 } b2g_schedule_type;
typedef struct {
  int32_t kind, type;
  double initial, gamma, power, step, decay_rate;
  int32_t n_map;
  const int32_t* map_keys;
  const double* map_values;
} b2g_lr_schedule;
int32_t b2g_net_set_lr_schedule(b2g_net* net, const char* layer, const b2g_lr_schedule* s);
int32_t b2g_net_get_learning_rate(b2g_net* net, const char* layer, float* out);
int32_t b2g_net_get_epoch(b2g_net* net, int64_t* out);
int32_t b2g_net_set_epoch(b2g_net* net, int64_t epoch);
int32_t b2g_net_simt_gemm_calls(b2g_net* net, uint64_t* out);

typedef struct {
  int32_t fake_bn_train;
  int32_t use_cuda_graph;
} b2g_gan_config;
int32_t b2g_gan_create(b2g_net* gen, b2g_net* dis, const b2g_gan_config* cfg, b2g_gan** out);
int32_t b2g_gan_destroy(b2g_gan* gan);
int32_t b2g_gan_step(b2g_gan* gan, const float* x_real, const float* z_d, const float* z_g,
                     const float* y_real, const float* y_fake, const float* y_gen, int32_t batch, float* losses);
int32_t b2g_gan_upload(b2g_gan* gan, const float* x_real, const float* z_d, const float* z_g,
                       const float* y_real, const float* y_fake, const float* y_gen, int32_t batch);
int32_t b2g_gan_step_resident(b2g_gan* gan, int32_t batch);
int32_t b2g_gan_read_losses(b2g_gan* gan, float* losses);
int32_t b2g_gan_last_step_ms(b2g_gan* gan, float* ms);

#define B2G_NCCL_ID_BYTES 128
int32_t b2g_comm_unique_id(void* id128);
int32_t b2g_ctx_comm_init(b2g_ctx* ctx, int32_t world, int32_t rank, const void* id128);
int32_t b2g_ctx_comm_destroy(b2g_ctx* ctx);
int32_t b2g_net_set_grad_allreduce(b2g_net* net, int32_t enabled);
int32_t b2g_net_average_parameters(b2g_net* net);
int32_t b2g_net_set_sync_bn(b2g_net* net, int32_t enabled);
int32_t b2g_net_set_grad_payload_bf16(b2g_net* net, int32_t enabled);
int32_t b2g_net_enable_p2p_allreduce(b2g_net* net, int32_t* enabled);
int32_t b2g_ctx_allreduce_test(b2g_ctx* ctx, float* host_inout, int64_t n);

typedef struct {
  int32_t n, h, w, c;
  int32_t oh, ow, o;
  int32_t kh, kw, sh, sw, ph, pw;
} b2g_conv_geom;
int32_t b2g_test_conv(b2g_ctx* ctx, int32_t kind, int32_t impl, int32_t precision, const b2g_conv_geom* g,
                      const float* x_or_dy, const float* w_or_x, float* out, int32_t iters, float* ms_per_iter);
typedef struct {
  int32_t epi;
  int32_t act; float alpha;
  const float* bias;
  const float* scale;
  int32_t groups;
  const float* aux;
  const float* aux2;
  double* stats;
  char kernel[64];
  int32_t bn;
  int32_t max_ctas;
  int32_t poison;
  int32_t w_mn;
  int32_t per_tap;
  int32_t slab;
  int32_t defer;
  float* db;
  int32_t param_offset;
  int32_t splits;
} b2g_test_conv_opts;
int32_t b2g_test_conv_ex(b2g_ctx* ctx, int32_t kind, int32_t impl, int32_t precision, const b2g_conv_geom* g,
                         const float* x_or_dy, const float* w_or_x, float* out, int32_t iters, float* ms_per_iter, b2g_test_conv_opts* opts);

int32_t b2g_test_hbm_kernels(b2g_net* net, int32_t rows, int32_t channels, int32_t iters, float* ms3);

int32_t b2g_test_bn(b2g_ctx* ctx, int32_t precision, int32_t path, int32_t groups, int32_t rows, int32_t C, const float* x, const float* eps_out,
                    const float* gamma, const float* beta, const float* run_mean, const float* run_var, int32_t act, float alpha, float eps, float decay,
                    int32_t want_param_grads, float* y, float* eps_in, float* g_gamma, float* g_beta, float* g_mean, float* g_var, float* mean, float* invstd);
int32_t b2g_test_net_shadow(b2g_net* net, int32_t layer, int32_t which, float* out, int64_t n);
int32_t b2g_test_dropout(b2g_ctx* ctx, int32_t precision, uint64_t seed, int32_t layer, int32_t rank, int64_t pass, int32_t rows, int32_t h, int32_t w,
                         int32_t c, float p, const float* x, const float* dy, float* y, float* dx);

typedef enum {
  B2G_EW_REDUCE_SPLITS = 0, B2G_EW_REDUCE_MULTI = 1, B2G_EW_COLSUM = 2, B2G_EW_XENT = 3, B2G_EW_SOFTMAX_XENT = 4,
  B2G_EW_ACT_FWD = 5, B2G_EW_ACT_BWD = 6, B2G_EW_MAXPOOL = 7, B2G_EW_UPSAMPLE = 8, B2G_EW_SUMSQ = 9, B2G_EW_LOSS = 10,
  B2G_EW_ACT_EXT_FWD = 11, B2G_EW_ACT_EXT_BWD = 12, B2G_EW_CNN_XENT = 13, B2G_EW_CNN_SOFTMAX_XENT = 14,
  B2G_EW_VERTEX_FWD = 15, B2G_EW_VERTEX_BWD = 16, B2G_EW_MERGE_FWD = 17, B2G_EW_MERGE_BWD = 18, B2G_EW_SKIP_ADD = 19
} b2g_ew_op;
typedef struct {
  int64_t n, stride, src_off, dst_off;
  int32_t splits;
  int32_t wide;
} b2g_ew_reduce_job;
typedef struct {
  int32_t op;
  int64_t n;
  int32_t rows, cols;
  int32_t groups;
  int32_t splits; int64_t stride;
  int32_t N, H, W, C, KH, KW, SH, SW;
  int32_t act; float alpha;
  float clip_eps;
  int32_t offset;
  int32_t in_place;
  int32_t accumulate;
  int32_t poison;
  int32_t n_jobs; b2g_ew_reduce_job* jobs;
  int32_t n_seg; const int64_t* seg_off; const int64_t* seg_len; const float* seg_coef;
  double sumsq;
  char kernel[64];
  int32_t loss;
} b2g_test_ew_opts;
int32_t b2g_test_ew(b2g_ctx* ctx, int32_t precision, b2g_test_ew_opts* opts, const float* in0, const float* in1, float* out0, float* out1, float* out2);

typedef enum { B2G_TEST_POOL2D = 0, B2G_TEST_GLOBAL_POOL = 1 } b2g_test_pool_op;
typedef struct {
  int32_t op;
  int32_t pool;
  float pnorm;
  int32_t N, H, W, C, KH, KW, SH, SW, PH, PW;
  int32_t offset;
  int32_t poison;
  char kernel[64];
  int32_t splits;
} b2g_test_pool_opts;
int32_t b2g_test_pool(b2g_ctx* ctx, int32_t precision, b2g_test_pool_opts* opts, const float* in0, const float* in1, float* out0, float* out1, float* out2);

#ifdef __cplusplus
}
#endif
#endif
```

Baseline: 92600.

## Size conv grids to leave room for concurrent wgrad kernels

Passes the grid size and per-CTA work of the weight-gradient kernel running alongside into the fprop/dgrad tensor-core conv launches, so their persistent grid can be capped to share SMs with the side-stream wgrad. When no input gradient is needed, wgrad now runs on the main stream instead of forking to the side stream, and pending reductions are flushed on the main stream after the join. Adds a test hook that logs the chosen grids. The cap could leave SMs idle if the work estimates are wrong.

```diff
diff --git a/gan_deeplearning4j_b200/__init__.py b/gan_deeplearning4j_b200/__init__.py
--- a/gan_deeplearning4j_b200/__init__.py
+++ b/gan_deeplearning4j_b200/__init__.py
@@ -1,3 +1,3 @@
 from ._lib import B200GanError, LIB_PATH, PROTOTYPES, load
-from .engine import BF16, FP32, EPI_ACTBWD, EPI_BNBWD, EPI_PLAIN, EPI_STATS, Context, Gan, Net, comm_unique_id, test_bn, test_conv, test_conv_ex, test_dropout, test_ew, test_pool
+from .engine import BF16, FP32, EPI_ACTBWD, EPI_BNBWD, EPI_PLAIN, EPI_STATS, Context, Gan, Net, comm_unique_id, test_bn, test_conv, test_conv_ex, test_conv_grids, test_dropout, test_ew, test_pool
 from . import data, models, parallel, serializer
diff --git a/gan_deeplearning4j_b200/_lib.py b/gan_deeplearning4j_b200/_lib.py
--- a/gan_deeplearning4j_b200/_lib.py
+++ b/gan_deeplearning4j_b200/_lib.py
@@ -134,6 +134,7 @@
     "b2g_ctx_allreduce_test": (_i32, [_vp, _fp, _i64]),
     "b2g_test_conv": (_i32, [_vp, _i32, _i32, _i32, C.POINTER(ConvGeom), _fp, _fp, _fp, _i32, _fp]),
     "b2g_test_hbm_kernels": (_i32, [_vp, _i32, _i32, _i32, _fp]),
+    "b2g_test_conv_grids": (_i32, [_i32, C.POINTER(C.c_int64), _i32]),
     "b2g_test_conv_ex": (_i32, [_vp, _i32, _i32, _i32, C.POINTER(ConvGeom), _fp, _fp, _fp, _i32, _fp, C.POINTER(TestConvOpts)]),
     "b2g_test_bn": (_i32, [_vp, _i32, _i32, _i32, _i32, _i32, _fp, _fp, _fp, _fp, _fp, _fp, _i32, C.c_float, C.c_float, C.c_float,
                            _i32, _fp, _fp, _fp, _fp, _fp, _fp, _fp, _fp]),
diff --git a/gan_deeplearning4j_b200/csrc/engine.cu b/gan_deeplearning4j_b200/csrc/engine.cu
--- a/gan_deeplearning4j_b200/csrc/engine.cu
+++ b/gan_deeplearning4j_b200/csrc/engine.cu
@@ -512,7 +512,7 @@
 
 static inline int sync_bn_world(const b2g_net* n) { return (n->sync_bn && n->ctx->comm && n->ctx->world > 1) ? n->ctx->world : 1; }
 static int32_t gemm_fprop(b2g_net* n, const LayerRT& l, const ConvGeom& g, const void* x, const float* bias, void* out, int act, float alpha,
-                          const float* scale = nullptr, const TcEpi* fuse = nullptr, bool* fused = nullptr) {
+                          const float* scale = nullptr, const TcEpi* fuse = nullptr, bool* fused = nullptr, const TcGrid* beside = nullptr) {
   cudaStream_t s = fstream(n); int wp; const void* w = w_ptr(n, l, &wp);
   if (fused) *fused = false;
   if (scale) {
@@ -523,15 +523,15 @@
   if (edge_conv_small_cin_supported(g)) { note_simt(n); k_edge_conv_small_cin(n->prec, wp, g, x, w, bias, out, act, alpha, s); return 0; }
   if (dense_small_o_supported(g)) { note_simt(n); k_dense_small_o_fwd(n->prec, wp, g, x, w, bias, out, act, alpha, s); return 0; }
   if (tc_on(n) && tc_fprop_supported(g)) {
-    if (fuse && k_tc_fprop(g, (const __nv_bfloat16*)x, (const __nv_bfloat16*)w, bias, (__nv_bfloat16*)out, act, alpha, s, fuse) == 0) { if (fused) *fused = true; return 0; }
-    if (k_tc_fprop(g, (const __nv_bfloat16*)x, (const __nv_bfloat16*)w, bias, (__nv_bfloat16*)out, act, alpha, s) == 0) return 0;
+    if (fuse && k_tc_fprop(g, (const __nv_bfloat16*)x, (const __nv_bfloat16*)w, bias, (__nv_bfloat16*)out, act, alpha, s, fuse, 0, beside) == 0) { if (fused) *fused = true; return 0; }
+    if (k_tc_fprop(g, (const __nv_bfloat16*)x, (const __nv_bfloat16*)w, bias, (__nv_bfloat16*)out, act, alpha, s, nullptr, 0, beside) == 0) return 0;
     return fail(B2G_ERR_CUDA, "tensor-core fprop launch failed");
   }
   if (n->prec == PREC_BF16 && head_conv_supported(g)) { k_head_fwd(g, (const __nv_bfloat16*)x, (const __nv_bfloat16*)w, bias, (__nv_bfloat16*)out, act, alpha, s); return 0; }
   note_simt(n); k_simt_fprop(n->prec, wp, g, x, w, bias, out, act, alpha, s); return 0;
 }
 static int32_t gemm_dgrad(b2g_net* n, const LayerRT& l, const ConvGeom& g, const void* dy, const float* bias, void* dx, int act, float alpha,
-                          const float* scale = nullptr, const TcEpi* fuse = nullptr, bool* fused = nullptr) {
+                          const float* scale = nullptr, const TcEpi* fuse = nullptr, bool* fused = nullptr, const TcGrid* beside = nullptr) {
   cudaStream_t s = fstream(n); int wp; const void* w = w_ptr(n, l, &wp);
   if (fused) *fused = false;
   if (scale) {
@@ -540,7 +540,7 @@
   }
   if (tc_on(n) && l.off_Wps_bf >= 0 && tc_deconv_ps_supported(g)) {
     const TcEpi* f = (fuse && fuse->mode == EPI_ACTBWD) ? fuse : nullptr;
-    if (k_tc_deconv_ps(g, (const __nv_bfloat16*)dy, n->shadow + l.off_Wps_bf, bias, (__nv_bfloat16*)dx, act, alpha, s, f) == 0) { if (fused) *fused = f != nullptr; return 0; }
+    if (k_tc_deconv_ps(g, (const __nv_bfloat16*)dy, n->shadow + l.off_Wps_bf, bias, (__nv_bfloat16*)dx, act, alpha, s, f, beside) == 0) { if (fused) *fused = f != nullptr; return 0; }
     return fail(B2G_ERR_CUDA, "tensor-core pixel-shuffle deconv launch failed");
   }
   if (edge_deconv_small_c_supported(g)) { note_simt(n); k_edge_deconv_small_c(n->prec, wp, g, dy, w, bias, dx, act, alpha, s); return 0; }
@@ -549,26 +549,29 @@
   if (tc_on(n) && g.KH == 1 && g.KW == 1 && g.H == 1 && g.W == 1) {
     ConvGeom t = g; t.C = g.O; t.O = g.C;
     if (tc_fprop_supported(t)) {
-      if (fuse && k_tc_fprop(t, (const __nv_bfloat16*)dy, (const __nv_bfloat16*)w, bias, (__nv_bfloat16*)dx, act, alpha, s, fuse, 1) == 0) { if (fused) *fused = true; return 0; }
-      if (k_tc_fprop(t, (const __nv_bfloat16*)dy, (const __nv_bfloat16*)w, bias, (__nv_bfloat16*)dx, act, alpha, s, nullptr, 1) == 0) return 0;
+      if (fuse && k_tc_fprop(t, (const __nv_bfloat16*)dy, (const __nv_bfloat16*)w, bias, (__nv_bfloat16*)dx, act, alpha, s, fuse, 1, beside) == 0) { if (fused) *fused = true; return 0; }
+      if (k_tc_fprop(t, (const __nv_bfloat16*)dy, (const __nv_bfloat16*)w, bias, (__nv_bfloat16*)dx, act, alpha, s, nullptr, 1, beside) == 0) return 0;
       return fail(B2G_ERR_CUDA, "tensor-core dense dgrad launch failed");
     }
   }
   if (tc_on(n) && tc_dgrad_supported(g)) {
-    if (fuse && k_tc_dgrad(g, (const __nv_bfloat16*)dy, (const __nv_bfloat16*)w, bias, (__nv_bfloat16*)dx, act, alpha, s, fuse) == 0) { if (fused) *fused = true; return 0; }
-    if (k_tc_dgrad(g, (const __nv_bfloat16*)dy, (const __nv_bfloat16*)w, bias, (__nv_bfloat16*)dx, act, alpha, s) == 0) return 0;
+    if (fuse && k_tc_dgrad(g, (const __nv_bfloat16*)dy, (const __nv_bfloat16*)w, bias, (__nv_bfloat16*)dx, act, alpha, s, fuse, beside) == 0) { if (fused) *fused = true; return 0; }
+    if (k_tc_dgrad(g, (const __nv_bfloat16*)dy, (const __nv_bfloat16*)w, bias, (__nv_bfloat16*)dx, act, alpha, s, nullptr, beside) == 0) return 0;
     return fail(B2G_ERR_CUDA, "tensor-core dgrad launch failed");
   }
   if (n->prec == PREC_BF16 && head_conv_supported(g)) { k_head_dgrad(g, (const __nv_bfloat16*)dy, (const __nv_bfloat16*)w, bias, (__nv_bfloat16*)dx, act, alpha, s); return 0; }
   note_simt(n); k_simt_dgrad(n->prec, wp, g, dy, w, bias, dx, act, alpha, s); return 0;
 }
-static int32_t gemm_wgrad(b2g_net* n, LayerRT& l, const ConvGeom& g, const void* x, const void* dy, float* dw, cudaStream_t s, float* scratch, float* db = nullptr, bool* bias_done = nullptr) {
-  if (tc_on(n) && tc_edge_wgrad_supported(g) && l.wg_part) { const int r = k_tc_edge_wgrad(g, (const __nv_bfloat16*)x, (const __nv_bfloat16*)dy, dw, db, l.wg_part, l.wg_part_floats, 0, s, &n->pending); if (r >= 0) { if (bias_done) *bias_done = r == 1; return 0; } }
+static int32_t gemm_wgrad(b2g_net* n, LayerRT& l, const ConvGeom& g, const void* x, const void* dy, float* dw, cudaStream_t s, float* scratch, float* db = nullptr, bool* bias_done = nullptr,
+                          TcGrid* grid = nullptr) {
+  if (grid) *grid = TcGrid{0, 0};
+  if (tc_on(n) && tc_edge_wgrad_supported(g) && l.wg_part) { const int r = k_tc_edge_wgrad(g, (const __nv_bfloat16*)x, (const __nv_bfloat16*)dy, dw, db, l.wg_part, l.wg_part_floats, 0, s, &n->pending);
+    if (r >= 0) { if (bias_done) *bias_done = r == 1; if (grid) *grid = k_tc_edge_wgrad_grid(g); return 0; } }
   if (edge_wgrad_small_cin_supported(g)) { note_simt(n); k_edge_wgrad_small_cin(n->prec, g, x, dy, dw, scratch, 0, s); return 0; }
   if (dense_small_o_supported(g)) { note_simt(n); k_dense_small_o_wgrad(n->prec, g, x, dy, dw, scratch, 0, s); return 0; }
   if (dense_small_k_supported(g) && !(tc_on(n) && tc_wgrad_supported(g))) { note_simt(n); k_dense_small_k_wgrad(n->prec, g, x, dy, dw, s); return 0; }
   if (tc_on(n) && tc_wgrad_supported(g) && l.wg_part) {
-    if (k_tc_wgrad(g, (const __nv_bfloat16*)x, (const __nv_bfloat16*)dy, dw, l.wg_part, l.wg_part_floats, 0, s, &n->pending) == 0) return 0;
+    if (k_tc_wgrad(g, (const __nv_bfloat16*)x, (const __nv_bfloat16*)dy, dw, l.wg_part, l.wg_part_floats, 0, s, &n->pending) == 0) { if (grid) *grid = k_tc_wgrad_grid(g); return 0; }
     return fail(B2G_ERR_CUDA, "tensor-core wgrad launch failed");
   }
   if (n->prec == PREC_BF16 && head_conv_supported(g) && l.wg_part) {
@@ -749,28 +752,32 @@
         ConvGeom g = l.geom; g.N = R;
         if (d.act != B2G_ACT_IDENTITY && !act_done[i]) k_act_bwd_from_output(n->prec, l.out, cur, cur, (size_t)R * l.out_elems, d.act, d.act_alpha, s);
         if (l.ext_z) k_act_ext_bwd(n->prec, l.ext_act, l.ext_alpha, l.ext_z, cur, (size_t)R * l.out_elems, s);
+        TcGrid wg{0, 0};
         if (want_wgrad_l) {
-          fork_wgrad(i, cur);
+          const cudaStream_t ws = need_in ? s2 : s; float* const ws_scratch = need_in ? n->scratch2 : n->scratch;
+          if (need_in) fork_wgrad(i, cur);
           bool bias_done = false;
-          B2(gemm_wgrad(n, l, g, lin, cur, n->grads + l.off_W, s2, n->scratch2, l.off_b >= 0 ? n->grads + l.off_b : nullptr, &bias_done));
-          if (l.off_b >= 0 && !bias_done) k_colsum(n->prec, cur, R * l.oh * l.ow, l.oc, n->scratch2, n->grads + l.off_b, 0, s2);
-          mark_reader(i, cur);
+          B2(gemm_wgrad(n, l, g, lin, cur, n->grads + l.off_W, ws, ws_scratch, l.off_b >= 0 ? n->grads + l.off_b : nullptr, &bias_done, &wg));
+          if (l.off_b >= 0 && !bias_done) k_colsum(n->prec, cur, R * l.oh * l.ow, l.oc, ws_scratch, n->grads + l.off_b, 0, ws);
+          if (need_in) mark_reader(i, cur);
         }
         if (need_in) { void* nx = other(cur); TcEpi e{}; int tgt; bool fused = false; const bool can = pick_fuse(i, &e, &tgt);
-          B2(gemm_dgrad(n, l, g, cur, nullptr, nx, ACT_IDENTITY, 0.f, nullptr, can ? &e : nullptr, &fused)); note_fused(tgt, e, fused); cur = nx; }
+          B2(gemm_dgrad(n, l, g, cur, nullptr, nx, ACT_IDENTITY, 0.f, nullptr, can ? &e : nullptr, &fused, &wg)); note_fused(tgt, e, fused); cur = nx; }
       } break;
       case B2G_LAYER_DECONV2D: {
         ConvGeom g = l.geom; g.N = R;
         if (d.act != B2G_ACT_IDENTITY && !act_done[i]) k_act_bwd_from_output(n->prec, l.out, cur, cur, (size_t)R * l.out_elems, d.act, d.act_alpha, s);
         if (l.ext_z) k_act_ext_bwd(n->prec, l.ext_act, l.ext_alpha, l.ext_z, cur, (size_t)R * l.out_elems, s);
+        TcGrid wg{0, 0};
         if (want_wgrad_l) {
-          fork_wgrad(i, cur);
-          B2(gemm_wgrad(n, l, g,  cur,  lin, n->grads + l.off_W, s2, n->scratch2));
-          if (l.off_b >= 0) k_colsum(n->prec, cur, R * l.oh * l.ow, l.oc, n->scratch2, n->grads + l.off_b, 0, s2);
-          mark_reader(i, cur);
+          const cudaStream_t ws = need_in ? s2 : s; float* const ws_scratch = need_in ? n->scratch2 : n->scratch;
+          if (need_in) fork_wgrad(i, cur);
+          B2(gemm_wgrad(n, l, g,  cur,  lin, n->grads + l.off_W, ws, ws_scratch, nullptr, nullptr, &wg));
+          if (l.off_b >= 0) k_colsum(n->prec, cur, R * l.oh * l.ow, l.oc, ws_scratch, n->grads + l.off_b, 0, ws);
+          if (need_in) mark_reader(i, cur);
         }
         if (need_in) { void* nx = other(cur); TcEpi e{}; int tgt; bool fused = false; const bool can = pick_fuse(i, &e, &tgt);
-          B2(gemm_fprop(n, l, g, cur, nullptr, nx, ACT_IDENTITY, 0.f, nullptr, can ? &e : nullptr, &fused)); note_fused(tgt, e, fused); cur = nx; }
+          B2(gemm_fprop(n, l, g, cur, nullptr, nx, ACT_IDENTITY, 0.f, nullptr, can ? &e : nullptr, &fused, &wg)); note_fused(tgt, e, fused); cur = nx; }
       } break;
       case B2G_LAYER_BATCHNORM: {
         if (d.frozen) { if (need_in) return fail(B2G_ERR_UNSUPPORTED, "layer %d: a gradient through a frozen BatchNorm (trainable layer or input gradient below it) is not implemented", i); break; }
@@ -813,7 +820,8 @@
     if (!need_in) { cur = nullptr; break; }
   }
   n->input_grad = cur;
-  if (forked) { flush_pending_reduce(n, s2); cudaEventRecord(n->ev_join, s2); cudaStreamWaitEvent(s, n->ev_join, 0); }
+  if (forked) { cudaEventRecord(n->ev_join, s2); cudaStreamWaitEvent(s, n->ev_join, 0); }
+  flush_pending_reduce(n, s);
   CHECK_KERNELS();
   return 0;
 }
@@ -2138,6 +2146,18 @@
   return 0;
 }
 
+extern "C" int32_t b2g_test_conv_grids(int32_t no_side_cap, int64_t* out, int32_t max_entries) {
+  if (max_entries > 0 && !out) return fail(B2G_ERR_ARG, "null");
+  const int made = g_tc_conv_log.count, kept = std::min(std::min(made, (int)TcConvLog::CAP), std::max(max_entries, 0));
+  for (int i = 0; i < kept; ++i) {
+    const TcConvLog::Entry& e = g_tc_conv_log.e[i];
+    const int64_t v[5] = {e.grid, e.tiles, e.tile_work, e.beside.ctas, e.beside.work};
+    memcpy(out + 5 * i, v, sizeof(v));
+  }
+  g_tc_conv_log.count = 0; g_tc_test_no_side_cap = no_side_cap ? 1 : 0;
+  return made;
+}
+
 extern "C" int32_t b2g_test_hbm_kernels(b2g_net* n, int32_t rows, int32_t channels, int32_t iters, float* ms3) {
   if (!n || !ms3 || rows < 8 || iters < 1) return fail(B2G_ERR_ARG, "bad arguments"); b2g_ctx* c = n->ctx; CU(cudaSetDevice(c->device)); cudaStream_t s = c->stream;
   if (!k_bn_vec_ok(PREC_BF16, channels)) return fail(B2G_ERR_UNSUPPORTED, "channels %d not supported by the vector BatchNorm kernels", channels);
diff --git a/gan_deeplearning4j_b200/csrc/kernels.h b/gan_deeplearning4j_b200/csrc/kernels.h
--- a/gan_deeplearning4j_b200/csrc/kernels.h
+++ b/gan_deeplearning4j_b200/csrc/kernels.h
@@ -195,6 +195,16 @@
 extern int g_tc_test_per_tap;
 extern bool g_tc_last_slab;
 extern int g_tc_test_splits, g_tc_last_splits;
+struct TcGrid { int ctas; long work; };
+TcGrid k_tc_wgrad_grid(const ConvGeom& g);
+TcGrid k_tc_edge_wgrad_grid(const ConvGeom& g);
+struct TcConvLog {
+  static const int CAP = 256;
+  struct Entry { int grid, tiles; long tile_work; TcGrid beside; } e[CAP];
+  int count;
+};
+extern TcConvLog g_tc_conv_log;
+extern int g_tc_test_no_side_cap;
 enum { EPI_PLAIN = 0, EPI_STATS = 1, EPI_BNBWD = 2, EPI_ACTBWD = 3 };
 struct TcEpi {
   int mode;
@@ -205,8 +215,10 @@
   const __nv_bfloat16* aux2;
   int act; float alpha;
 };
-int k_tc_fprop(const ConvGeom& g, const __nv_bfloat16* x, const __nv_bfloat16* w, const float* bias, __nv_bfloat16* out, int act, float alpha, cudaStream_t s, const TcEpi* epi = nullptr, int w_mn = 0);
-int k_tc_dgrad(const ConvGeom& g, const __nv_bfloat16* dy, const __nv_bfloat16* w, const float* bias, __nv_bfloat16* dx, int act, float alpha, cudaStream_t s, const TcEpi* epi = nullptr);
+int k_tc_fprop(const ConvGeom& g, const __nv_bfloat16* x, const __nv_bfloat16* w, const float* bias, __nv_bfloat16* out, int act, float alpha, cudaStream_t s, const TcEpi* epi = nullptr, int w_mn = 0,
+               const TcGrid* beside = nullptr);
+int k_tc_dgrad(const ConvGeom& g, const __nv_bfloat16* dy, const __nv_bfloat16* w, const float* bias, __nv_bfloat16* dx, int act, float alpha, cudaStream_t s, const TcEpi* epi = nullptr,
+               const TcGrid* beside = nullptr);
 int k_tc_wgrad(const ConvGeom& g, const __nv_bfloat16* x, const __nv_bfloat16* dy, float* dw, float* scratch, size_t scratch_floats, int accumulate, cudaStream_t s, ReduceList* defer = nullptr);
 size_t k_tc_wgrad_scratch_floats(const ConvGeom& g);
 bool tc_deconv_ps_shape(const ConvGeom& g);
@@ -218,6 +230,7 @@
 size_t k_tc_edge_wgrad_scratch_floats(const ConvGeom& g);
 int k_tc_edge_conv(const ConvGeom& g, const __nv_bfloat16* x, const __nv_bfloat16* w, const float* bias, __nv_bfloat16* out, int act, float alpha, cudaStream_t s);
 int k_tc_edge_wgrad(const ConvGeom& g, const __nv_bfloat16* x, const __nv_bfloat16* dy, float* dw, float* db, float* scratch, size_t scratch_floats, int accumulate, cudaStream_t s, ReduceList* defer = nullptr);
-int k_tc_deconv_ps(const ConvGeom& g, const __nv_bfloat16* dy, const __nv_bfloat16* wps, const float* bias, __nv_bfloat16* dx, int act, float alpha, cudaStream_t s, const TcEpi* epi = nullptr);
+int k_tc_deconv_ps(const ConvGeom& g, const __nv_bfloat16* dy, const __nv_bfloat16* wps, const float* bias, __nv_bfloat16* dx, int act, float alpha, cudaStream_t s, const TcEpi* epi = nullptr,
+                   const TcGrid* beside = nullptr);
 
 }
diff --git a/gan_deeplearning4j_b200/csrc/kernels_tc.cu b/gan_deeplearning4j_b200/csrc/kernels_tc.cu
--- a/gan_deeplearning4j_b200/csrc/kernels_tc.cu
+++ b/gan_deeplearning4j_b200/csrc/kernels_tc.cu
@@ -493,6 +493,8 @@
 bool g_tc_last_slab = false;
 int g_tc_test_bn = 0, g_tc_test_max_ctas = 0, g_tc_test_per_tap = 0, g_tc_test_splits = 0;
 int g_tc_last_splits = 0;
+TcConvLog g_tc_conv_log = {};
+int g_tc_test_no_side_cap = 0;
 static int tc_device() { int dev = 0; cudaGetDevice(&dev); return dev < 0 || dev >= 64 ? 0 : dev; }
 #define TC_SET_SMEM_ONCE(kernel, bytes)                                                                                            \
   do { static bool set_[64] = {}; const int d_ = tc_device();                                                                       \
@@ -526,31 +528,46 @@
 }
 static bool tc_epi_ok(const TcEpi* e, int Nt) { return !e || e->mode == EPI_PLAIN || e->mode == EPI_ACTBWD || (e->imgs_per_group > 0 && e->imgs_per_group % Nt == 0 && e->acc); }
 
+static int side_cap(long tiles, long tile_work, const TcGrid* beside) {
+  const int sms = device_sm_count();
+  if (!beside || g_tc_test_no_side_cap || beside->ctas <= 0 || beside->ctas >= sms) return 0;
+  const long free = sms - beside->ctas, full = std::min<long>(tiles, sms);
+  if (full <= free) return 0;
+  const long capped = std::max(beside->work, (tiles + free - 1) / free * tile_work);
+  const long uncapped = beside->work + (tiles + full - 1) / full * tile_work;
+  return capped < uncapped ? (int)free : 0;
+}
+static unsigned conv_grid(long tiles, long tile_work, const TcGrid* beside) {
+  const int cap = g_tc_test_max_ctas > 0 ? g_tc_test_max_ctas : side_cap(tiles, tile_work, beside);
+  const unsigned grid = (unsigned)std::min<long>(tiles, cap > 0 ? cap : device_sm_count());
+  if (g_tc_conv_log.count < TcConvLog::CAP) g_tc_conv_log.e[g_tc_conv_log.count] = {(int)grid, (int)tiles, tile_work, beside ? *beside : TcGrid{0, 0}};
+  ++g_tc_conv_log.count;
+  return grid;
+}
 template <int BN, int STAGES, int EPI, bool AFFINE, bool PS = false, bool SLAB = false>
-static int launch_conv_e(const CUtensorMap& tmA, const CUtensorMap& tmB, const TcConvParams& p, cudaStream_t s) {
+static int launch_conv_e(const CUtensorMap& tmA, const CUtensorMap& tmB, const TcConvParams& p, unsigned grid, cudaStream_t s) {
   using S = TcSmem<BN, STAGES, EPI, SLAB>;
   TC_SET_SMEM_ONCE((tc_conv_kernel<BN, STAGES, EPI, AFFINE, PS, SLAB>), S::TOTAL);
-  const long tiles = (long)p.tiles_m * p.tiles_n * p.phases;
-  const unsigned grid = (unsigned)std::min<long>(tiles, g_tc_test_max_ctas > 0 ? g_tc_test_max_ctas : device_sm_count());
   launch_pdl(tc_conv_kernel<BN, STAGES, EPI, AFFINE, PS, SLAB>, dim3(grid), dim3(TC_CONV_THREADS), (size_t)(S::TOTAL), s, tmA, tmB, p);
   LAUNCHED();
   return cudaPeekAtLastError() == cudaSuccess ? 0 : -3;
 }
 template <int BN, int STAGES, bool SLAB>
-static int launch_conv(const CUtensorMap& tmA, const CUtensorMap& tmB, const TcConvParams& p, cudaStream_t s, const char* name) {
+static int launch_conv(const CUtensorMap& tmA, const CUtensorMap& tmB, const TcConvParams& p, unsigned grid, cudaStream_t s, const char* name) {
   g_tc_last_kernel = name; g_tc_last_slab = SLAB;
   switch (p.epi) {
-    case EPI_STATS: return launch_conv_e<BN, STAGES, EPI_STATS, false, false, SLAB>(tmA, tmB, p, s);
-    case EPI_BNBWD: return launch_conv_e<BN, STAGES, EPI_BNBWD, false, false, SLAB>(tmA, tmB, p, s);
-    case EPI_ACTBWD: return launch_conv_e<BN, STAGES, EPI_ACTBWD, false, false, SLAB>(tmA, tmB, p, s);
-  }
-  return (p.scale && p.bias) ? launch_conv_e<BN, STAGES, EPI_PLAIN, true, false, SLAB>(tmA, tmB, p, s) : launch_conv_e<BN, STAGES, EPI_PLAIN, false, false, SLAB>(tmA, tmB, p, s);
-}
-static int dispatch_conv(int BN, bool slab, const CUtensorMap& tmA, const CUtensorMap& tmB, const TcConvParams& p, cudaStream_t s) {
+    case EPI_STATS: return launch_conv_e<BN, STAGES, EPI_STATS, false, false, SLAB>(tmA, tmB, p, grid, s);
+    case EPI_BNBWD: return launch_conv_e<BN, STAGES, EPI_BNBWD, false, false, SLAB>(tmA, tmB, p, grid, s);
+    case EPI_ACTBWD: return launch_conv_e<BN, STAGES, EPI_ACTBWD, false, false, SLAB>(tmA, tmB, p, grid, s);
+  }
+  return (p.scale && p.bias) ? launch_conv_e<BN, STAGES, EPI_PLAIN, true, false, SLAB>(tmA, tmB, p, grid, s) : launch_conv_e<BN, STAGES, EPI_PLAIN, false, false, SLAB>(tmA, tmB, p, grid, s);
+}
+static int dispatch_conv(int BN, bool slab, const CUtensorMap& tmA, const CUtensorMap& tmB, const TcConvParams& p, long tile_work, const TcGrid* beside, cudaStream_t s) {
+  const unsigned grid = conv_grid((long)p.tiles_m * p.tiles_n * p.phases, tile_work, beside);
   switch (BN * 2 + slab) {
-    case 128: return launch_conv<64, 4, false>(tmA, tmB, p, s, "tc_conv_kernel<64,4>");
-    case 256: return launch_conv<128, 4, false>(tmA, tmB, p, s, "tc_conv_kernel<128,4>");
-    case 129: return launch_conv<64, 4, true>(tmA, tmB, p, s, "tc_conv_kernel<64,4>");
+    case 128: return launch_conv<64, 4, false>(tmA, tmB, p, grid, s, "tc_conv_kernel<64,4>");
+    case 256: return launch_conv<128, 4, false>(tmA, tmB, p, grid, s, "tc_conv_kernel<128,4>");
+    case 129: return launch_conv<64, 4, true>(tmA, tmB, p, grid, s, "tc_conv_kernel<64,4>");
   }
   return -4;
 }
@@ -581,7 +598,8 @@
   if (e->mode == EPI_BNBWD || e->mode == EPI_ACTBWD) { p.act = e->act; p.alpha = e->alpha; p.bias = nullptr; p.scale = nullptr; }
 }
 
-int k_tc_fprop(const ConvGeom& g, const __nv_bfloat16* x, const __nv_bfloat16* w, const float* bias, __nv_bfloat16* out, int act, float alpha, cudaStream_t s, const TcEpi* epi, int w_mn) {
+int k_tc_fprop(const ConvGeom& g, const __nv_bfloat16* x, const __nv_bfloat16* w, const float* bias, __nv_bfloat16* out, int act, float alpha, cudaStream_t s, const TcEpi* epi, int w_mn,
+               const TcGrid* beside) {
   TcConvParams p{}; p.mode = 0;
   if (!pick_row_tile(g.N, g.OH, g.OW, 128, &p.Nt, &p.Ht, &p.Wt) || !tc_epi_ok(epi, p.Nt)) return -1;
   if (w_mn && (g.KH != 1 || g.KW != 1)) return -1;
@@ -599,10 +617,11 @@
   if (make_map_bf16(&tmA, x, 4, dims, strides, box, es)) return -1;
   p.tiles_m = g.N * g.OH * g.OW / 128; p.tiles_n = g.O / BN; p.phases = 1;
   if (w_mn ? weight_map(&tmB, w, g.C, 1, g.O, 64) : weight_map(&tmB, w, g.O, g.KH * g.KW, g.C, BN)) return -1;
-  return dispatch_conv(BN, slab, tmA, tmB, p, s);
-}
-
-int k_tc_dgrad(const ConvGeom& g, const __nv_bfloat16* dy, const __nv_bfloat16* w, const float* bias, __nv_bfloat16* dx, int act, float alpha, cudaStream_t s, const TcEpi* epi) {
+  return dispatch_conv(BN, slab, tmA, tmB, p, (long)g.KH * g.KW * p.chunks * BN, beside, s);
+}
+
+int k_tc_dgrad(const ConvGeom& g, const __nv_bfloat16* dy, const __nv_bfloat16* w, const float* bias, __nv_bfloat16* dx, int act, float alpha, cudaStream_t s, const TcEpi* epi,
+               const TcGrid* beside) {
   TcConvParams p{}; p.mode = 1;
   if (!pick_row_tile(g.N, g.OH, g.OW, 128, &p.Nt, &p.Ht, &p.Wt) || !tc_epi_ok(epi, p.Nt)) return -1;
   const int BN = pick_bn_fill(g.C, (long)g.N * g.OH * g.OW / 128 * 4);
@@ -619,7 +638,7 @@
   if (weight_map(&tmB, w, g.O, 16, g.C, 64)) return -1;
   if (make_map_bf16(&tmA, dy, 4, dims, strides, box, es)) return -1;
   p.tiles_m = g.N * g.OH * g.OW / 128; p.tiles_n = g.C / BN; p.phases = 4;
-  return dispatch_conv(BN, slab, tmA, tmB, p, s);
+  return dispatch_conv(BN, slab, tmA, tmB, p, 4L * p.chunks * BN, beside, s);
 }
 
 bool tc_deconv_ps_shape(const ConvGeom& g) { return is_k4s2p1_geom(g) && g.C >= 1 && g.C <= 4 && g.O % 64 == 0; }
@@ -636,7 +655,8 @@
 void k_pack_deconv_ps(const float* w, __nv_bfloat16* wps, int O, int C, cudaStream_t s) {
   launch_pdl(pack_deconv_ps_kernel, dim3((16 * 9 * O + 255) / 256), dim3(256), (size_t)(0), s, w, wps, O, C); LAUNCHED();
 }
-int k_tc_deconv_ps(const ConvGeom& g, const __nv_bfloat16* dy, const __nv_bfloat16* wps, const float* bias, __nv_bfloat16* dx, int act, float alpha, cudaStream_t s, const TcEpi* epi) {
+int k_tc_deconv_ps(const ConvGeom& g, const __nv_bfloat16* dy, const __nv_bfloat16* wps, const float* bias, __nv_bfloat16* dx, int act, float alpha, cudaStream_t s, const TcEpi* epi,
+                   const TcGrid* beside) {
   TcConvParams p{}; p.mode = 0;
   if (!tc_deconv_ps_shape(g) || !pick_row_tile(g.N, g.OH, g.OW, 128, &p.Nt, &p.Ht, &p.Wt)) return -1;
   if (epi && epi->mode != EPI_PLAIN && epi->mode != EPI_ACTBWD) return -1;
@@ -651,7 +671,8 @@
   if (weight_map(&tmB, wps, 16, 9, g.O, 16)) return -1;
   p.tiles_m = (int)((long)g.N * g.OH * g.OW / 128); p.tiles_n = 1; p.phases = 1;
   g_tc_last_kernel = "tc_conv_kernel<16,4,PS>";
-  return p.epi == EPI_ACTBWD ? launch_conv_e<16, 4, EPI_ACTBWD, false, true>(tmA, tmB, p, s) : launch_conv_e<16, 4, EPI_PLAIN, false, true>(tmA, tmB, p, s);
+  const unsigned grid = conv_grid(p.tiles_m, 9L * p.chunks * 16, beside);
+  return p.epi == EPI_ACTBWD ? launch_conv_e<16, 4, EPI_ACTBWD, false, true>(tmA, tmB, p, grid, s) : launch_conv_e<16, 4, EPI_PLAIN, false, true>(tmA, tmB, p, grid, s);
 }
 
 struct TcEdgeParams {
@@ -845,6 +866,11 @@
   const int tiles = g.N * (g.OH / ht), target = g_tc_test_splits > 0 ? g_tc_test_splits : tc_edge_wgrad_target();
   const int per = (tiles + target - 1) / target; *tpc = per < 1 ? 1 : per;
   return (tiles + *tpc - 1) / *tpc;
+}
+TcGrid k_tc_edge_wgrad_grid(const ConvGeom& g) {
+  if (!tc_edge_wgrad_supported(g)) return {0, 0};
+  int tpc = 1; const int ctas = tc_edge_wgrad_ctas(g, &tpc);
+  return {ctas, 64L * tpc};
 }
 size_t k_tc_edge_wgrad_scratch_floats(const ConvGeom& g) { return tc_edge_wgrad_supported(g) ? (size_t)tc_edge_wgrad_target() * (64 * 16 * g.C + 64) : 0; }
 int k_tc_edge_conv(const ConvGeom& g, const __nv_bfloat16* x, const __nv_bfloat16* w, const float* bias, __nv_bfloat16* out, int act, float alpha, cudaStream_t s) {
@@ -989,6 +1015,12 @@
   int a, b, c;
   return g.O % 128 == 0 && wgrad_bnw(g) != 0 && g.SH >= 1 && g.SH <= 2 && g.SW == g.SH && ((long)g.N * g.OH * g.OW) % 64 == 0 &&
          pick_row_tile(g.N, g.OH, g.OW, 64, &a, &b, &c) && c * g.SW <= 256 && b * g.SH <= 256;
+}
+TcGrid k_tc_wgrad_grid(const ConvGeom& g) {
+  if (!tc_wgrad_supported(g)) return {0, 0};
+  const int bnw = wgrad_bnw(g), splits = tc_wgrad_splits(g);
+  const long kbt = (long)g.N * g.OH * g.OW / 64, per = (kbt + splits - 1) / splits;
+  return {splits * (g.KH * g.KW * g.C / bnw) * (g.O / 128), per * bnw};
 }
 size_t k_tc_wgrad_scratch_floats(const ConvGeom& g) {
   if (!tc_wgrad_supported(g)) return 0;
diff --git a/gan_deeplearning4j_b200/engine.py b/gan_deeplearning4j_b200/engine.py
--- a/gan_deeplearning4j_b200/engine.py
+++ b/gan_deeplearning4j_b200/engine.py
@@ -547,6 +547,14 @@
             self.h = None
 
 
+def test_conv_grids(no_side_cap: bool = False) -> np.ndarray:
+    lib = _lib.load()
+    out = np.zeros((256, 5), np.int64)
+    n = lib.b2g_test_conv_grids(1 if no_side_cap else 0, out.ctypes.data_as(C.POINTER(C.c_int64)), out.shape[0])
+    check(min(n, 0))
+    return out[:min(n, out.shape[0])].copy()
+
+
 def test_conv(ctx: Context, kind: int, impl: int, precision: int, geom: Dict[str, int], a, b, out_size: int, iters: int = 1):
     g = _lib.ConvGeom(**geom)
     a, b = _f32(a).ravel(), _f32(b).ravel()
diff --git a/include/b200gan.h b/include/b200gan.h
--- a/include/b200gan.h
+++ b/include/b200gan.h
@@ -217,6 +217,8 @@
 int32_t b2g_test_conv_ex(b2g_ctx* ctx, int32_t kind, int32_t impl, int32_t precision, const b2g_conv_geom* g,
                          const float* x_or_dy, const float* w_or_x, float* out, int32_t iters, float* ms_per_iter, b2g_test_conv_opts* opts);
 
+int32_t b2g_test_conv_grids(int32_t no_side_cap, int64_t* out, int32_t max_entries);
+
 int32_t b2g_test_hbm_kernels(b2g_net* net, int32_t rows, int32_t channels, int32_t iters, float* ms3);
 
 int32_t b2g_test_bn(b2g_ctx* ctx, int32_t precision, int32_t path, int32_t groups, int32_t rows, int32_t C, const float* x, const float* eps_out,
```

After: 94330, median of 6. 1.9% higher.
